# IVRL/NoiseDiff

Measured on AMD Instinct MI355X. Metric: sampled RAW patches/sec (256x256x4, 1000-step DDPM), higher is better.
Workload: dtype f32; 1 GPU; NoiseDiffNet dim=64, 256x256x4 patches, 1000-step DDPM (sigmoid2, pred_v), 16 patches per GPU; a step = one reverse-diffusion step (U-Net forward + fused posterior/noise update) over the per-GPU batch; patches/s = n_gpus*16/(1000*s_per_step); global_batch=16, launch=hipGraph replay, noise=device Philox4x32-10

## Files before the change

### include/noisediff_hip.h

```cpp
#ifndef NOISEDIFF_HIP_H
#define NOISEDIFF_HIP_H

#include <stdint.h>

#ifdef __cplusplus
extern "C" {
#endif

#define ND_E_BADARG   (-1)
#define ND_E_SHAPE    (-2)
#define ND_E_ALIGN    (-3)
#define ND_E_STATE    (-4)

int         nd_version(void);
const char* nd_last_error(void);
int         nd_device_arch(char* buf, int n);


enum nd_prologue {
    ND_PRO_NONE        = 0,
    ND_PRO_AFFINE_SILU = 1,
    ND_PRO_AFFINE_MAP_SILU = 2,
    ND_PRO_LAYERNORM   = 3,
    ND_PRO_SILU        = 4,
    ND_PRO_LEAKY       = 5,
    ND_PRO_LEAKY_SECOND = 6,
    ND_PRO_AFFINE_GENMAP_SILU = 7
};

typedef struct nd_src {
    const float* p0;
    const float* p1;
    int32_t c0, c1;
    int32_t ld0, ld1;
    int32_t mode;
    int32_t upsample;
    int32_t unshuffle;
    int32_t map_blocked;
    const float* mad;
    const float* map;
    const float* vec;
    const float* gamma;
    const float* beta;
    const float* rowstats;
} nd_src;

enum nd_act { ND_ACT_NONE = 0, ND_ACT_GELU = 1, ND_ACT_SILU = 2 };


typedef struct nd_conv3x3 {
    nd_src   src;
    const float* weight;
    const float* bias;
    float*   out;
    float*   stats;
    float*   slot_count;
    int32_t  B, H, W;
    int32_t  cin, cout, ldo;
} nd_conv3x3;

int nd_conv3x3_nhwc_f32(const nd_conv3x3* d, void* stream);
int nd_conv3x3_stat_slots(int H, int W, int cout, int B);
int nd_conv3x3_tiling_id(int B, int H, int W, int cout);
int64_t nd_pack_conv3x3_weight_floats(int cin, int cout);
int nd_pack_conv3x3_weight(const float* oihw, float* packed, int cin, int cout, void* stream);
int nd_pack_conv3x3_weight_dgrad(const float* oihw_fwd, float* packed, int cin, int cout, void* stream);

int nd_conv3x3_wino_nhwc_f32(const nd_conv3x3* d, void* stream);
int nd_conv3x3_wino2_nhwc_f32(const nd_conv3x3* d, void* stream);
int nd_conv3x3_wino_stat_slots(int H, int W);
int64_t nd_pack_conv3x3_wino_weight_floats(int cin, int cout);
int nd_pack_conv3x3_wino_weight(const float* oihw, float* packed, int cin, int cout, void* stream);
int nd_pack_conv3x3_wino_weight_dgrad(const float* oihw_fwd, float* packed, int cin, int cout, void* stream);

int nd_conv3x3_wino4_nhwc_f32(const nd_conv3x3* d, void* stream);
int nd_conv3x3_wino4_16_nhwc_f32(const nd_conv3x3* d, void* stream);
int nd_conv3x3_wino4_stat_slots(int H, int W);
int64_t nd_pack_conv3x3_wino4_weight_floats(int cin, int cout);
int nd_pack_conv3x3_wino4_weight(const float* oihw, float* packed, int cin, int cout, void* stream);
int nd_pack_conv3x3_wino4_weight_dgrad(const float* oihw_fwd, float* packed, int cin, int cout, void* stream);
typedef struct nd_pack_item {
    const float* w;
    float*       packed;
    int32_t      cin, cout, transposed, reserved;
} nd_pack_item;
int nd_pack_conv3x3_wino4_weights_batch(const nd_pack_item* items_dev, int n_items, void* stream);
int nd_conv3x3_wino4_splitk_plan(int B, int H, int W, int cin, int cout);
int64_t nd_conv3x3_wino4_splitk_workspace_floats(int B, int H, int W, int cout, int splits);
int nd_conv3x3_wino4_splitk_nhwc_f32(const nd_conv3x3* d, float* workspace, int splits, void* stream);
int nd_conv3x3_wino4_16_splitk_plan(int H, int W, int cin, int cout);
int nd_conv3x3_wino4_16_splitk_nhwc_f32(const nd_conv3x3* d, float* workspace, int splits, void* stream);


int64_t nd_conv3x3_wgrad_workspace_floats(int B, int H, int W, int cin, int cout);
int nd_conv3x3_wgrad_cat_nhwc_f32(const float* x0, int ldx0, int c0, const float* x1, int ldx1, int c1, const float* dy, int ldy, float* dw_oihw,
                                  float* dbias, float* workspace, int B, int H, int W, int cout, void* stream);
int nd_conv3x3_wgrad_form(int form);
int nd_conv3x3_wgrad_nhwc_f32(const float* x, int ldx, const float* dy, int ldy, float* dw_oihw, float* dbias, float* workspace,
                              int B, int H, int W, int cin, int cout, void* stream);
int nd_conv3x3_wgrad_leaky_nhwc_f32(const float* x, int ldx, const float* dy, int ldy, float* dw_oihw, float* dbias, float* workspace,
                                    int B, int H, int W, int cin, int cout, void* stream);
int64_t nd_conv3x3_wgrad_cat_workspace_floats(int B, int H, int W, int c0, int c1, int cout);
int nd_conv3x3_wgrad_cat_leaky_second_nhwc_f32(const float* x0, int ldx0, int c0, const float* x1, int ldx1, int c1, const float* dy, int ldy,
                                               float* dw_oihw, float* dbias, float* workspace, int B, int H, int W, int cout, void* stream);
int nd_leaky_grad_join_f32(const float* z, float* dz, const float* d_direct, int ld_direct, const float* d_pool, int B, int H, int W, int C,
                           void* stream);

int64_t nd_groupnorm_train_workspace_floats(int B, int HW, int C);
int nd_groupnorm_train_forward_f32(const float* x, int ldx, const float* gamma, const float* beta, float* y, int ldy, float* mean_rstd,
                                   float* workspace, int B, int HW, int C, int groups, float eps, void* stream);
int nd_groupnorm_train_backward_f32(const float* dy, int lddy, const float* x, int ldx, const float* gamma, const float* mean_rstd,
                                    float* dx, int lddx, float* dgamma, float* dbeta, float* workspace, int B, int HW, int C, int groups,
                                    void* stream);

int64_t nd_groupnorm_silu_train_workspace_floats(int B, int HW, int C);
int nd_groupnorm_silu_train_forward_f32(const float* x, int ldx, const float* gamma, const float* beta, const float* scale_shift, const float* res, int ldr,
                                        float* y, int ldy, float* mean_rstd, float* mad, float* workspace, int B, int HW, int C, int groups, float eps,
                                        void* stream);
int nd_groupnorm_silu_train_backward_f32(const float* dy, int lddy, const float* x, int ldx, const float* gamma, const float* beta,
                                         const float* scale_shift, const float* mean_rstd, const float* mad, float* dx, int lddx,
                                         float* dgamma, float* dbeta, float* dscale_shift, float* workspace, int B, int HW, int C, int groups,
                                         void* stream);

int nd_modulate_silu_forward_f32(const float* n, int ldn, const float* map, int ldm, float* y, int ldy, int64_t N, int C, void* stream);
int nd_modulate_silu_backward_f32(const float* dy, int lddy, const float* n, int ldn, const float* map, int ldm, float* dn, int lddn, float* dmap, int lddm,
                                  int64_t N, int C, void* stream);

int64_t nd_token_sum_workspace_floats(int B, int HW, int C);
int nd_token_sum_f32(const float* x, int ldx, float* out, float* workspace, int B, int HW, int C, void* stream);

int64_t nd_layernorm_train_workspace_floats(int64_t N, int C);
int nd_layernorm_train_forward_f32(const float* x, int ldx, const float* gamma, const float* beta, float* y, int ldy, float* stats,
                                   int64_t N, int C, float eps, void* stream);
int nd_layernorm_train_backward_f32(const float* dy, int lddy, const float* x, int ldx, const float* gamma, const float* stats,
                                    float* dx, int lddx, float* dgamma, float* dbeta, float* workspace, int64_t N, int C, void* stream);

int64_t nd_linear_wgrad_workspace_floats(int64_t N, int cin, int cout);
int nd_linear_wgrad_f32(const float* x, int ldx, const float* dy, int ldy, float* dw, float* dbias, float* workspace,
                        int64_t N, int cin, int cout, void* stream);
int nd_linear_wgrad_leaky_f32(const float* x, int ldx, const float* dy, int ldy, float* dw, float* dbias, float* workspace,
                              int64_t N, int cin, int cout, void* stream);
int64_t nd_convt2x2_wgrad_workspace_floats(int B, int h, int w, int cin, int cout);
int nd_convt2x2_wgrad_leaky_f32(const float* x, int ldx, const float* d_up, int ld_up, float* dw, float* workspace, int B, int h, int w,
                                int cin, int cout, int up_h, int up_w, void* stream);


typedef struct nd_pointwise {
    nd_src   src;
    const float* weight;
    const float* bias;
    float*   out;
    const float* res0; const float* res1;
    const float* vec;
    const float* gn_t;
    const float* gn_mad;
    int32_t  B, HW, W;
    int32_t  cin, cout, ldo, ldr0, ldr1, ldt;
    int32_t  act;
    int32_t  shuffle_c;
    int32_t  shuffle_h, shuffle_w;
} nd_pointwise;

int nd_pointwise_gemm_nhwc_f32(const nd_pointwise* d, void* stream);
int nd_pointwise_gemm_unshuffle_crop_nhwc_f32(const nd_pointwise* d, int src_h, int src_w, void* stream);

int64_t nd_image_quality_workspace_bytes(int B, int C, int H, int W);
int nd_image_quality_f32(const float* est, const float* target, const float* scale, double data_range, double* psnr, double* ssim,
                         double* mse, void* workspace, int B, int C, int H, int W, void* stream);
int64_t nd_illum_scale_workspace_bytes(int B, int C, int H, int W);
int nd_illum_scale_f32(const float* pred, const float* source, int source_batch, float* k32, double* k64, void* workspace,
                       int B, int C, int H, int W, void* stream);
int nd_illum_apply_f32(const float* pred, const float* k32, float* out, int B, int C, int H, int W, void* stream);

int     nd_histogram_chunk_elements(void);
int64_t nd_histogram_workspace_bytes(int S, int64_t n, int n_bins);
int nd_histogram_f32(const float* x, int S, int64_t n, const double* edges, int n_edges, int64_t* counts, void* workspace, void* stream);
int nd_kl_div_f64(const int64_t* p_counts, const int64_t* q_counts, int64_t n_p, int64_t n_q, int n_bins, int S, int q_sets, double* out,
                  void* stream);
int nd_kl_div_hist_f64(const double* p, const double* q, int n_bins, int S, int q_sets, double* out, void* stream);
int64_t nd_patch_std_mean_workspace_bytes(int B, int C, int H, int W);
int nd_patch_std_mean_f32(const float* x, float* std, float* mean, double* fit, void* workspace, int B, int C, int H, int W, void* stream);

int64_t nd_level_table_bytes(int n_levels);
int nd_level_moments_reset(uint64_t* table, int n_levels, uint64_t* counters, void* stream);
int nd_level_moments_f32(const float* clean, const float* noisy, int64_t n, float scale, int n_levels, uint64_t* table, uint64_t* counters,
                         void* stream);
int nd_level_stats_f64(const uint64_t* table, int n_levels, int64_t* count, double* mean, double* std, void* stream);
int nd_level_curve_f64(const int64_t* count, const double* std, int n_levels, float scale, int below_median, double* x, double* y, int32_t* m,
                       void* stream);
int64_t nd_theil_sen_workspace_bytes(int max_m, int64_t n_pairs);
int nd_theil_sen_f64(const double* x, const double* y, const int32_t* m, int max_m, const int32_t* pairs, int64_t n_pairs, int max_iter,
                     double tol, double* out, void* workspace, void* stream);

typedef struct nd_denoise_sample {
    int32_t x0, y0;
    int32_t cx, cy;
    int32_t flip;
    int32_t branch;
    float iso, ratio, blc;
    int32_t reserved[3];
} nd_denoise_sample;
#define ND_DENOISE_SNA_WORDS 8
int nd_denoise_batch_f32(const float* noise, const float* clean, const float* ds_k_high, const float* ds_b_high, const float* ds_k_low,
                         const float* ds_b_low, int map_h, int map_w, const nd_denoise_sample* table, const float* sna, const int64_t* rng,
                         uint64_t seed, int64_t first_sample, int32_t draw, const float* counts_in, float* counts_out, float* noisy,
                         float* clean_out, int B, int patch, int crop_h, int crop_w, void* stream);
int nd_philox_poisson_f32(const float* rate, float* out, uint64_t seed, int64_t first_sample, int32_t draw, int B, int64_t n_per_sample,
                          void* stream);
int nd_pack_darkshading_f32(const float* bayer, float* planes, int H2, int W2, void* stream);

typedef struct nd_raw_sample {
    int32_t frame;
    int32_t frame_clean;
    int32_t x0, y0;
    int32_t flip;
    int32_t branch;
    float iso, ratio, blc;
    int32_t reserved;
    double k, sd, ratio64;
} nd_raw_sample;
enum nd_raw_mode {
    ND_RAW_PACK = 0,
    ND_RAW_PACK_SHADED = 1,
    ND_RAW_TRAIN_REAL = 2
};
#define ND_RAW_RESCALE 1
#define ND_RAW_CLIP 2
int nd_raw_pack_u16_f32(const uint16_t* frames, int N, int H2, int W2, const float* ds_k_high, const float* ds_b_high, const float* ds_k_low,
                        const float* ds_b_low, int map_h, int map_w, const nd_raw_sample* table, int mode, int flags, float black, float white,
                        float* out, float* clean_out, int B, int h, int w, void* stream);
int nd_raw_poisson_gaussian_f32(const uint16_t* frames, int N, int H2, int W2, const nd_raw_sample* table, const int64_t* rng, uint64_t seed,
                                int64_t first_sample, int32_t draw, const float* counts_in, const float* normals_in, float* counts_out,
                                float* normals_out, float black, float white, float* noisy, float* clean_out, int B, int h, int w,
                                void* stream);
int nd_raw_to_bayer_u16(const float* img, uint16_t* out, const int32_t* bl, int white, int B, int h, int w, void* stream);
int nd_raw_diffusion_batch_f32(const uint16_t* frames, int N, int H2, int W2, const nd_raw_sample* table, float black, float white, float* noise,
                               float* noisy, float* clean, float* coord, int B, int h, int w, void* stream);
int64_t nd_pack_pointwise_weight_floats(int cin, int cout);
int nd_pack_pointwise_weight(const float* w, float* packed, int cin, int cout, int unshuffle_c, void* stream);
int nd_pack_pointwise_weight_t(const float* w_t, float* packed, int cin, int cout, void* stream);
int nd_pack_pointwise_weights_batch(const nd_pack_item* items_dev, int n_items, void* stream);

int nd_pointwise_gemm_split_nhwc_f32(const nd_pointwise* d, void* stream);
int nd_pointwise_gemm_split_takes(const nd_pointwise* d);
int64_t nd_pack_pointwise_weight_split_floats(int cin, int cout);
int nd_pack_pointwise_weight_split(const float* w, float* packed, int cin, int cout, void* stream);

enum nd_chain_res { ND_CHAIN_RES_NONE = 0, ND_CHAIN_RES_INPUT = 1 , ND_CHAIN_RES_INPUT_RAW = 2  };
typedef struct nd_chain_stage {
    const float* weight;
    const float* bias;
    int32_t  cin, cout;
    int32_t  act;
    int32_t  res;
} nd_chain_stage;
typedef struct nd_chain {
    nd_src   src;
    nd_chain_stage st[3];
    float*   out;
    int32_t  n_stages, B, HW, ldo;
} nd_chain;
int nd_pointwise_chain_nhwc_f32(const nd_chain* d, void* stream);
int nd_pointwise_chain_supported(int cin, int n1, int n2, int n3);
int64_t nd_pack_chain_weight_floats(int cin, int cout, int first_stage);
int nd_pack_chain_weight(const float* w, float* packed, int cin, int cout, int first_stage, void* stream);
int nd_pointwise_chain_split_nhwc_f32(const nd_chain* d, void* stream);
int64_t nd_pack_chain_weight_split_floats(int cin, int cout, int first_stage);
int nd_pack_chain_weight_split(const float* w, float* packed, int cin, int cout, int first_stage, void* stream);


int nd_groupnorm_finalize_f32(const float* stats, const float* slot_count, int slots,
                              const float* gamma, const float* beta,
                              const float* scale_shift, int ld_ss,
                              float* mad, int B, int C, int groups, float eps, void* stream);
int nd_groupnorm_finalize_train_f32(const float* stats, const float* slot_count, int slots, const float* gamma, const float* beta,
                                    const float* scale_shift, int ld_ss, float* mad, float* mean_rstd, int B, int C, int groups, float eps,
                                    void* stream);

int nd_layernorm_stats_f32(const float* x, int ldx, const float* vec, float* stats,
                           int B, int HW, int C, float eps, void* stream);

int nd_affine_silu_add_f32(const float* t, int ldt, const float* mad,
                           const float* res0, int ldr0, const float* res1, int ldr1,
                           float* out, int ldo, int B, int HW, int C, void* stream);


int nd_linear_rows_f32(const float* in, int ld_in, const float* W, const float* bias,
                       float* out, int ld_out, int B, int K, int N,
                       int act_in, int act_out, void* stream);
int nd_sinusoidal_time_emb_f32(const int64_t* time, const float* freqs, float* emb, int B, int half, void* stream);
int64_t nd_cond_step_lds_bytes(int B, int dim);
int nd_cond_step_f32(const int64_t* time, const float* freqs, const float* W1, const float* b1, const float* W2, const float* b2,
                     const float* Wp, const float* bp, float* out, int ld_out, int B, int dim, int J, void* stream);
int nd_cond_table_build_f32(const float* freqs, const float* W1, const float* b1, const float* W2, const float* b2, float* table, int rows, int dim,
                            void* stream);
int nd_cond_step_table_f32(const int64_t* time, const float* freqs, const float* W1, const float* b1, const float* W2, const float* b2,
                           const float* Wp, const float* bp, float* out, int ld_out, int B, int dim, int J, const float* table, int table_rows,
                           void* stream);
int nd_cond_step_ptable_f32(const int64_t* time, const float* freqs, const float* W1, const float* b1, const float* W2, const float* b2,
                            const float* Wp, const float* bp, float* out, int ld_out, int B, int dim, int J, const float* table, int table_rows,
                            const float* ptable, void* stream);
int nd_embedding_rows_f32(const int64_t* idx, const float* table, float* out, int B, int rows, int dim, void* stream);


int nd_conv7x7_c4_f32(const float* x, const float* wpacked, const float* bias, float* out, int ldo,
                      int B, int H, int W, int cout, void* stream);
int64_t nd_conv7x7_c4_wgrad_workspace_floats(int B, int H, int W, int cout);
int nd_conv7x7_c4_wgrad_f32(const float* x, const float* dy, int ldy, float* dw_oihw, float* dbias, float* workspace, int B, int H, int W, int cout,
                            void* stream);
int nd_pack_conv7x7_weight(const float* oihw, float* packed, int cout, void* stream);
int nd_conv7x7_c4_split_f32(const float* x, const float* wsplit, const float* bias, float* out, int ldo,
                            int B, int H, int W, int cout, void* stream);
int64_t nd_pack_conv7x7_weight_split_floats(int cout);
int nd_pack_conv7x7_weight_split(const float* oihw, float* packed, int cout, void* stream);
int nd_pos_enc_f32(const float* position_nchw, const float* w , const float* bias,
                   float* out, int B, int H, int W, int hid, void* stream);
int nd_maxpool2x2_nhwc_f32(const float* in, float* out, int B, int H, int W, int C, void* stream);
int nd_nchw_to_nhwc_f32(const float* in, float* out, int B, int C, int H, int W, void* stream);
int nd_nhwc_to_nchw_f32(const float* in, float* out, int B, int C, int H, int W, void* stream);
int nd_nchw_to_nhwc_pad_f32(const float* in, float* out, int B, int C, int H, int W, int Cpad, void* stream);


typedef struct nd_sampler_state {
    int32_t* step;
    const int32_t* t_cur;
    const int32_t* t_next;
    const float* coef;
    int64_t* time_out;
    const int64_t* rng;
    int32_t n_steps, B;
} nd_sampler_state;

int nd_sampler_begin_step(const nd_sampler_state* s, void* stream);
int nd_sampler_advance(const nd_sampler_state* s, void* stream);

int nd_sampler_step_ddpm_f32(float* x, const float* model_out, const float* noise, int64_t noise_step_stride,
                             const nd_sampler_state* s, int objective,
                             uint64_t seed, int64_t first_sample,
                             int B, int HW, int C, void* stream);
int nd_sampler_step_ddim_f32(float* x, const float* model_out, const float* noise, int64_t noise_step_stride,
                             const nd_sampler_state* s, int objective,
                             uint64_t seed, int64_t first_sample,
                             int B, int HW, int C, void* stream);
int nd_philox_normal_f32(float* out, uint64_t seed, int64_t first_sample, int32_t step,
                         int B, int HW, int C, void* stream);


int nd_attention_mfma_f32(const float* qkv, int ld_qkv, float* out, int ld_out,
                          int B, int N, int heads, int dh, void* stream);
int64_t nd_linear_attention_workspace_floats(int B, int N, int heads);
int nd_linear_attention_f32(const float* qkv, int ld_qkv, float* out, int ld_out, float* workspace,
                            int B, int N, int heads, int dh, void* stream);
int nd_rmsnorm_nhwc_f32(const float* x, int ldx, const float* g, float* out, int ldo,
                        int B, int HW, int C, void* stream);
int nd_rmsnorm_add_nhwc_f32(const float* x, int ldx, const float* g, const float* res, int ldr, float* out, int ldo, int B, int HW, int C, void* stream);


int nd_attention_train_forward_f32(const float* qkv, int ld_qkv, float* out, int ld_out, float* lse,
                                   int B, int N, int heads, int dh, void* stream);
int64_t nd_attention_backward_workspace_floats(int B, int N, int heads);
int nd_attention_backward_f32(const float* qkv, int ld_qkv, const float* out, int ld_out, const float* dout, int ld_dout, const float* lse,
                              float* dqkv, int ld_dqkv, float* workspace, int B, int N, int heads, int dh, void* stream);
int64_t nd_linear_attention_backward_workspace_floats(int B, int N, int heads);
int nd_linear_attention_backward_f32(const float* qkv, int ld_qkv, const float* dout, int ld_dout, const float* fwd_workspace, float* dqkv,
                                     int ld_dqkv, float* workspace, int B, int N, int heads, int dh, void* stream);
int64_t nd_rmsnorm_backward_workspace_floats(int64_t npix, int C);
int nd_rmsnorm_backward_f32(const float* dy, int lddy, const float* x, int ldx, const float* g, float* dx, int lddx, float* dg, float* workspace,
                            int B, int HW, int C, void* stream);

typedef struct nd_adam_item {
    float*       p;
    const float* g;
    float*       m;
    float*       v;
    int64_t      n;
    float        step_size, bias2_sqrt;
    int32_t      vec4, reserved;
    float*       step;
} nd_adam_item;
int nd_adam_chunk_elements(void);
int nd_adam_step_f32(const nd_adam_item* items_dev, int n_items, const int32_t* chunks_dev, int n_chunks, float beta1, float beta2, float eps,
                     float weight_decay, void* stream);
int nd_adam_step_capturable_f32(const nd_adam_item* items_dev, int n_items, const int32_t* chunks_dev, int n_chunks, float lr, float beta1, float beta2,
                                float eps, float weight_decay, void* stream);
int nd_adam_step_capturable_lr_f32(const nd_adam_item* items_dev, int n_items, const int32_t* chunks_dev, int n_chunks, const float* lr_dev, float beta1,
                                   float beta2, float eps, float weight_decay, void* stream);

typedef struct nd_ema_item {
    float*       ema;
    const float* src;
    int64_t      n;
    int32_t      vec4, no_ema;
} nd_ema_item;
int nd_ema_chunk_elements(void);
int nd_ema_update_f32(const nd_ema_item* items_dev, int n_items, const int32_t* chunks_dev, int n_chunks, int64_t* step_dev, uint8_t* initted_dev,
                      void* plan_dev, double beta, int64_t update_after_step, int64_t update_every, double inv_gamma, double power, double min_value,
                      void* stream);

typedef struct nd_diffusion_noising {
    const float* x0;
    const float* noise;
    const float* offset;
    const int64_t* t_in;
    const float* sqrt_alphas_cumprod;
    const float* sqrt_one_minus_alphas_cumprod;
    const int64_t* rng;
    int64_t* t_out;
    float* x_t;
    float* target;
    float* noise_out;
    float* offset_out;
    uint64_t seed;
    int64_t first_sample;
    int64_t draw;
    float offset_strength;
    int32_t B, C, H, W, T;
    int32_t objective, auto_normalize, x0_channels_last;
} nd_diffusion_noising;
int nd_diffusion_noising_f32(const nd_diffusion_noising* p, void* stream);
int nd_diffusion_train_advance(int64_t* rng, void* stream);
int nd_diffusion_loss_slice_elements(void);
int64_t nd_diffusion_loss_workspace_bytes(int B, int C, int HW);
int nd_diffusion_loss_f32(const float* model_out, const float* target, const int64_t* t, const float* loss_weight, int B, int C, int HW, int T,
                          int x0_term, void* workspace, float* loss, float* sample_loss, void* stream);
int nd_diffusion_loss_backward_f32(const float* model_out, const float* target, const int64_t* t, const float* loss_weight, const float* g,
                                   const void* workspace, float* grad_out, int B, int C, int HW, int T, int x0_term, void* stream);

enum nd_layout { ND_LAYOUT_NCHW = 0, ND_LAYOUT_NHWC = 1 };
int nd_denoise_loss_slice_pixels(void);
int64_t nd_denoise_loss_workspace_bytes(int B, int C, int HW);
int nd_denoise_loss_f32(const float* out, int out_layout, const float* target, int B, int C, int HW, double lambda_l1, double lambda_mse,
                        void* workspace, float* terms, float* sample_terms, void* stream);
int nd_denoise_loss_backward_f32(const float* out, int out_layout, const float* target, const float* g, float* grad, int B, int C, int HW,
                                 double lambda_l1, double lambda_mse, void* stream);

int nd_stream_create(void** stream);
int nd_stream_destroy(void* stream);
int nd_stream_sync(void* stream);
int nd_graph_begin(void* stream);
int nd_graph_end(void* stream, void** graph_exec);
int nd_graph_launch(void* graph_exec, void* stream);
int nd_graph_destroy(void* graph_exec);
int nd_stream_device(void* stream);
int nd_event_create(void** ev);
int nd_event_record(void* ev, void* stream);
int nd_event_elapsed_ms(void* start, void* stop, float* ms);
int nd_event_destroy(void* ev);
int nd_event_create_untimed(void** ev);
int nd_stream_wait_event(void* stream, void* ev);

#ifdef __cplusplus
}
#endif
#endif
```

### noisediff_amd/_lib.py

```python
from __future__ import annotations

import ctypes as C
import os
from typing import Optional

HERE = os.path.dirname(os.path.abspath(__file__))
LIB_PATH = os.path.join(HERE, "libnoisediff_hip.so")

PRO_NONE, PRO_AFFINE_SILU, PRO_AFFINE_MAP_SILU, PRO_LAYERNORM, PRO_SILU, PRO_LEAKY, PRO_LEAKY_SECOND, PRO_AFFINE_GENMAP_SILU = 0, 1, 2, 3, 4, 5, 6, 7
ACT_NONE, ACT_GELU, ACT_SILU = 0, 1, 2
OBJECTIVES = {"pred_noise": 0, "pred_x0": 1, "pred_v": 2}
LAYOUT_NCHW, LAYOUT_NHWC = 0, 1

fptr = C.c_void_p


class HipError(RuntimeError):
    pass


class Src(C.Structure):
    _fields_ = [("p0", fptr), ("p1", fptr), ("c0", C.c_int32), ("c1", C.c_int32), ("ld0", C.c_int32), ("ld1", C.c_int32),
                ("mode", C.c_int32), ("upsample", C.c_int32), ("unshuffle", C.c_int32), ("map_blocked", C.c_int32),
                ("mad", fptr), ("map", fptr), ("vec", fptr), ("gamma", fptr), ("beta", fptr), ("rowstats", fptr)]


class AdamItem(C.Structure):
    _fields_ = [("p", fptr), ("g", fptr), ("m", fptr), ("v", fptr), ("n", C.c_int64), ("step_size", C.c_float), ("bias2_sqrt", C.c_float),
                ("vec4", C.c_int32), ("reserved", C.c_int32), ("step", fptr)]


class EmaItem(C.Structure):
    _fields_ = [("ema", fptr), ("src", fptr), ("n", C.c_int64), ("vec4", C.c_int32), ("no_ema", C.c_int32)]


class PackItem(C.Structure):
    _fields_ = [("w", fptr), ("packed", fptr), ("cin", C.c_int32), ("cout", C.c_int32), ("transposed", C.c_int32), ("reserved", C.c_int32)]


class Conv3x3(C.Structure):
    _fields_ = [("src", Src), ("weight", fptr), ("bias", fptr), ("out", fptr), ("stats", fptr), ("slot_count", fptr),
                ("B", C.c_int32), ("H", C.c_int32), ("W", C.c_int32), ("cin", C.c_int32), ("cout", C.c_int32), ("ldo", C.c_int32)]


class Pointwise(C.Structure):
    _fields_ = [("src", Src), ("weight", fptr), ("bias", fptr), ("out", fptr), ("res0", fptr), ("res1", fptr), ("vec", fptr),
                ("gn_t", fptr), ("gn_mad", fptr), ("B", C.c_int32), ("HW", C.c_int32), ("W", C.c_int32), ("cin", C.c_int32),
                ("cout", C.c_int32), ("ldo", C.c_int32), ("ldr0", C.c_int32), ("ldr1", C.c_int32), ("ldt", C.c_int32), ("act", C.c_int32),
                ("shuffle_c", C.c_int32), ("shuffle_h", C.c_int32), ("shuffle_w", C.c_int32)]


class ChainStage(C.Structure):
    _fields_ = [("weight", fptr), ("bias", fptr), ("cin", C.c_int32), ("cout", C.c_int32), ("act", C.c_int32), ("res", C.c_int32)]


class Chain(C.Structure):
    _fields_ = [("src", Src), ("st", ChainStage * 3), ("out", fptr), ("n_stages", C.c_int32), ("B", C.c_int32), ("HW", C.c_int32),
                ("ldo", C.c_int32)]


class RawSample(C.Structure):
    _fields_ = [("frame", C.c_int32), ("frame_clean", C.c_int32), ("x0", C.c_int32), ("y0", C.c_int32), ("flip", C.c_int32),
                ("branch", C.c_int32), ("iso", C.c_float), ("ratio", C.c_float), ("blc", C.c_float), ("reserved", C.c_int32),
                ("k", C.c_double), ("sd", C.c_double), ("ratio64", C.c_double)]


RAW_PACK, RAW_PACK_SHADED, RAW_TRAIN_REAL = 0, 1, 2
RAW_RESCALE, RAW_CLIP = 1, 2
CHAIN_RES_NONE, CHAIN_RES_INPUT, CHAIN_RES_INPUT_RAW = 0, 1, 2


class SamplerState(C.Structure):
    _fields_ = [("step", fptr), ("t_cur", fptr), ("t_next", fptr), ("coef", fptr), ("time_out", fptr), ("rng", fptr),
                ("n_steps", C.c_int32), ("B", C.c_int32)]


class DiffusionNoising(C.Structure):
    _fields_ = [("x0", fptr), ("noise", fptr), ("offset", fptr), ("t_in", fptr), ("sqrt_alphas_cumprod", fptr), ("sqrt_one_minus_alphas_cumprod", fptr),
                ("rng", fptr), ("t_out", fptr), ("x_t", fptr), ("target", fptr), ("noise_out", fptr), ("offset_out", fptr),
                ("seed", C.c_uint64), ("first_sample", C.c_int64), ("draw", C.c_int64), ("offset_strength", C.c_float),
                ("B", C.c_int32), ("C", C.c_int32), ("H", C.c_int32), ("W", C.c_int32), ("T", C.c_int32),
                ("objective", C.c_int32), ("auto_normalize", C.c_int32), ("x0_channels_last", C.c_int32)]


i32, i64, u64, vp, f32, f64 = C.c_int, C.c_int64, C.c_uint64, C.c_void_p, C.c_float, C.c_double

SIGNATURES = {
    "nd_version": (i32, []),
    "nd_last_error": (C.c_char_p, []),
    "nd_device_arch": (i32, [C.c_char_p, i32]),
    "nd_conv3x3_nhwc_f32": (i32, [C.POINTER(Conv3x3), vp]),
    "nd_conv3x3_stat_slots": (i32, [i32, i32, i32, i32]),
    "nd_conv3x3_tiling_id": (i32, [i32, i32, i32, i32]),
    "nd_pack_conv3x3_weight_floats": (i64, [i32, i32]),
    "nd_pack_conv3x3_weight": (i32, [vp, vp, i32, i32, vp]),
    "nd_pack_conv3x3_weight_dgrad": (i32, [vp, vp, i32, i32, vp]),
    "nd_conv3x3_wino_nhwc_f32": (i32, [C.POINTER(Conv3x3), vp]),
    "nd_conv3x3_wino2_nhwc_f32": (i32, [C.POINTER(Conv3x3), vp]),
    "nd_conv3x3_wino_stat_slots": (i32, [i32, i32]),
    "nd_conv3x3_wino4_stat_slots": (i32, [i32, i32]),
    "nd_pack_conv3x3_wino_weight_floats": (i64, [i32, i32]),
    "nd_pack_conv3x3_wino_weight": (i32, [vp, vp, i32, i32, vp]),
    "nd_pack_conv3x3_wino_weight_dgrad": (i32, [vp, vp, i32, i32, vp]),
    "nd_conv3x3_wino4_nhwc_f32": (i32, [C.POINTER(Conv3x3), vp]),
    "nd_conv3x3_wino4_16_nhwc_f32": (i32, [C.POINTER(Conv3x3), vp]),
    "nd_pack_conv3x3_wino4_weight_floats": (i64, [i32, i32]),
    "nd_pack_conv3x3_wino4_weight": (i32, [vp, vp, i32, i32, vp]),
    "nd_pack_conv3x3_wino4_weight_dgrad": (i32, [vp, vp, i32, i32, vp]),
    "nd_conv3x3_wino4_splitk_plan": (i32, [i32, i32, i32, i32, i32]),
    "nd_conv3x3_wino4_splitk_workspace_floats": (i64, [i32, i32, i32, i32, i32]),
    "nd_conv3x3_wino4_splitk_nhwc_f32": (i32, [vp, vp, i32, vp]),
    "nd_conv3x3_wino4_16_splitk_plan": (i32, [i32, i32, i32, i32]),
    "nd_conv3x3_wino4_16_splitk_nhwc_f32": (i32, [vp, vp, i32, vp]),
    "nd_conv3x3_wgrad_workspace_floats": (i64, [i32, i32, i32, i32, i32]),
    "nd_conv3x3_wgrad_nhwc_f32": (i32, [vp, i32, vp, i32, vp, vp, vp, i32, i32, i32, i32, i32, vp]),
    "nd_groupnorm_train_workspace_floats": (i64, [i32, i32, i32]),
    "nd_linear_wgrad_workspace_floats": (i64, [i64, i32, i32]),
    "nd_groupnorm_silu_train_workspace_floats": (i64, [i32, i32, i32]),
    "nd_groupnorm_silu_train_forward_f32": (i32, [vp, i32, vp, vp, vp, vp, i32, vp, i32, vp, vp, vp, i32, i32, i32, i32, C.c_float, vp]),
    "nd_token_sum_workspace_floats": (i64, [i32, i32, i32]),
    "nd_token_sum_f32": (i32, [vp, i32, vp, vp, i32, i32, i32, vp]),
    "nd_modulate_silu_forward_f32": (i32, [vp, i32, vp, i32, vp, i32, i64, i32, vp]),
    "nd_modulate_silu_backward_f32": (i32, [vp, i32, vp, i32, vp, i32, vp, i32, vp, i32, i64, i32, vp]),
    "nd_groupnorm_silu_train_backward_f32": (i32, [vp, i32, vp, i32, vp, vp, vp, vp, vp, vp, i32, vp, vp, vp, vp, i32, i32, i32, i32, vp]),
    "nd_layernorm_train_workspace_floats": (i64, [i64, i32]),
    "nd_layernorm_train_forward_f32": (i32, [vp, i32, vp, vp, vp, i32, vp, i64, i32, C.c_float, vp]),
    "nd_layernorm_train_backward_f32": (i32, [vp, i32, vp, i32, vp, vp, vp, i32, vp, vp, vp, i64, i32, vp]),
    "nd_linear_wgrad_f32": (i32, [vp, i32, vp, i32, vp, vp, vp, i64, i32, i32, vp]),
    "nd_groupnorm_train_forward_f32": (i32, [vp, i32, vp, vp, vp, i32, vp, vp, i32, i32, i32, i32, C.c_float, vp]),
    "nd_groupnorm_train_backward_f32": (i32, [vp, i32, vp, i32, vp, vp, vp, i32, vp, vp, vp, i32, i32, i32, i32, vp]),
    "nd_pointwise_gemm_nhwc_f32": (i32, [C.POINTER(Pointwise), vp]),
    "nd_pointwise_chain_nhwc_f32": (i32, [C.POINTER(Chain), vp]),
    "nd_pointwise_chain_supported": (i32, [i32, i32, i32, i32]),
    "nd_pack_chain_weight_floats": (i64, [i32, i32, i32]),
    "nd_pack_chain_weight": (i32, [vp, vp, i32, i32, i32, vp]),
    "nd_pointwise_chain_split_nhwc_f32": (i32, [C.POINTER(Chain), vp]),
    "nd_pack_chain_weight_split_floats": (i64, [i32, i32, i32]),
    "nd_pack_chain_weight_split": (i32, [vp, vp, i32, i32, i32, vp]),
    "nd_pointwise_gemm_split_nhwc_f32": (i32, [C.POINTER(Pointwise), vp]),
    "nd_pointwise_gemm_split_takes": (i32, [C.POINTER(Pointwise)]),
    "nd_pack_pointwise_weight_split_floats": (i64, [i32, i32]),
    "nd_pack_pointwise_weight_split": (i32, [vp, vp, i32, i32, vp]),
    "nd_pack_pointwise_weight_floats": (i64, [i32, i32]),
    "nd_pack_pointwise_weight": (i32, [vp, vp, i32, i32, i32, vp]),
    "nd_pack_pointwise_weight_t": (i32, [vp, vp, i32, i32, vp]),
    "nd_pack_pointwise_weights_batch": (i32, [vp, i32, vp]),
    "nd_pack_conv3x3_wino4_weights_batch": (i32, [vp, i32, vp]),
    "nd_conv3x3_wgrad_cat_nhwc_f32": (i32, [vp, i32, i32, vp, i32, i32, vp, i32, vp, vp, vp, i32, i32, i32, i32, vp]),
    "nd_conv3x3_wgrad_form": (i32, [i32]),
    "nd_conv7x7_c4_wgrad_workspace_floats": (i64, [i32, i32, i32, i32]),
    "nd_conv7x7_c4_wgrad_f32": (i32, [vp, vp, i32, vp, vp, vp, i32, i32, i32, i32, vp]),
    "nd_adam_chunk_elements": (i32, []),
    "nd_adam_step_f32": (i32, [vp, i32, vp, i32, f32, f32, f32, f32, vp]),
    "nd_adam_step_capturable_f32": (i32, [vp, i32, vp, i32, f32, f32, f32, f32, f32, vp]),
    "nd_adam_step_capturable_lr_f32": (i32, [vp, i32, vp, i32, vp, f32, f32, f32, f32, vp]),
    "nd_ema_chunk_elements": (i32, []),
    "nd_ema_update_f32": (i32, [vp, i32, vp, i32, vp, vp, vp, f64, i64, i64, f64, f64, f64, vp]),
    "nd_diffusion_noising_f32": (i32, [C.POINTER(DiffusionNoising), vp]),
    "nd_diffusion_train_advance": (i32, [vp, vp]),
    "nd_diffusion_loss_slice_elements": (i32, []),
    "nd_diffusion_loss_workspace_bytes": (i64, [i32, i32, i32]),
    "nd_diffusion_loss_f32": (i32, [vp, vp, vp, vp, i32, i32, i32, i32, i32, vp, vp, vp, vp]),
    "nd_diffusion_loss_backward_f32": (i32, [vp, vp, vp, vp, vp, vp, vp, i32, i32, i32, i32, i32, vp]),
    "nd_denoise_loss_slice_pixels": (i32, []),
    "nd_denoise_loss_workspace_bytes": (i64, [i32, i32, i32]),
    "nd_denoise_loss_f32": (i32, [vp, i32, vp, i32, i32, i32, f64, f64, vp, vp, vp, vp]),
    "nd_denoise_loss_backward_f32": (i32, [vp, i32, vp, vp, vp, i32, i32, i32, f64, f64, vp]),
    "nd_groupnorm_finalize_f32": (i32, [vp, vp, i32, vp, vp, vp, i32, vp, i32, i32, i32, f32, vp]),
    "nd_groupnorm_finalize_train_f32": (i32, [vp, vp, i32, vp, vp, vp, i32, vp, vp, i32, i32, i32, f32, vp]),
    "nd_layernorm_stats_f32": (i32, [vp, i32, vp, vp, i32, i32, i32, f32, vp]),
    "nd_affine_silu_add_f32": (i32, [vp, i32, vp, vp, i32, vp, i32, vp, i32, i32, i32, i32, vp]),
    "nd_linear_rows_f32": (i32, [vp, i32, vp, vp, vp, i32, i32, i32, i32, i32, i32, vp]),
    "nd_sinusoidal_time_emb_f32": (i32, [vp, vp, vp, i32, i32, vp]),
    "nd_cond_step_lds_bytes": (i64, [i32, i32]),
    "nd_cond_step_f32": (i32, [vp, vp, vp, vp, vp, vp, vp, vp, vp, i32, i32, i32, i32, vp]),
    "nd_cond_table_build_f32": (i32, [vp, vp, vp, vp, vp, vp, i32, i32, vp]),
    "nd_cond_step_table_f32": (i32, [vp, vp, vp, vp, vp, vp, vp, vp, vp, i32, i32, i32, i32, vp, i32, vp]),
    "nd_cond_step_ptable_f32": (i32, [vp, vp, vp, vp, vp, vp, vp, vp, vp, i32, i32, i32, i32, vp, i32, vp, vp]),
    "nd_embedding_rows_f32": (i32, [vp, vp, vp, i32, i32, i32, vp]),
    "nd_conv7x7_c4_f32": (i32, [vp, vp, vp, vp, i32, i32, i32, i32, i32, vp]),
    "nd_pack_conv7x7_weight": (i32, [vp, vp, i32, vp]),
    "nd_conv7x7_c4_split_f32": (i32, [vp, vp, vp, vp, i32, i32, i32, i32, i32, vp]),
    "nd_pack_conv7x7_weight_split_floats": (i64, [i32]),
    "nd_pack_conv7x7_weight_split": (i32, [vp, vp, i32, vp]),
    "nd_pos_enc_f32": (i32, [vp, vp, vp, vp, i32, i32, i32, i32, vp]),
    "nd_maxpool2x2_nhwc_f32": (i32, [vp, vp, i32, i32, i32, i32, vp]),
    "nd_nchw_to_nhwc_pad_f32": (i32, [vp, vp, i32, i32, i32, i32, i32, vp]),
    "nd_nchw_to_nhwc_f32": (i32, [vp, vp, i32, i32, i32, i32, vp]),
    "nd_nhwc_to_nchw_f32": (i32, [vp, vp, i32, i32, i32, i32, vp]),
    "nd_sampler_begin_step": (i32, [C.POINTER(SamplerState), vp]),
    "nd_sampler_advance": (i32, [C.POINTER(SamplerState), vp]),
    "nd_sampler_step_ddpm_f32": (i32, [vp, vp, vp, i64, C.POINTER(SamplerState), i32, u64, i64, i32, i32, i32, vp]),
    "nd_sampler_step_ddim_f32": (i32, [vp, vp, vp, i64, C.POINTER(SamplerState), i32, u64, i64, i32, i32, i32, vp]),
    "nd_philox_normal_f32": (i32, [vp, u64, i64, i32, i32, i32, i32, vp]),
    "nd_attention_mfma_f32": (i32, [vp, i32, vp, i32, i32, i32, i32, i32, vp]),
    "nd_attention_train_forward_f32": (i32, [vp, i32, vp, i32, vp, i32, i32, i32, i32, vp]),
    "nd_attention_backward_workspace_floats": (i64, [i32, i32, i32]),
    "nd_attention_backward_f32": (i32, [vp, i32, vp, i32, vp, i32, vp, vp, i32, vp, i32, i32, i32, i32, vp]),
    "nd_linear_attention_backward_workspace_floats": (i64, [i32, i32, i32]),
    "nd_linear_attention_backward_f32": (i32, [vp, i32, vp, i32, vp, vp, i32, vp, i32, i32, i32, i32, vp]),
    "nd_rmsnorm_backward_workspace_floats": (i64, [i64, i32]),
    "nd_rmsnorm_backward_f32": (i32, [vp, i32, vp, i32, vp, vp, i32, vp, vp, i32, i32, i32, vp]),
    "nd_linear_attention_workspace_floats": (i64, [i32, i32, i32]),
    "nd_linear_attention_f32": (i32, [vp, i32, vp, i32, vp, i32, i32, i32, i32, vp]),
    "nd_rmsnorm_nhwc_f32": (i32, [vp, i32, vp, vp, i32, i32, i32, i32, vp]),
    "nd_rmsnorm_add_nhwc_f32": (i32, [vp, i32, vp, vp, i32, vp, i32, i32, i32, i32, vp]),
    "nd_stream_create": (i32, [C.POINTER(vp)]),
    "nd_stream_destroy": (i32, [vp]),
    "nd_stream_sync": (i32, [vp]),
    "nd_graph_begin": (i32, [vp]),
    "nd_graph_end": (i32, [vp, C.POINTER(vp)]),
    "nd_graph_launch": (i32, [vp, vp]),
    "nd_graph_destroy": (i32, [vp]),
    "nd_event_create": (i32, [C.POINTER(vp)]),
    "nd_event_record": (i32, [vp, vp]),
    "nd_event_elapsed_ms": (i32, [vp, vp, C.POINTER(f32)]),
    "nd_event_destroy": (i32, [vp]),
    "nd_event_create_untimed": (i32, [C.POINTER(vp)]),
    "nd_stream_wait_event": (i32, [vp, vp]),
    "nd_stream_device": (i32, [vp]),
    "nd_conv3x3_wgrad_leaky_nhwc_f32": (i32, [vp, i32, vp, i32, vp, vp, vp, i32, i32, i32, i32, i32, vp]),
    "nd_conv3x3_wgrad_cat_workspace_floats": (i64, [i32, i32, i32, i32, i32, i32]),
    "nd_conv3x3_wgrad_cat_leaky_second_nhwc_f32": (i32, [vp, i32, i32, vp, i32, i32, vp, i32, vp, vp, vp, i32, i32, i32, i32, vp]),
    "nd_leaky_grad_join_f32": (i32, [vp, vp, vp, i32, vp, i32, i32, i32, i32, vp]),
    "nd_linear_wgrad_leaky_f32": (i32, [vp, i32, vp, i32, vp, vp, vp, i64, i32, i32, vp]),
    "nd_convt2x2_wgrad_workspace_floats": (i64, [i32, i32, i32, i32, i32]),
    "nd_convt2x2_wgrad_leaky_f32": (i32, [vp, i32, vp, i32, vp, vp, i32, i32, i32, i32, i32, i32, i32, vp]),
    "nd_pointwise_gemm_unshuffle_crop_nhwc_f32": (i32, [C.POINTER(Pointwise), i32, i32, vp]),
    "nd_image_quality_workspace_bytes": (i64, [i32, i32, i32, i32]),
    "nd_image_quality_f32": (i32, [vp, vp, vp, f64, vp, vp, vp, vp, i32, i32, i32, i32, vp]),
    "nd_illum_scale_workspace_bytes": (i64, [i32, i32, i32, i32]),
    "nd_illum_scale_f32": (i32, [vp, vp, i32, vp, vp, vp, i32, i32, i32, i32, vp]),
    "nd_illum_apply_f32": (i32, [vp, vp, vp, i32, i32, i32, i32, vp]),
    "nd_histogram_chunk_elements": (i32, []),
    "nd_histogram_workspace_bytes": (i64, [i32, i64, i32]),
    "nd_histogram_f32": (i32, [vp, i32, i64, vp, i32, vp, vp, vp]),
    "nd_kl_div_f64": (i32, [vp, vp, i64, i64, i32, i32, i32, vp, vp]),
    "nd_kl_div_hist_f64": (i32, [vp, vp, i32, i32, i32, vp, vp]),
    "nd_patch_std_mean_workspace_bytes": (i64, [i32, i32, i32, i32]),
    "nd_patch_std_mean_f32": (i32, [vp, vp, vp, vp, vp, i32, i32, i32, i32, vp]),
    "nd_level_table_bytes": (i64, [i32]),
    "nd_level_moments_reset": (i32, [vp, i32, vp, vp]),
    "nd_level_moments_f32": (i32, [vp, vp, i64, f32, i32, vp, vp, vp]),
    "nd_level_stats_f64": (i32, [vp, i32, vp, vp, vp, vp]),
    "nd_level_curve_f64": (i32, [vp, vp, i32, f32, i32, vp, vp, vp, vp]),
    "nd_theil_sen_workspace_bytes": (i64, [i32, i64]),
    "nd_theil_sen_f64": (i32, [vp, vp, vp, i32, vp, i64, i32, f64, vp, vp, vp]),
    "nd_denoise_batch_f32": (i32, [vp, vp, vp, vp, vp, vp, i32, i32, vp, vp, vp, u64, i64, i32, vp, vp, vp, vp, i32, i32, i32, i32, vp]),
    "nd_philox_poisson_f32": (i32, [vp, vp, u64, i64, i32, i32, i64, vp]),
    "nd_pack_darkshading_f32": (i32, [vp, vp, i32, i32, vp]),
    "nd_raw_pack_u16_f32": (i32, [vp, i32, i32, i32, vp, vp, vp, vp, i32, i32, vp, i32, i32, f32, f32, vp, vp, i32, i32, i32, vp]),
    "nd_raw_poisson_gaussian_f32": (i32, [vp, i32, i32, i32, vp, vp, u64, i64, i32, vp, vp, vp, vp, f32, f32, vp, vp, i32, i32, i32, vp]),
    "nd_raw_to_bayer_u16": (i32, [vp, vp, C.POINTER(C.c_int32), i32, i32, i32, i32, vp]),
    "nd_raw_diffusion_batch_f32": (i32, [vp, i32, i32, i32, vp, f32, f32, vp, vp, vp, vp, i32, i32, i32, vp]),
}

_UNCHECKED = {"nd_version", "nd_last_error", "nd_stream_device", "nd_conv3x3_wgrad_form", "nd_adam_chunk_elements", "nd_ema_chunk_elements", "nd_conv7x7_c4_wgrad_workspace_floats", "nd_conv3x3_stat_slots", "nd_conv3x3_tiling_id", "nd_pack_conv3x3_weight_floats",
              "nd_pack_pointwise_weight_floats", "nd_linear_attention_workspace_floats", "nd_conv3x3_wino_stat_slots", "nd_conv3x3_wino4_stat_slots",
              "nd_pack_conv3x3_wino_weight_floats", "nd_pack_conv3x3_wino4_weight_floats", "nd_conv3x3_wino4_splitk_plan", "nd_conv3x3_wino4_16_splitk_plan", "nd_conv3x3_wino4_splitk_workspace_floats", "nd_token_sum_workspace_floats", "nd_cond_step_lds_bytes", "nd_conv3x3_wgrad_workspace_floats",
              "nd_groupnorm_train_workspace_floats", "nd_linear_wgrad_workspace_floats",
              "nd_layernorm_train_workspace_floats", "nd_groupnorm_silu_train_workspace_floats", "nd_conv3x3_wgrad_cat_workspace_floats",
              "nd_convt2x2_wgrad_workspace_floats", "nd_image_quality_workspace_bytes", "nd_illum_scale_workspace_bytes",
              "nd_histogram_chunk_elements", "nd_histogram_workspace_bytes", "nd_patch_std_mean_workspace_bytes", "nd_level_table_bytes",
              "nd_theil_sen_workspace_bytes", "nd_attention_backward_workspace_floats", "nd_linear_attention_backward_workspace_floats",
              "nd_rmsnorm_backward_workspace_floats", "nd_diffusion_loss_slice_elements", "nd_diffusion_loss_workspace_bytes",
              "nd_denoise_loss_slice_pixels", "nd_denoise_loss_workspace_bytes"}

_lib: Optional[C.CDLL] = None


def load(path: str = LIB_PATH) -> C.CDLL:
    global _lib
    if _lib is not None:
        return _lib
    import torch
    if not os.path.exists(path):
        raise HipError(f"{path} is missing: the HIP library is the product and there is no fallback. "
                       "Build it with `python -m noisediff_amd.build`.")
    lib = C.CDLL(path)
    for name, (res, args) in SIGNATURES.items():
        fn = getattr(lib, name)
        fn.restype, fn.argtypes = res, args
    _lib = lib
    return lib


def check(code: int, what: str = "") -> None:
    if code != 0:
        msg = load().nd_last_error().decode(errors="replace")
        raise HipError(f"{what or 'libnoisediff_hip'} failed with code {code}: {msg}")


def call(name: str, *args):
    r = getattr(load(), name)(*args)
    if name not in _UNCHECKED:
        check(r, name)
    return r


def ptr(t) -> Optional[int]:
    return None if t is None else t.data_ptr()
```

### noisediff_amd/csrc/pointwise.hip

```cpp
#include <stdlib.h>
#include <type_traits>
#include "nd_common.h"
#include "split_bf16.h"

namespace {

constexpr int KC = 64;
constexpr int LDA = KC + 4;

struct PwArgs {
    nd_pointwise d;
    int m_tiles, n_tiles, coutP, cinP, total_wg;
    int uns_h, uns_w;
};

template <int MB, int NB, int JB = 0>
__device__ __forceinline__ void pw_epilogue(const PwArgs& a, f32x16 (&acc)[MB][NB], float* As, int b, int p0, int n0, unsigned long long* ph = nullptr) {
    constexpr int BM = 2 * MB * 32, BN = 2 * NB * 32;
    constexpr int LDO = BN + 4;
    const int tid = threadIdx.x, lane = tid & 63, wave = tid >> 6;
    const int wm = wave >> 1, wn = wave & 1;
    const int col = lane & 31;
    const int HW = a.d.HW, W = a.d.W, Cout = a.d.cout;
    if (ph) ph[0] = __builtin_amdgcn_s_memtime();
// ... 530 lines not shown
                const float* m = s.mad + (size_t)b * 3 * Cin + c + 4 * j;
                pA[j] = nd_ld4(m); pB[j] = nd_ld4(m + Cin); pC[j] = nd_ld4(m + 2 * Cin);
            }
        }
    };
    auto stage_write = [&](char* dst) {
#pragma unroll
        for (int it = 0; it < 2; ++it) {
            const int r = prow + it * 64;
            u32x4 t1, t2, t3;
#pragma unroll
            for (int j = 0; j < 2; ++j) {
                f32x4 v = raw[it][j];
                if (MODE == ND_PRO_LAYERNORM) v = ((v + pC[j]) - rmean[it]) * rrstd[it] * pA[j] + pB[j];
                else if (MODE == ND_PRO_SILU) v = nd_silu4(v);
                else if (MODE == ND_PRO_AFFINE_SILU) v = nd_silu4((v - pA[j]) * pB[j] + pC[j]);
                else if (MODE == ND_PRO_LEAKY) v = nd_leaky4(v);
                const f32x4 zero = {0, 0, 0, 0};
                v = (p0 + r < HW) ? v : zero;
                unsigned u1, u2, u3;
                nd_split2_bf16(v.x, v.y, u1, u2, u3);  t1[2 * j] = u1;  t2[2 * j] = u2;  t3[2 * j] = u3;
                nd_split2_bf16(v.z, v.w, u1, u2, u3);  t1[2 * j + 1] = u1;  t2[2 * j + 1] = u2;  t3[2 * j + 1] = u3;
            }
            char* o = dst + r * SROW + seg * 16;
            *reinterpret_cast<u32x4*>(o) = t1;
            *reinterpret_cast<u32x4*>(o + SPLANE) = t2;
            *reinterpret_cast<u32x4*>(o + 2 * SPLANE) = t3;
        }
    };
    auto kstep = [&](auto slot_c, const char* src, int k2) {
        constexpr int S = decltype(slot_c)::value;
        u32x4 av[MB][3];
#pragma unroll
        for (int mb = 0; mb < MB; ++mb)
#pragma unroll
            for (int t = 0; t < 3; ++t) av[mb][t] = *reinterpret_cast<const u32x4*>(src + t * SPLANE + a_off[mb] + k2 * 32);
#pragma unroll
        for (int mb = 0; mb < MB; ++mb)
#pragma unroll
            for (int nb = 0; nb < NB; ++nb) {
                f32x16 c = acc[mb][nb];
                c = nd_mfma_bf16(av[mb][0], bq[S][0][nb], c);
                c = nd_mfma_bf16(av[mb][1], bq[S][0][nb], c);
                c = nd_mfma_bf16(av[mb][0], bq[S][1][nb], c);
                c = nd_mfma_bf16(av[mb][1], bq[S][1][nb], c);
                c = nd_mfma_bf16(av[mb][2], bq[S][0][nb], c);
                c = nd_mfma_bf16(av[mb][0], bq[S][2][nb], c);
                acc[mb][nb] = c;
            }
    };
    using S0 = std::integral_constant<int, 0>;
    using S1 = std::integral_constant<int, 1>;

    const int n_chunks = a.cinP / SKC, last_ks = 2 * n_chunks - 1;
#ifdef PWS_STAMP
    const unsigned long long st0 = __builtin_amdgcn_s_memtime();
#endif
    stage_load(0);
    load_b(0, 0);
    load_b(1, 1);
    stage_write(As);
    __syncthreads();
#ifdef PWS_STAMP
    const unsigned long long st1 = __builtin_amdgcn_s_memtime();
#endif
    for (int c = 0; c < n_chunks; ++c) {
        const char* cur = As + (c & 1) * SABUF;
        char* nxt = As + ((c + 1) & 1) * SABUF;
        const int cbn = (c + 1 < n_chunks ? c + 1 : c) * SKC;
        stage_load(cbn);
        __builtin_amdgcn_sched_barrier(0);
        kstep(S0{}, cur, 0);
        __builtin_amdgcn_sched_barrier(0);
        load_b(0, min(2 * c + 2, last_ks));
        __builtin_amdgcn_sched_barrier(0);
        kstep(S1{}, cur, 1);
        __builtin_amdgcn_sched_barrier(0);
        load_b(1, min(2 * c + 3, last_ks));
        stage_write(nxt);
        __syncthreads();
    }
#ifdef PWS_STAMP
    const unsigned long long st2 = __builtin_amdgcn_s_memtime();
    unsigned long long ph[4];
    pw_epilogue<MB, NB, 8>(a, acc, Ab, b, p0, n0, ph);
    if (tid == 0) {
        unsigned long long* o = reinterpret_cast<unsigned long long*>(a.d.out + ((size_t)b * HW + p0) * a.d.ldo + n0);
        const unsigned long long st3 = __builtin_amdgcn_s_memtime();
        o[0] = st1 - st0;  o[1] = st2 - st1;  o[2] = st3 - st2;
        o[3] = (ph[1] - ph[0]) | ((ph[2] - ph[1]) << 16) | ((ph[3] - ph[2]) << 32) | ((st3 - ph[3]) << 48);
    }
#else
    pw_epilogue<MB, NB, 8>(a, acc, Ab, b, p0, n0);
#endif
}

template <int MB, int NB, int MODE>
__global__ __launch_bounds__(256) void pointwise_kernel(const PwArgs a) {
    constexpr int WM = 2, WN = 2;
    constexpr int BM = WM * MB * 32, BN = WN * NB * 32;
    constexpr int STAGE_IT = BM / 16;
    constexpr int LDO = BN + 4;
    constexpr int SMEM = BM * (LDA > LDO ? LDA : LDO);
    __shared__ __attribute__((aligned(16))) float As[SMEM];

    const int tid = threadIdx.x, lane = tid & 63, wave = tid >> 6;
    const int wm = wave >> 1, wn = wave & 1;
    const int half = lane >> 5, col = lane & 31;

    int lid = nd_xcd_remap(blockIdx.x, a.total_wg);
    const int nt = lid % a.n_tiles;  lid /= a.n_tiles;
    const int mt = lid % a.m_tiles;
    const int b = lid / a.m_tiles;

    const nd_src& s = a.d.src;
    const int HW = a.d.HW, W = a.d.W, Cin = a.d.cin;
    const int p0 = mt * BM, n0 = nt * BN;

    int a_off[MB];
#pragma unroll
    for (int mb = 0; mb < MB; ++mb) a_off[mb] = ((wm * MB + mb) * 32 + col) * LDA + 4 * half;
    const __amdgpu_buffer_rsrc_t wrsrc = __builtin_amdgcn_make_buffer_rsrc(const_cast<float*>(a.d.weight), 0, a.cinP * a.coutP * 4, 0x00020000);
    const unsigned wvoff = (unsigned)((half * a.coutP + n0 + wn * NB * 32 + col) * 16);

    f32x16 acc[MB][NB];
#pragma unroll
    for (int mb = 0; mb < MB; ++mb)
#pragma unroll
        for (int nb = 0; nb < NB; ++nb)
#pragma unroll
            for (int r = 0; r < 16; ++r) acc[mb][nb][r] = 0.0f;

    const int quad = tid & 15, prow = tid >> 4;
    const int Cs = s.unshuffle ? (s.c0 >> 2) : 1;
    const int Hs2 = a.uns_h > 0 ? a.uns_h : 2 * (HW / max(W, 1));
    const int Ws2 = a.uns_w > 0 ? a.uns_w : 2 * W;

    for (int cb = 0; cb < a.cinP; cb += KC) {
        const int ng = min(8, (a.cinP - cb) >> 3);
        f32x4 bq[8][NB];
#pragma unroll
        for (int g = 0; g < 8; ++g)
#pragma unroll
            for (int nb = 0; nb < NB; ++nb)
                bq[g][nb] = __builtin_bit_cast(f32x4, __builtin_amdgcn_raw_buffer_load_b128(
                    wrsrc, wvoff, __builtin_amdgcn_readfirstlane((((cb >> 2) + 2 * min(g, ng - 1)) * a.coutP + nb * 32) * 16), 0));
        {
            const int c = cb + quad * 4;
            const bool cvalid = c < Cin;
            const int cs = cvalid ? c : 0;
            const float* base = s.p0;
            int ld = s.ld0, cc = cs, py = 0, px = 0;
            if (s.unshuffle) {
                const int sub = cs / Cs;
                cc = cs - sub * Cs; py = sub >> 1; px = sub & 1;
            } else if (cs >= s.c0) {
                base = s.p1; ld = s.ld1; cc = cs - s.c0;
            }
            f32x4 g4 = {1, 1, 1, 1}, b4 = {0, 0, 0, 0}, vec4 = {0, 0, 0, 0};
            f32x4 tM = {0, 0, 0, 0}, tA = {1, 1, 1, 1}, tD = {0, 0, 0, 0};
            if (MODE == ND_PRO_LAYERNORM) {
                g4 = nd_ld4(s.gamma + cs); b4 = nd_ld4(s.beta + cs);
                if (s.vec) vec4 = nd_ld4(s.vec + (size_t)b * Cin + cs);
            }
            if (MODE == ND_PRO_AFFINE_SILU) {
                const float* m = s.mad + (size_t)b * 3 * Cin + cs;
                tM = nd_ld4(m); tA = nd_ld4(m + Cin); tD = nd_ld4(m + 2 * Cin);
            }
            f32x4 raw[STAGE_IT];
            float rmean[STAGE_IT], rrstd[STAGE_IT];
            bool uin[STAGE_IT];
#pragma unroll
            for (int it = 0; it < STAGE_IT; ++it) {
                const int p = min(p0 + prow + it * 16, HW - 1);
                size_t pix = (size_t)b * HW + p;
                uin[it] = true;
                if (s.unshuffle) {
                    const int y = p / W, x = p - y * W;
                    const int sy = 2 * y + py, sx = 2 * x + px;
                    uin[it] = sy < Hs2 && sx < Ws2;
                    pix = ((size_t)b * Hs2 + (uin[it] ? sy : 0)) * Ws2 + (uin[it] ? sx : 0);
                }
                raw[it] = nd_ld4(base + pix * ld + cc);
                if (MODE == ND_PRO_LAYERNORM && s.rowstats) {
                    rmean[it] = s.rowstats[2 * pix];
                    rrstd[it] = s.rowstats[2 * pix + 1];
                }
            }
            if (MODE == ND_PRO_LAYERNORM && !s.rowstats) {
                const f32x4 zero = {0, 0, 0, 0};
#pragma unroll
                for (int it = 0; it < STAGE_IT; ++it) {
                    const f32x4 v = cvalid ? raw[it] + vec4 : zero;
                    const float mean = nd_row16_sum(v.x + v.y + v.z + v.w) / (float)Cin;
                    const f32x4 dv = cvalid ? v - mean : zero;
                    const float m2 = nd_row16_sum(dv.x * dv.x + dv.y * dv.y + dv.z * dv.z + dv.w * dv.w);
                    rmean[it] = mean;
                    rrstd[it] = rsqrtf(m2 / (float)Cin + 1e-5f);
                }
            }
            __syncthreads();
#pragma unroll
            for (int it = 0; it < STAGE_IT; ++it) {
                const int r = prow + it * 16;
                f32x4 v = raw[it];
                if (MODE == ND_PRO_LAYERNORM) v = ((v + vec4) - rmean[it]) * rrstd[it] * g4 + b4;
                else if (MODE == ND_PRO_SILU) v = nd_silu4(v);
                else if (MODE == ND_PRO_AFFINE_SILU) v = nd_silu4((v - tM) * tA + tD);
                else if (MODE == ND_PRO_LEAKY) v = nd_leaky4(v);
                const f32x4 zero = {0, 0, 0, 0};
                v = (cvalid && p0 + r < HW && uin[it]) ? v : zero;
                nd_st4(&As[r * LDA + quad * 4], v);
            }
        }
        __syncthreads();

        if (ng == 8) {
#pragma unroll
            for (int g = 0; g < 8; ++g) {
                f32x4 av[MB];
#pragma unroll
                for (int mb = 0; mb < MB; ++mb) av[mb] = nd_ld4(&As[a_off[mb] + g * 8]);
#pragma unroll
                for (int k = 0; k < 4; ++k)
#pragma unroll
                    for (int mb = 0; mb < MB; ++mb)
#pragma unroll
                        for (int nb = 0; nb < NB; ++nb)
                            acc[mb][nb] = nd_mfma(av[mb][k], bq[g][nb][k], acc[mb][nb]);
            }
        } else {
#pragma unroll
            for (int g = 0; g < 8; ++g) {
                if (g < ng) {
                    f32x4 av[MB];
#pragma unroll
                    for (int mb = 0; mb < MB; ++mb) av[mb] = nd_ld4(&As[a_off[mb] + g * 8]);
#pragma unroll
                    for (int k = 0; k < 4; ++k)
#pragma unroll
                        for (int mb = 0; mb < MB; ++mb)
#pragma unroll
                            for (int nb = 0; nb < NB; ++nb)
                                acc[mb][nb] = nd_mfma(av[mb][k], bq[g][nb][k], acc[mb][nb]);
                }
            }
        }
    }

    pw_epilogue<MB, NB>(a, acc, As, b, p0, n0);
}

template <int CO>
__global__ __launch_bounds__(256) void pointwise_narrow_kernel(const PwArgs a) {
    __shared__ __attribute__((aligned(16))) float wl[256 * 8 * 4];
    const int tid = threadIdx.x, part = tid & 3;
    const nd_src& s = a.d.src;
    const int nq = a.d.cin >> 2, cout = a.d.cout;
    for (int i = tid; i < nq * CO; i += 256) {
        const int kq = i / CO, n = i - kq * CO;
        const f32x4 zero = {0, 0, 0, 0};
        nd_st4(wl + i * 4, n < cout ? nd_ld4(a.d.weight + ((size_t)kq * a.coutP + n) * 4) : zero);
    }
    __syncthreads();
    const long P = (long)a.d.B * a.d.HW;
    for (long base = (long)blockIdx.x * 64; base < P; base += (long)gridDim.x * 64) {
        const long pix = base + (tid >> 2), pc = pix < P ? pix : P - 1;
        float acc[CO];
#pragma unroll
        for (int n = 0; n < CO; ++n) acc[n] = 0.0f;
        const float* r0 = s.p0 + pc * s.ld0;
        const float* r1 = s.p1 ? s.p1 + pc * s.ld1 - s.c0 : r0;
#pragma unroll 4
        for (int kq = part; kq < nq; kq += 4) {
            const int c = kq * 4;
            const f32x4 x = nd_ld4((c < s.c0 ? r0 : r1) + c);
#pragma unroll
            for (int n = 0; n < CO; ++n) {
                const f32x4 w = nd_ld4(wl + (kq * CO + n) * 4);
                acc[n] = fmaf(x.w, w.w, fmaf(x.z, w.z, fmaf(x.y, w.y, fmaf(x.x, w.x, acc[n]))));
            }
        }
#pragma unroll
        for (int n = 0; n < CO; ++n) {
            acc[n] += __int_as_float(__builtin_amdgcn_update_dpp(0, __float_as_int(acc[n]), 0xB1, 0xF, 0xF, true));
            acc[n] += __int_as_float(__builtin_amdgcn_update_dpp(0, __float_as_int(acc[n]), 0x4E, 0xF, 0xF, true));
        }
        if (part == 0 && pix < P) {
#pragma unroll
            for (int q = 0; q < CO / 4; ++q) {
                if (q * 4 >= cout) break;
                f32x4 v = {acc[4 * q], acc[4 * q + 1], acc[4 * q + 2], acc[4 * q + 3]};
                if (a.d.bias) v += nd_ld4(a.d.bias + 4 * q);
                if (a.d.act == ND_ACT_GELU) v = nd_gelu4(v);
                else if (a.d.act == ND_ACT_SILU) v = nd_silu4(v);
                if (a.d.res0) v += nd_ld4(a.d.res0 + pix * a.d.ldr0 + 4 * q);
                if (a.d.res1) v += nd_ld4(a.d.res1 + pix * a.d.ldr1 + 4 * q);
                nd_st4(a.d.out + pix * a.d.ldo + 4 * q, v);
            }
        }
    }
}

__global__ void pack_pointwise_kernel(const float* __restrict__ w, float* __restrict__ out,
                                      int cin, int cout, int cinP, int coutP, int unshuffle_c, int transposed) {
    const size_t total = (size_t)cinP * coutP;
    for (size_t i = blockIdx.x * (size_t)blockDim.x + threadIdx.x; i < total; i += (size_t)gridDim.x * blockDim.x) {
        const int e = i & 3;
        size_t r = i >> 2;
        const int n = r % coutP;
        const int q = r / coutP;
        const int kp = q * 4 + e;
        float v = 0.0f;
        if (n < cout && kp < cin) {
            int k = kp;
            if (unshuffle_c > 0) {
                const int sub = kp / unshuffle_c, c = kp - sub * unshuffle_c;
                k = c * 4 + sub;
            }
            v = transposed ? w[(size_t)k * cout + n] : w[(size_t)n * cin + k];
        }
        out[i] = v;
    }
}

__global__ void pack_pointwise_batch_kernel(const nd_pack_item* __restrict__ items) {
    const nd_pack_item it = items[blockIdx.y];
    const int cinP = (it.cin + 7) / 8 * 8, coutP = (it.cout + 63) / 64 * 64;
    const size_t total = (size_t)cinP * coutP;
    for (size_t i = blockIdx.x * (size_t)blockDim.x + threadIdx.x; i < total; i += (size_t)gridDim.x * blockDim.x) {
        const int e = i & 3;
        const size_t r = i >> 2;
        const int n = r % coutP, kp = (int)(r / coutP) * 4 + e;
        float v = 0.0f;
        if (n < it.cout && kp < it.cin) v = it.transposed ? it.w[(size_t)kp * it.cout + n] : it.w[(size_t)n * it.cin + kp];
        it.packed[i] = v;
    }
}

template <int MB, int NB>
void launch_pipe(const PwArgs& a, hipStream_t st) {
    const dim3 grid(a.total_wg), block(256);
    switch (a.d.src.mode) {
        case ND_PRO_LAYERNORM: hipLaunchKernelGGL((pointwise_pipe_kernel<MB, NB, ND_PRO_LAYERNORM>), grid, block, 0, st, a); break;
        case ND_PRO_SILU: hipLaunchKernelGGL((pointwise_pipe_kernel<MB, NB, ND_PRO_SILU>), grid, block, 0, st, a); break;
        case ND_PRO_AFFINE_SILU: hipLaunchKernelGGL((pointwise_pipe_kernel<MB, NB, ND_PRO_AFFINE_SILU>), grid, block, 0, st, a); break;
        case ND_PRO_LEAKY: hipLaunchKernelGGL((pointwise_pipe_kernel<MB, NB, ND_PRO_LEAKY>), grid, block, 0, st, a); break;
        default: hipLaunchKernelGGL((pointwise_pipe_kernel<MB, NB, ND_PRO_NONE>), grid, block, 0, st, a);
    }
}

template <int NB>
int launch_big(const PwArgs& a, hipStream_t st) {
    constexpr size_t lds = sizeof(float) * (2 * 128 * BLDA > 128 * (64 * NB + 4) ? 2 * 128 * BLDA : 128 * (64 * NB + 4));
    const dim3 grid(a.total_wg), block(256);
#define PWB_LAUNCH(MODE)                                                                                                      \
    {                                                                                                                         \
        static nd_device_once configured;                                                                                     \
        if (int e = nd_reserve_lds(configured, reinterpret_cast<const void*>(pointwise_big_kernel<NB, MODE>), lds, "nd_pointwise")) return e; \
        hipLaunchKernelGGL((pointwise_big_kernel<NB, MODE>), grid, block, lds, st, a);                                    \
    }
    switch (a.d.src.mode) {
        case ND_PRO_LAYERNORM: PWB_LAUNCH(ND_PRO_LAYERNORM) break;
        case ND_PRO_SILU: PWB_LAUNCH(ND_PRO_SILU) break;
        case ND_PRO_AFFINE_SILU: PWB_LAUNCH(ND_PRO_AFFINE_SILU) break;
        case ND_PRO_LEAKY: PWB_LAUNCH(ND_PRO_LEAKY) break;
        default: PWB_LAUNCH(ND_PRO_NONE)
    }
#undef PWB_LAUNCH
    return 0;
}

template <int MB, int NB>
void launch(const PwArgs& a, hipStream_t st) {
    const dim3 grid(a.total_wg), block(256);
    switch (a.d.src.mode) {
        case ND_PRO_LAYERNORM: hipLaunchKernelGGL((pointwise_kernel<MB, NB, ND_PRO_LAYERNORM>), grid, block, 0, st, a); break;
        case ND_PRO_SILU: hipLaunchKernelGGL((pointwise_kernel<MB, NB, ND_PRO_SILU>), grid, block, 0, st, a); break;
        case ND_PRO_AFFINE_SILU: hipLaunchKernelGGL((pointwise_kernel<MB, NB, ND_PRO_AFFINE_SILU>), grid, block, 0, st, a); break;
        case ND_PRO_LEAKY: hipLaunchKernelGGL((pointwise_kernel<MB, NB, ND_PRO_LEAKY>), grid, block, 0, st, a); break;
        default: hipLaunchKernelGGL((pointwise_kernel<MB, NB, ND_PRO_NONE>), grid, block, 0, st, a);
    }
}

__global__ void pack_pointwise_split_kernel(const float* __restrict__ w, unsigned short* __restrict__ out, int cin, int cout, int cinP, int coutP) {
    const size_t total = (size_t)cinP * coutP;
    const int n32 = coutP / 32;
    for (size_t idx = blockIdx.x * (size_t)blockDim.x + threadIdx.x; idx < total; idx += (size_t)gridDim.x * blockDim.x) {
        const int i = (int)(idx & 7), l = (int)((idx >> 3) & 63);
        const size_t rest = idx >> 9;
        const int tile = (int)(rest % n32), ks = (int)(rest / n32);
        const int n = 32 * tile + (l & 31), k = 16 * ks + 8 * (l >> 5) + i;
        const float v = (n < cout && k < cin) ? w[(size_t)n * cin + k] : 0.0f;
        const bf16_terms t = nd_split3_bf16(v);
        unsigned short* o = out + (((size_t)ks * 3 * n32 + tile) * 64 + l) * 8 + i;
        const size_t term = (size_t)n32 * 512;
        o[0] = t.t1;  o[term] = t.t2;  o[2 * term] = t.t3;
    }
}

int launch_split(const PwArgs& a, hipStream_t st) {
    const dim3 grid(a.total_wg), block(256);
#define PWS_LAUNCH(MODE)                                                                                                      \
    {                                                                                                                         \
        static nd_device_once configured;                                                                                     \
        if (int e = nd_reserve_lds(configured, reinterpret_cast<const void*>(pointwise_split_kernel<MODE>), SPLIT_LDS, "nd_pointwise_split")) return e; \
        hipLaunchKernelGGL((pointwise_split_kernel<MODE>), grid, block, SPLIT_LDS, st, a);                                    \
    }
    switch (a.d.src.mode) {
        case ND_PRO_LAYERNORM: PWS_LAUNCH(ND_PRO_LAYERNORM) break;
        case ND_PRO_SILU: PWS_LAUNCH(ND_PRO_SILU) break;
        case ND_PRO_AFFINE_SILU: PWS_LAUNCH(ND_PRO_AFFINE_SILU) break;
        case ND_PRO_LEAKY: PWS_LAUNCH(ND_PRO_LEAKY) break;
        default: PWS_LAUNCH(ND_PRO_NONE)
    }
#undef PWS_LAUNCH
    return 0;
}

}

extern "C" int64_t nd_pack_pointwise_weight_floats(int cin, int cout) {
    return (int64_t)nd_round_up(cin, 8) * nd_round_up(cout, 64);
}

extern "C" int nd_pack_pointwise_weight(const float* w, float* packed, int cin, int cout, int unshuffle_c, void* stream) {
    ND_REQUIRE(w && packed, ND_E_BADARG, "nd_pack_pointwise_weight: null pointer");
    ND_REQUIRE(cin > 0 && cout > 0, ND_E_BADARG, "nd_pack_pointwise_weight: non-positive size");
    ND_REQUIRE(unshuffle_c == 0 || (unshuffle_c * 4 == cin && unshuffle_c % 4 == 0), ND_E_SHAPE,
               "nd_pack_pointwise_weight: unshuffle_c=%d must be cin/4 and a multiple of 4", unshuffle_c);
    const int cinP = nd_round_up(cin, 8), coutP = nd_round_up(cout, 64);
    const size_t total = (size_t)cinP * coutP;
    const int blocks = (int)((total + 255) / 256 < 2048 ? (total + 255) / 256 : 2048);
    hipLaunchKernelGGL(pack_pointwise_kernel, dim3(blocks), dim3(256), 0, (hipStream_t)stream, w, packed, cin, cout, cinP, coutP, unshuffle_c, 0);
    return nd_launch_status("nd_pack_pointwise_weight");
}

extern "C" int nd_pack_pointwise_weight_t(const float* w_t, float* packed, int cin, int cout, void* stream) {
    ND_REQUIRE(w_t && packed, ND_E_BADARG, "nd_pack_pointwise_weight_t: null pointer");
    ND_REQUIRE(cin > 0 && cout > 0, ND_E_BADARG, "nd_pack_pointwise_weight_t: non-positive size");
    const int cinP = nd_round_up(cin, 8), coutP = nd_round_up(cout, 64);
    const size_t total = (size_t)cinP * coutP;
    const int blocks = (int)((total + 255) / 256 < 2048 ? (total + 255) / 256 : 2048);
    hipLaunchKernelGGL(pack_pointwise_kernel, dim3(blocks), dim3(256), 0, (hipStream_t)stream, w_t, packed, cin, cout, cinP, coutP, 0, 1);
    return nd_launch_status("nd_pack_pointwise_weight_t");
}

extern "C" int nd_pack_pointwise_weights_batch(const nd_pack_item* items_dev, int n_items, void* stream) {
    ND_REQUIRE(items_dev && n_items > 0 && n_items <= 65535, ND_E_BADARG, "nd_pack_pointwise_weights_batch: needs 1 .. 65535 items in device memory");
    hipLaunchKernelGGL(pack_pointwise_batch_kernel, dim3(32, (unsigned)n_items), dim3(256), 0, (hipStream_t)stream, items_dev);
    return nd_launch_status("nd_pack_pointwise_weights_batch");
}

namespace {
bool pw_pipe_takes(const nd_pointwise* d) {
    static const bool use_pipe = !(getenv("ND_PW_PIPE") && atoi(getenv("ND_PW_PIPE")) == 0);
    const nd_src& s = d->src;
    return use_pipe && d->cin % PKC == 0 && d->cin >= 2 * PKC && !s.unshuffle && (s.mode != ND_PRO_LAYERNORM || s.rowstats) && (s.c1 == 0 || nd_aligned16(s.p1));
}
long pw_big_tiles(const nd_pointwise* d) {
    static const int use_big = getenv("ND_PW_BIG") ? atoi(getenv("ND_PW_BIG")) : 1;
    const nd_src& s = d->src;
    if (!(pw_pipe_takes(d) && use_big && d->cin % BKC == 0 && d->cin >= 2 * BKC && d->cout % 128 == 0 && d->shuffle_c == 0 &&
          (s.c1 == 0 || s.c0 % BKC == 0) && (long)d->B * d->HW * s.ld0 * 4 < (1L << 32) && (long)d->B * d->HW * s.ld1 * 4 < (1L << 32))) return 0;
    const long tiles = (long)d->B * nd_cdiv(d->HW, 128) * (d->cout / 128);
    return tiles >= nd_device_cus() ? tiles : 0;
}

bool pw_split_takes(const nd_pointwise* d) {
    const nd_src& s = d->src;
    return d->cin % SKC == 0 && d->cin >= 2 * SKC && d->cout % 128 == 0 && !s.unshuffle && d->shuffle_c == 0 && (s.mode != ND_PRO_LAYERNORM || s.rowstats) &&
           (s.c1 == 0 || (s.c0 % SKC == 0 && nd_aligned16(s.p1)));
}

int pw_run(const nd_pointwise* d, void* stream, bool split = false, int uns_h = 0, int uns_w = 0) {
    ND_REQUIRE(d, ND_E_BADARG, "nd_pointwise: null descriptor");
    const nd_src& s = d->src;
    ND_REQUIRE(s.p0 && d->weight && d->out, ND_E_BADARG, "nd_pointwise: null tensor pointer");
    ND_REQUIRE(d->B > 0 && d->HW > 0 && d->cin > 0 && d->cout > 0, ND_E_BADARG, "nd_pointwise: non-positive size");
    ND_REQUIRE(d->cin % 4 == 0, ND_E_SHAPE, "nd_pointwise: cin=%d must be a multiple of 4", d->cin);
    ND_REQUIRE(s.c0 + s.c1 == d->cin && s.c0 % 4 == 0 && s.c1 % 4 == 0 && s.c0 > 0, ND_E_SHAPE,
               "nd_pointwise: source channels %d+%d do not match cin=%d", s.c0, s.c1, d->cin);
    ND_REQUIRE((s.c1 == 0) == (s.p1 == nullptr), ND_E_BADARG, "nd_pointwise: p1/c1 mismatch");
    ND_REQUIRE(s.ld0 % 4 == 0 && (s.c1 == 0 || s.ld1 % 4 == 0), ND_E_ALIGN, "nd_pointwise: pixel strides must be multiples of 4");
    ND_REQUIRE(nd_aligned16(s.p0) && nd_aligned16(s.p1) && nd_aligned16(d->weight) && nd_aligned16(s.vec) &&
               nd_aligned16(s.gamma) && nd_aligned16(s.beta) && nd_aligned16(s.mad), ND_E_ALIGN, "nd_pointwise: pointers must be 16-byte aligned");
    ND_REQUIRE(!s.upsample, ND_E_BADARG, "nd_pointwise: upsample is a conv3x3-only addressing mode");
    if (s.unshuffle) {
        ND_REQUIRE(s.c1 == 0 && d->W > 0 && d->HW % d->W == 0 && (s.c0 / 4) % 4 == 0 && s.mode == ND_PRO_NONE, ND_E_SHAPE,
                   "nd_pointwise: unshuffle needs one source, W | HW, c0/4 %% 4 == 0, no prologue");
        ND_REQUIRE(s.ld0 >= s.c0 / 4, ND_E_SHAPE, "nd_pointwise: ld0 < source channels");
    } else {
        ND_REQUIRE(s.ld0 >= s.c0 && (s.c1 == 0 || s.ld1 >= s.c1), ND_E_SHAPE, "nd_pointwise: ld < channels");
    }
    ND_REQUIRE(s.mode == ND_PRO_NONE || s.mode == ND_PRO_LAYERNORM || s.mode == ND_PRO_SILU || s.mode == ND_PRO_AFFINE_SILU ||
               s.mode == ND_PRO_LEAKY, ND_E_BADARG, "nd_pointwise: unsupported prologue %d", s.mode);
    if (d->shuffle_c > 0)
        ND_REQUIRE(d->cout == 4 * d->shuffle_c && d->shuffle_c % 4 == 0 && d->W > 0 && d->HW % d->W == 0 && d->shuffle_h > 0 && d->shuffle_w > 0 &&
                   d->ldo >= d->shuffle_c && !d->res0 && !d->res1 && !d->gn_t && !d->vec, ND_E_SHAPE,
                   "nd_pointwise: shuffle_c=%d needs cout == 4*shuffle_c, W | HW, an output size and no residual operands", d->shuffle_c);
    if (s.mode == ND_PRO_LAYERNORM) {
        ND_REQUIRE(s.gamma && s.beta && s.c1 == 0 && d->cin <= 1024, ND_E_SHAPE, "nd_pointwise: LayerNorm needs gamma/beta, one source, C <= 1024");
        ND_REQUIRE(d->cin <= 64 || s.rowstats, ND_E_BADARG, "nd_pointwise: LayerNorm over C=%d > 64 needs src.rowstats (nd_layernorm_stats_f32)", d->cin);
    }
    if (s.mode == ND_PRO_AFFINE_SILU) ND_REQUIRE(s.mad && s.c1 == 0, ND_E_BADARG, "nd_pointwise: affine prologue needs mad, one source");
    ND_REQUIRE(d->ldo >= d->cout || d->shuffle_c > 0, ND_E_SHAPE, "nd_pointwise: ldo < cout");
    ND_REQUIRE(d->ldo % 4 == 0 && (!d->res0 || d->ldr0 % 4 == 0) && (!d->res1 || d->ldr1 % 4 == 0) && (!d->gn_t || d->ldt % 4 == 0),
               ND_E_ALIGN, "nd_pointwise: output / residual pixel strides must be multiples of 4");
    ND_REQUIRE(nd_aligned16(d->out) && nd_aligned16(d->res0) && nd_aligned16(d->res1) && nd_aligned16(d->gn_t) && nd_aligned16(d->bias) &&
               nd_aligned16(d->vec) && nd_aligned16(d->gn_mad), ND_E_ALIGN, "nd_pointwise: epilogue pointers must be 16-byte aligned");
    ND_REQUIRE(!d->res0 || d->ldr0 >= d->cout, ND_E_SHAPE, "nd_pointwise: ldr0 < cout");
    ND_REQUIRE(!d->res1 || d->ldr1 >= d->cout, ND_E_SHAPE, "nd_pointwise: ldr1 < cout");
    ND_REQUIRE(!d->gn_t || (d->gn_mad && d->ldt >= d->cout), ND_E_BADARG, "nd_pointwise: gn_t needs gn_mad and ldt >= cout");
    ND_REQUIRE(d->act >= ND_ACT_NONE && d->act <= ND_ACT_SILU, ND_E_BADARG, "nd_pointwise: bad act");

    if (uns_h > 0 || uns_w > 0)
        ND_REQUIRE(s.unshuffle && uns_h > 0 && uns_w > 0 && uns_h <= 2 * (d->HW / d->W) && uns_w <= 2 * d->W, ND_E_SHAPE,
                   "nd_pointwise_gemm_unshuffle_crop: source (%d, %d) must lie within twice the (%d, %d) output", uns_h, uns_w, d->HW / d->W, d->W);
    PwArgs a;
    a.d = *d;
    a.uns_h = uns_h;  a.uns_w = uns_w;
    if (split) {
        ND_REQUIRE(pw_split_takes(d), ND_E_SHAPE, "nd_pointwise_gemm_split: %d -> %d is not a layer of the split kernel (cin %% 32, cin >= 64, cout %% 128, plain "
                   "addressing, LayerNorm with rowstats, concat on a 32-channel boundary: nd_pointwise_gemm_split_takes)", d->cin, d->cout);
        a.cinP = d->cin;  a.coutP = d->cout;
        a.m_tiles = nd_cdiv(d->HW, 128);
        a.n_tiles = d->cout / 128;
        const long wgs = (long)d->B * a.m_tiles * a.n_tiles;
        ND_REQUIRE(wgs < (1L << 31), ND_E_SHAPE, "nd_pointwise_gemm_split: grid too large");
        a.total_wg = (int)wgs;
        if (int e = launch_split(a, (hipStream_t)stream)) return e;
        return nd_launch_status("nd_pointwise_gemm_split_nhwc_f32");
    }
    a.cinP = nd_round_up(d->cin, 8);
    a.coutP = nd_round_up(d->cout, 64);
    static const int force_mb = getenv("ND_PW_MB") ? atoi(getenv("ND_PW_MB")) : 0;
    static const int force_nb = getenv("ND_PW_NB") ? atoi(getenv("ND_PW_NB")) : 0;
    int mb = force_mb ? force_mb : 1, nb = force_nb ? force_nb : ((d->cout % 128 == 0) ? 2 : 1);
    auto count = [&](int mb_, int nb_) { return (long)d->B * nd_cdiv(d->HW, 64 * mb_) * nd_cdiv(d->cout, 64 * nb_); };
    if (nb == 2 && count(mb, 2) < 512) nb = 1;
    if (count(mb, nb) < 512) mb = 1;
    a.m_tiles = nd_cdiv(d->HW, 64 * mb);
    a.n_tiles = nd_cdiv(d->cout, 64 * nb);
    const long wg = count(mb, nb);
    ND_REQUIRE(wg < (1L << 31), ND_E_SHAPE, "nd_pointwise: grid too large");
    a.total_wg = (int)wg;
    hipStream_t st = (hipStream_t)stream;
    static const bool use_narrow = !(getenv("ND_PW_NARROW") && atoi(getenv("ND_PW_NARROW")) == 0);
    if (use_narrow && d->cout <= 8 && d->cout % 4 == 0 && d->cin <= 1024 && s.mode == ND_PRO_NONE && !s.unshuffle && d->shuffle_c == 0 && !d->gn_t && !d->vec &&
        (s.c1 == 0 || nd_aligned16(s.p1))) {
        const long blocks = ((long)d->B * d->HW + 63) / 64;
        const int grid = (int)(blocks < 8L * nd_device_cus() ? blocks : 8L * nd_device_cus());
        if (d->cout <= 4) hipLaunchKernelGGL((pointwise_narrow_kernel<4>), dim3(grid), dim3(256), 0, st, a);
        else hipLaunchKernelGGL((pointwise_narrow_kernel<8>), dim3(grid), dim3(256), 0, st, a);
        return nd_launch_status("nd_pointwise_gemm_nhwc_f32");
    }
    const bool pipe = pw_pipe_takes(d);
    const long tiles = pw_big_tiles(d);
    if (tiles > 0) {
        a.m_tiles = nd_cdiv(d->HW, 128);
        a.n_tiles = d->cout / 128;
        a.total_wg = (int)tiles;
        if (int e = launch_big<2>(a, st)) return e;
        return nd_launch_status("nd_pointwise_gemm_nhwc_f32");
    }
    if (pipe) {
        if (mb == 2 && nb == 2) launch_pipe<2, 2>(a, st);
        else if (mb == 2) launch_pipe<2, 1>(a, st);
        else if (nb == 2) launch_pipe<1, 2>(a, st);
        else launch_pipe<1, 1>(a, st);
        return nd_launch_status("nd_pointwise_gemm_nhwc_f32");
    }
    if (mb == 2 && nb == 2) launch<2, 2>(a, st);
    else if (mb == 2) launch<2, 1>(a, st);
    else if (nb == 2) launch<1, 2>(a, st);
    else launch<1, 1>(a, st);
    return nd_launch_status("nd_pointwise_gemm_nhwc_f32");
}
}

extern "C" int nd_pointwise_gemm_nhwc_f32(const nd_pointwise* d, void* stream) { return pw_run(d, stream); }

extern "C" int nd_pointwise_gemm_unshuffle_crop_nhwc_f32(const nd_pointwise* d, int src_h, int src_w, void* stream) {
    ND_REQUIRE(d && d->W > 0 && d->src.unshuffle && src_h > 0 && src_w > 0, ND_E_BADARG, "nd_pointwise_gemm_unshuffle_crop: needs src.unshuffle and a source size");
    return pw_run(d, stream, false, src_h, src_w);
}

extern "C" int nd_pointwise_gemm_split_nhwc_f32(const nd_pointwise* d, void* stream) { return pw_run(d, stream, true); }

extern "C" int nd_pointwise_gemm_split_takes(const nd_pointwise* d) { return d && pw_split_takes(d) ? 1 : 0; }

extern "C" int64_t nd_pack_pointwise_weight_split_floats(int cin, int cout) {
    return (int64_t)nd_round_up(cin, 32) * nd_round_up(cout, 128) * 3 / 2;
}

extern "C" int nd_pack_pointwise_weight_split(const float* w, float* packed, int cin, int cout, void* stream) {
    ND_REQUIRE(w && packed && nd_aligned16(packed), ND_E_BADARG, "nd_pack_pointwise_weight_split: null or unaligned pointer");
    ND_REQUIRE(cin > 0 && cout > 0, ND_E_BADARG, "nd_pack_pointwise_weight_split: non-positive size");
    const int cinP = nd_round_up(cin, 32), coutP = nd_round_up(cout, 128);
    const size_t total = (size_t)cinP * coutP;
    const int blocks = (int)((total + 255) / 256 < 2048 ? (total + 255) / 256 : 2048);
    hipLaunchKernelGGL(pack_pointwise_split_kernel, dim3(blocks), dim3(256), 0, (hipStream_t)stream, w, reinterpret_cast<unsigned short*>(packed), cin, cout, cinP, coutP);
    return nd_launch_status("nd_pack_pointwise_weight_split");
}
```

### noisediff_amd/csrc/pwchain.hip

```cpp
#include <type_traits>
#include "nd_common.h"
#include "split_bf16.h"

namespace {

struct ChainArgs {
    nd_chain d;
    int n_tiles;
    int tiles_per_sample;
};

template <int K, int N>
__device__ __forceinline__ void chain_gemm(const float (&in)[K / 2], const float* __restrict__ w, const float* __restrict__ bias,
                                           f32x16 (&acc)[N / 32], const int lane) {
    const int half = lane >> 5;
#pragma unroll
    for (int nt = 0; nt < N / 32; ++nt)
#pragma unroll
        for (int g = 0; g < 4; ++g) {
            const f32x4 b4 = nd_ld4(bias + 32 * nt + 8 * g + 4 * half);
#pragma unroll
            for (int i = 0; i < 4; ++i) acc[nt][4 * g + i] = b4[i];
        }
#pragma unroll
    for (int jq = 0; jq < K / 8; ++jq)
#pragma unroll
        for (int nt = 0; nt < N / 32; ++nt) {
            const f32x4 a4 = nd_ld4(w + ((nt * (K / 8) + jq) * 64 + lane) * 4);
#pragma unroll
            for (int i = 0; i < 4; ++i) acc[nt] = nd_mfma(a4[i], in[4 * jq + i], acc[nt]);
        }
}

template <int K, int N>
__device__ __forceinline__ void chain_gemm_split(const float (&in)[K / 2], const char* __restrict__ w, const float* __restrict__ bias,
                                                 f32x16 (&acc)[N / 32], const int lane) {
    static_assert(K % 16 == 0, "whole 16-channel K steps");
    constexpr int S = K / 16, NT = N / 32;
    const int half = lane >> 5;
    const u32x4* const wl = reinterpret_cast<const u32x4*>(w) + lane;
    u32x4 wq[2][3], xs[2][3];
    auto load_w = [&](int slot, int s_, int nt_) {
        const u32x4* p = wl + ((nt_ * S + s_) * 3) * 64;
        wq[slot][0] = p[0];  wq[slot][1] = p[64];  wq[slot][2] = p[128];
    };
    auto split = [&](int slot, int s_) {
#pragma unroll
        for (int j = 0; j < 4; ++j) {
            unsigned t1, t2, t3;
            nd_split2_bf16(in[8 * s_ + 2 * j], in[8 * s_ + 2 * j + 1], t1, t2, t3);
            xs[slot][0][j] = t1;  xs[slot][1][j] = t2;  xs[slot][2][j] = t3;
        }
    };
    load_w(0, 0, 0);
#pragma unroll
    for (int nt = 0; nt < NT; ++nt)
#pragma unroll
        for (int g = 0; g < 4; ++g) {
            const f32x4 b4 = nd_ld4(bias + 32 * nt + 8 * g + 4 * half);
#pragma unroll
            for (int i = 0; i < 4; ++i) acc[nt][4 * g + i] = b4[i];
        }
    split(0, 0);
#pragma unroll
    for (int s = 0; s < S; ++s)
#pragma unroll
        for (int nt = 0; nt < NT; ++nt) {
            const int g = s * NT + nt;
            if (g + 1 < S * NT) load_w((g + 1) & 1, nt + 1 < NT ? s : s + 1, nt + 1 < NT ? nt + 1 : 0);
            __builtin_amdgcn_sched_barrier(0);
            if (nt == 0 && s + 1 < S) split((s + 1) & 1, s + 1);
            const u32x4 w1 = wq[g & 1][0], w2 = wq[g & 1][1], w3 = wq[g & 1][2];
            const u32x4 x1 = xs[s & 1][0], x2 = xs[s & 1][1], x3 = xs[s & 1][2];
            acc[nt] = nd_mfma_bf16(w1, x1, acc[nt]);
            acc[nt] = nd_mfma_bf16(w1, x2, acc[nt]);
            acc[nt] = nd_mfma_bf16(w2, x1, acc[nt]);
            acc[nt] = nd_mfma_bf16(w2, x2, acc[nt]);
            acc[nt] = nd_mfma_bf16(w1, x3, acc[nt]);
            acc[nt] = nd_mfma_bf16(w3, x1, acc[nt]);
            __builtin_amdgcn_sched_barrier(0);
        }
}

template <int N>
__device__ __forceinline__ void chain_act(f32x16 (&acc)[N / 32], const int act) {
    if (act == ND_ACT_NONE) return;
#pragma unroll
    for (int nt = 0; nt < N / 32; ++nt)
#pragma unroll
        for (int r = 0; r < 16; r += 2) {
            if (act == ND_ACT_GELU) {
                const f32x2 g = nd_gelu2(f32x2{acc[nt][r], acc[nt][r + 1]});
                acc[nt][r] = g.x;  acc[nt][r + 1] = g.y;
            } else { acc[nt][r] = nd_silu(acc[nt][r]);  acc[nt][r + 1] = nd_silu(acc[nt][r + 1]); }
        }
}

template <int K0, int N>
__device__ __forceinline__ void chain_res(f32x16 (&acc)[N / 32], const f32x4 (&x)[K0 / 8], const float* vstash, const int res, const int half) {
    if (res == ND_CHAIN_RES_NONE) return;
#pragma unroll
    for (int nt = 0; nt < N / 32; ++nt)
#pragma unroll
        for (int g = 0; g < 4; ++g) {
            const int q = 4 * nt + g;
            if (q < K0 / 8) {
                f32x4 v = x[q];
                if (res == ND_CHAIN_RES_INPUT_RAW && vstash) v -= nd_ld4(vstash + 8 * q + 4 * half);
#pragma unroll
                for (int i = 0; i < 4; ++i) acc[nt][4 * g + i] += v[i];
            }
        }
}

template <int N>
__device__ __forceinline__ void chain_store_buf(const f32x16 (&acc)[N / 32], __amdgpu_buffer_rsrc_t rso, const unsigned row_bytes, const int cout, const int half) {
#pragma unroll
    for (int nt = 0; nt < N / 32; ++nt)
#pragma unroll
        for (int g = 0; g < 4; ++g) {
            const int n0 = 32 * nt + 8 * g + 4 * half;
            const f32x4 v = {acc[nt][4 * g], acc[nt][4 * g + 1], acc[nt][4 * g + 2], acc[nt][4 * g + 3]};
            __builtin_amdgcn_raw_buffer_store_b128(__builtin_bit_cast(u32x4, v), rso, n0 < cout ? row_bytes + n0 * 4u : 0xFFFFFFF0u, 0, 0);
        }
}

template <int N>
__device__ __forceinline__ void chain_store(const f32x16 (&acc)[N / 32], float* row, const int cout, const int half) {
#pragma unroll
    for (int nt = 0; nt < N / 32; ++nt)
#pragma unroll
        for (int g = 0; g < 4; ++g) {
            const int n0 = 32 * nt + 8 * g + 4 * half;
            if (n0 < cout) {
                const f32x4 v = {acc[nt][4 * g], acc[nt][4 * g + 1], acc[nt][4 * g + 2], acc[nt][4 * g + 3]};
                nd_st4(row + n0, v);
            }
        }
}

constexpr int chain_threads(int n1, bool split = false, int k0 = 0) { return split ? (n1 >= 128 || k0 >= 48 ? 512 : 768) : (n1 >= 128 ? 768 : 1024); }

#ifdef CHAIN_STAMP
__device__ unsigned long long chain_dbg[4096 * 16 * 10];
#define CH_T0() (stamp_t = __builtin_amdgcn_s_memtime())
#define CH_ACC(i) { const unsigned long long now_ = __builtin_amdgcn_s_memtime(); stamp[i] += now_ - stamp_t; stamp_t = now_; }
#else
#define CH_T0()
#define CH_ACC(i)
#endif

template <bool SPLIT> constexpr int chain_w_floats(int n, int k) { return SPLIT ? n * k * 3 / 2 : n * k; }

template <int K0, int N1, int N2, int N3, int MODE, bool SPLIT = false>
__global__ __launch_bounds__(chain_threads(N1, SPLIT, K0), 1) void chain_kernel(const ChainArgs a) {
    constexpr int THREADS = chain_threads(N1, SPLIT, K0), WAVES = THREADS / 64;
    static_assert(!SPLIT || K0 % 16 == 0, "SPLIT: the first stage reads whole 16-channel K steps");
    extern __shared__ __attribute__((aligned(16))) float lds[];
    float* w1 = lds;
    float* w2 = w1 + chain_w_floats<SPLIT>(N1, K0);
    float* w3 = w2 + chain_w_floats<SPLIT>(N2, N1);
    float* b1 = w3 + chain_w_floats<SPLIT>(N3, N2);
    float* b2 = b1 + N1;
    float* b3 = b2 + N2;
    float* gam = b3 + (N3 > 0 ? N3 : 0);
    float* bet = gam + K0;
    float* vst = bet + K0;

    const int tid = threadIdx.x, lane = tid & 63, wave = tid >> 6, half = lane >> 5;
    const nd_src& s = a.d.src;
    const int cin = s.c0 + s.c1;

    {
        auto copy4 = [&](float* dst, const float* src, int n) {
            for (int i = tid * 4; i < n; i += THREADS * 4) nd_st4(dst + i, nd_ld4(src + i));
        };
        auto copy_pad = [&](float* dst, const float* src, int n, int npad, float fill) {
            for (int i = tid; i < npad; i += THREADS) dst[i] = (src && i < n) ? src[i] : fill;
        };
        copy4(w1, a.d.st[0].weight, chain_w_floats<SPLIT>(N1, K0));
        copy4(w2, a.d.st[1].weight, chain_w_floats<SPLIT>(N2, N1));
        copy_pad(b1, a.d.st[0].bias, a.d.st[0].cout, N1, 0.0f);
        copy_pad(b2, a.d.st[1].bias, a.d.st[1].cout, N2, 0.0f);
        if (N3 > 0) {
            copy4(w3, a.d.st[2].weight, chain_w_floats<SPLIT>(N3, N2));
            copy_pad(b3, a.d.st[2].bias, a.d.st[2].cout, N3, 0.0f);
        }
        if (MODE == ND_PRO_LAYERNORM) {
            copy_pad(gam, s.gamma, cin, K0, 0.0f);
            copy_pad(bet, s.beta, cin, K0, 0.0f);
        }
    }
    __syncthreads();

    const int n_waves = gridDim.x * WAVES, wid = blockIdx.x * WAVES + wave;
    const int t_begin = (int)((long)wid * a.n_tiles / n_waves), t_end = (int)((long)(wid + 1) * a.n_tiles / n_waves);
    float* myv = vst + wave * K0;
    int b_cur = -1;
    const int cout_last = a.d.st[N3 > 0 ? 2 : 1].cout;

    constexpr bool TWO = SPLIT && K0 == 16;
    constexpr unsigned OOB = 0xFFFFFFF0u;
    const __amdgpu_buffer_rsrc_t rs0 = __builtin_amdgcn_make_buffer_rsrc(const_cast<float*>(s.p0), 0, (int)((unsigned)a.d.B * a.d.HW * s.ld0 * 4u), 0x00020000);
    const __amdgpu_buffer_rsrc_t rs1 = __builtin_amdgcn_make_buffer_rsrc(const_cast<float*>(s.p1 ? s.p1 : s.p0), 0,
                                                                          s.p1 ? (int)((unsigned)a.d.B * a.d.HW * s.ld1 * 4u) : 0, 0x00020000);
    const __amdgpu_buffer_rsrc_t rso = __builtin_amdgcn_make_buffer_rsrc(a.d.out, 0, (int)((unsigned)a.d.B * a.d.HW * a.d.ldo * 4u), 0x00020000);
    f32x4 Xn[SPLIT ? K0 / 8 : 1], Xm[TWO ? K0 / 8 : 1];
    auto prefetch_rows = [&](int t_) {
        const unsigned pix_ = (unsigned)t_ * 32u + (unsigned)(lane & 31);
#pragma unroll
        for (int q = 0; q < K0 / 8; ++q) {
            const int c = 8 * q + 4 * half;
            Xn[SPLIT ? q : 0] = __builtin_bit_cast(f32x4, __builtin_amdgcn_raw_buffer_load_b128(rs0, c < s.c0 ? (pix_ * (unsigned)s.ld0 + c) * 4u : OOB, 0, 0));
            if constexpr (TWO)
                Xm[q] = __builtin_bit_cast(f32x4, __builtin_amdgcn_raw_buffer_load_b128(rs1, (c >= s.c0 && c < cin) ? (pix_ * (unsigned)s.ld1 + (c - s.c0)) * 4u : OOB, 0, 0));
        }
    };
    if constexpr (SPLIT) {
        if (t_begin < t_end) prefetch_rows(t_begin);
    }

#ifdef CHAIN_STAMP
    unsigned long long stamp[8] = {0, 0, 0, 0, 0, 0, 0, 0}, stamp_t = 0;
    const unsigned long long stamp_c0 = __builtin_amdgcn_s_memtime(), stamp_r0 = __builtin_amdgcn_s_memrealtime();
#endif
    for (int t = t_begin; t < t_end; ++t) {
        CH_T0();
        const int b = t / a.tiles_per_sample;
        const size_t pix = (size_t)t * 32 + (lane & 31);
        if (s.vec && b != b_cur) {
            for (int c = lane; c < K0; c += 64) myv[c] = c < cin ? s.vec[(size_t)b * cin + c] : 0.0f;
            b_cur = b;
        }
        f32x4 X[K0 / 8];
        if constexpr (SPLIT) {
#pragma unroll
            for (int q = 0; q < K0 / 8; ++q) {
                X[q] = Xn[q];
                if constexpr (TWO) X[q] += Xm[q];
            }
            prefetch_rows(t + 1 < t_end ? t + 1 : t);
            if (s.vec) {
#pragma unroll
                for (int q = 0; q < K0 / 8; ++q) X[q] += nd_ld4(myv + 8 * q + 4 * half);
            }
        } else {
#pragma unroll
            for (int q = 0; q < K0 / 8; ++q) {
                const int c = 8 * q + 4 * half;
                const f32x4 zero = {0, 0, 0, 0};
                X[q] = zero;
                if (c < s.c0) X[q] = nd_ld4(s.p0 + pix * s.ld0 + c);
                else if (c < cin) X[q] = nd_ld4(s.p1 + pix * s.ld1 + (c - s.c0));
                if (s.vec) X[q] += nd_ld4(myv + c);
            }
        }
        float in0[K0 / 2];
        if (MODE == ND_PRO_LAYERNORM) {
            float sum = 0.0f;
#pragma unroll
            for (int q = 0; q < K0 / 8; ++q) sum += (X[q][0] + X[q][1]) + (X[q][2] + X[q][3]);
            sum += __shfl_xor(sum, 32);
            const float mean = sum / (float)cin;
            float m2 = 0.0f;
#pragma unroll
            for (int q = 0; q < K0 / 8; ++q) {
                if (8 * q + 4 * half < cin) {
#pragma unroll
                    for (int i = 0; i < 4; ++i) { const float dv = X[q][i] - mean; m2 = fmaf(dv, dv, m2); }
                }
            }
            m2 += __shfl_xor(m2, 32);
            const float rstd = rsqrtf(m2 / (float)cin + 1e-5f);
#pragma unroll
            for (int q = 0; q < K0 / 8; ++q) {
                const f32x4 g4 = nd_ld4(gam + 8 * q + 4 * half), be4 = nd_ld4(bet + 8 * q + 4 * half);
#pragma unroll
                for (int i = 0; i < 4; ++i) in0[4 * q + i] = (X[q][i] - mean) * rstd * g4[i] + be4[i];
            }
        } else {
#pragma unroll
            for (int q = 0; q < K0 / 8; ++q)
#pragma unroll
                for (int i = 0; i < 4; ++i) in0[4 * q + i] = X[q][i];
        }

        CH_ACC(0);
        f32x16 H1[N1 / 32];
        if constexpr (SPLIT) chain_gemm_split<K0, N1>(in0, reinterpret_cast<const char*>(w1), b1, H1, lane);
        else chain_gemm<K0, N1>(in0, w1, b1, H1, lane);
        CH_ACC(1);
        chain_res<K0, N1>(H1, X, s.vec ? myv : nullptr, a.d.st[0].res, half);
        chain_act<N1>(H1, a.d.st[0].act);
        CH_ACC(2);
        float in1[N1 / 2];
#pragma unroll
        for (int nt = 0; nt < N1 / 32; ++nt)
#pragma unroll
            for (int r = 0; r < 16; ++r) in1[16 * nt + r] = H1[nt][r];
        f32x16 H2[N2 / 32];
        if constexpr (SPLIT) chain_gemm_split<N1, N2>(in1, reinterpret_cast<const char*>(w2), b2, H2, lane);
        else chain_gemm<N1, N2>(in1, w2, b2, H2, lane);
        CH_ACC(3);
        chain_res<K0, N2>(H2, X, s.vec ? myv : nullptr, a.d.st[1].res, half);
        chain_act<N2>(H2, a.d.st[1].act);
        CH_ACC(4);
        float* row = a.d.out + pix * a.d.ldo;
        if (N3 > 0) {
            float in2[N2 / 2];
#pragma unroll
            for (int nt = 0; nt < N2 / 32; ++nt)
#pragma unroll
                for (int r = 0; r < 16; ++r) in2[16 * nt + r] = H2[nt][r];
            f32x16 H3[(N3 > 0 ? N3 : 32) / 32];
            if constexpr (SPLIT) chain_gemm_split<N2, (N3 > 0 ? N3 : 32)>(in2, reinterpret_cast<const char*>(w3), b3, H3, lane);
            else chain_gemm<N2, (N3 > 0 ? N3 : 32)>(in2, w3, b3, H3, lane);
            CH_ACC(5);
            chain_res<K0, (N3 > 0 ? N3 : 32)>(H3, X, s.vec ? myv : nullptr, a.d.st[2].res, half);
            chain_act<(N3 > 0 ? N3 : 32)>(H3, a.d.st[2].act);
            if constexpr (SPLIT) chain_store_buf<(N3 > 0 ? N3 : 32)>(H3, rso, (unsigned)pix * (unsigned)a.d.ldo * 4u, cout_last, half);
            else chain_store<(N3 > 0 ? N3 : 32)>(H3, row, cout_last, half);
        } else {
            if constexpr (SPLIT) chain_store_buf<N2>(H2, rso, (unsigned)pix * (unsigned)a.d.ldo * 4u, cout_last, half);
            else chain_store<N2>(H2, row, cout_last, half);
        }
        CH_ACC(6);
    }
#ifdef CHAIN_STAMP
    if (lane == 0 && wid < 4096 * 16) {
        unsigned long long* o = chain_dbg + (size_t)wid * 10;
        for (int i = 0; i < 7; ++i) o[i] = stamp[i];
        o[7] = __builtin_amdgcn_s_memtime() - stamp_c0;
        o[8] = __builtin_amdgcn_s_memrealtime() - stamp_r0;
        o[9] = (unsigned long long)(t_end - t_begin);
    }
#endif
}

__global__ void pack_chain_kernel(const float* __restrict__ w, float* __restrict__ out, int cin, int cout, int KP, int NP) {
    const int total = KP * NP;
    for (int idx = blockIdx.x * blockDim.x + threadIdx.x; idx < total; idx += gridDim.x * blockDim.x) {
        const int i = idx & 3, l = (idx >> 2) & 63, rest = idx >> 8;
        const int jq = rest % (KP / 8), nt = rest / (KP / 8);
        const int n = 32 * nt + (l & 31), k = 8 * jq + i + 4 * (l >> 5);
        out[idx] = (n < cout && k < cin) ? w[(size_t)n * cin + k] : 0.0f;
    }
}

__global__ void pack_chain_split_kernel(const float* __restrict__ w, unsigned short* __restrict__ out, int cin, int cout, int KP, int NP) {
    const int total = KP * NP;
    for (int idx = blockIdx.x * blockDim.x + threadIdx.x; idx < total; idx += gridDim.x * blockDim.x) {
        const int i = idx & 7, l = (idx >> 3) & 63, rest = idx >> 9;
        const int s = rest % (KP / 16), nt = rest / (KP / 16);
        const int n = 32 * nt + (l & 31), k = 16 * s + 8 * (i >> 2) + 4 * (l >> 5) + (i & 3);
        const float v = (n < cout && k < cin) ? w[(size_t)n * cin + k] : 0.0f;
        const bf16_terms t = nd_split3_bf16(v);
        unsigned short* o = out + ((size_t)(nt * (KP / 16) + s) * 3 * 64 + l) * 8 + i;
        o[0] = t.t1;  o[512] = t.t2;  o[1024] = t.t3;
    }
}

template <int K0, int N1, int N2, int N3, int MODE, bool SPLIT = false>
int launch(const ChainArgs& a, hipStream_t st) {
    static nd_device_once configured;
    constexpr int THREADS = chain_threads(N1, SPLIT, K0), WAVES = THREADS / 64;
    const size_t lds = (size_t)(chain_w_floats<SPLIT>(N1, K0) + chain_w_floats<SPLIT>(N2, N1) + chain_w_floats<SPLIT>(N3, N2) + N1 + N2 + N3 + 2 * K0 + WAVES * K0) * sizeof(float);
    static_assert((size_t)(chain_w_floats<SPLIT>(N1, K0) + chain_w_floats<SPLIT>(N2, N1) + chain_w_floats<SPLIT>(N3, N2) + N1 + N2 + N3 + 2 * K0 + 16 * K0) * 4 <= 160 * 1024, "LDS");
    if (int e = nd_reserve_lds(configured, reinterpret_cast<const void*>(chain_kernel<K0, N1, N2, N3, MODE, SPLIT>), lds, "nd_pointwise_chain")) return e;
    const int wgs = nd_cdiv(a.n_tiles, WAVES);
    const int grid = wgs < nd_device_cus() ? wgs : nd_device_cus();
    hipLaunchKernelGGL((chain_kernel<K0, N1, N2, N3, MODE, SPLIT>), dim3(grid), dim3(THREADS), lds, st, a);
    return 0;
}

template <int K0, int N1, int N2, int N3, bool SPLIT = false>
int launch_mode(const ChainArgs& a, hipStream_t st) {
    if (a.d.src.mode == ND_PRO_LAYERNORM) return launch<K0, N1, N2, N3, ND_PRO_LAYERNORM, SPLIT>(a, st);
    return launch<K0, N1, N2, N3, ND_PRO_NONE, SPLIT>(a, st);
}

}

extern "C" int64_t nd_pack_chain_weight_floats(int cin, int cout, int first_stage) {
    return (int64_t)nd_round_up(cin, first_stage ? 8 : 32) * nd_round_up(cout, 32);
}

extern "C" int nd_pack_chain_weight(const float* w, float* packed, int cin, int cout, int first_stage, void* stream) {
    ND_REQUIRE(w && packed, ND_E_BADARG, "nd_pack_chain_weight: null pointer");
    ND_REQUIRE(cin > 0 && cout > 0, ND_E_SHAPE, "nd_pack_chain_weight: non-positive size");
    const int KP = nd_round_up(cin, first_stage ? 8 : 32), NP = nd_round_up(cout, 32);
    const int total = KP * NP;
    hipLaunchKernelGGL(pack_chain_kernel, dim3(nd_cdiv(total, 256) < 1024 ? nd_cdiv(total, 256) : 1024), dim3(256), 0, (hipStream_t)stream,
                       w, packed, cin, cout, KP, NP);
    return nd_launch_status("nd_pack_chain_weight");
}

extern "C" int nd_pointwise_chain_supported(int cin, int n1, int n2, int n3) {
    const int K0 = nd_round_up(cin, 8), N1 = nd_round_up(n1, 32), N2 = nd_round_up(n2, 32), N3 = n3 > 0 ? nd_round_up(n3, 32) : 0;
    static const int table[][4] = {{8, 32, 32, 0},  {16, 32, 32, 0}, {16, 32, 32, 32}, {32, 32, 32, 0}, {32, 64, 32, 32},
                                   {8, 64, 64, 0},  {48, 64, 64, 0}, {48, 96, 64, 64}, {64, 64, 64, 0}, {64, 128, 64, 64},
                                   {64, 64, 32, 0}, {32, 32, 32, 32}, {48, 64, 32, 0}};
    for (const auto& e : table)
        if (e[0] == K0 && e[1] == N1 && e[2] == N2 && e[3] == N3) return 1;
    return 0;
}

extern "C" int64_t nd_pack_chain_weight_split_floats(int cin, int cout, int first_stage) {
    return (int64_t)nd_round_up(cin, first_stage ? 16 : 32) * nd_round_up(cout, 32) * 3 / 2;
}

extern "C" int nd_pack_chain_weight_split(const float* w, float* packed, int cin, int cout, int first_stage, void* stream) {
    ND_REQUIRE(w && packed && nd_aligned16(packed), ND_E_BADARG, "nd_pack_chain_weight_split: null or unaligned pointer");
    ND_REQUIRE(cin > 0 && cout > 0, ND_E_SHAPE, "nd_pack_chain_weight_split: non-positive size");
    const int KP = nd_round_up(cin, first_stage ? 16 : 32), NP = nd_round_up(cout, 32);
    const int total = KP * NP;
    hipLaunchKernelGGL(pack_chain_split_kernel, dim3(nd_cdiv(total, 256) < 1024 ? nd_cdiv(total, 256) : 1024), dim3(256), 0, (hipStream_t)stream,
                       w, reinterpret_cast<unsigned short*>(packed), cin, cout, KP, NP);
    return nd_launch_status("nd_pack_chain_weight_split");
}

static int chain_run(const nd_chain* d, void* stream, bool split) {
    ND_REQUIRE(d, ND_E_BADARG, "nd_pointwise_chain: null descriptor");
    const nd_src& s = d->src;
    ND_REQUIRE(d->n_stages == 2 || d->n_stages == 3, ND_E_BADARG, "nd_pointwise_chain: n_stages=%d (2 or 3)", d->n_stages);
    ND_REQUIRE(s.p0 && d->out, ND_E_BADARG, "nd_pointwise_chain: null tensor pointer");
    ND_REQUIRE(d->B > 0 && d->HW > 0 && d->HW % 32 == 0, ND_E_SHAPE, "nd_pointwise_chain: HW=%d must be a positive multiple of 32", d->HW);
    ND_REQUIRE(s.c0 > 0 && s.c0 % 4 == 0 && s.c1 % 4 == 0 && (s.c1 == 0) == (s.p1 == nullptr), ND_E_SHAPE,
               "nd_pointwise_chain: source channels %d+%d (multiples of 4; p1 iff c1)", s.c0, s.c1);
    const int cin = s.c0 + s.c1;
    ND_REQUIRE(s.ld0 >= s.c0 && s.ld0 % 4 == 0 && (s.c1 == 0 || (s.ld1 >= s.c1 && s.ld1 % 4 == 0)), ND_E_ALIGN,
               "nd_pointwise_chain: pixel strides must be >= channels and multiples of 4");
    ND_REQUIRE(s.mode == ND_PRO_NONE || s.mode == ND_PRO_LAYERNORM, ND_E_BADARG, "nd_pointwise_chain: unsupported prologue %d", s.mode);
    ND_REQUIRE(s.mode != ND_PRO_LAYERNORM || (s.gamma && s.beta), ND_E_BADARG, "nd_pointwise_chain: LayerNorm needs gamma and beta");
    ND_REQUIRE(!s.upsample && !s.unshuffle && !s.rowstats, ND_E_BADARG, "nd_pointwise_chain: plain pixel addressing only");
    int width = cin;
    for (int i = 0; i < d->n_stages; ++i) {
        const nd_chain_stage& g = d->st[i];
        ND_REQUIRE(g.weight && g.cin == width && g.cout > 0, ND_E_SHAPE, "nd_pointwise_chain: stage %d is %d->%d, expected input width %d", i,
                   g.cin, g.cout, width);
        ND_REQUIRE(g.res == ND_CHAIN_RES_NONE || g.cout == cin, ND_E_SHAPE, "nd_pointwise_chain: stage %d residual needs cout == input width", i);
        ND_REQUIRE(nd_aligned16(g.weight), ND_E_ALIGN, "nd_pointwise_chain: weights must be 16-byte aligned");
        width = g.cout;
    }
    ND_REQUIRE(width % 4 == 0 && d->ldo >= width && d->ldo % 4 == 0, ND_E_SHAPE, "nd_pointwise_chain: output width %d, ldo %d", width, d->ldo);
    ND_REQUIRE(nd_aligned16(s.p0) && nd_aligned16(s.p1) && nd_aligned16(d->out), ND_E_ALIGN, "nd_pointwise_chain: tensors must be 16-byte aligned");
    const int n3 = d->n_stages == 3 ? d->st[2].cout : 0;
    ND_REQUIRE(nd_pointwise_chain_supported(cin, d->st[0].cout, d->st[1].cout, n3), ND_E_SHAPE,
               "nd_pointwise_chain: widths %d->%d->%d->%d are not instantiated (use nd_pointwise_gemm_nhwc_f32 per layer)", cin,
               d->st[0].cout, d->st[1].cout, n3);
    ChainArgs a;
    a.d = *d;
    a.tiles_per_sample = d->HW / 32;
    const long tiles = (long)d->B * a.tiles_per_sample;
    ND_REQUIRE(tiles < (1L << 31), ND_E_SHAPE, "nd_pointwise_chain: too many pixels");
    a.n_tiles = (int)tiles;
    hipStream_t st = (hipStream_t)stream;
    const int K0 = nd_round_up(cin, split ? 16 : 8), N1 = nd_round_up(d->st[0].cout, 32), N2 = nd_round_up(d->st[1].cout, 32), N3 = n3 ? nd_round_up(n3, 32) : 0;
    int rc = ND_E_SHAPE;
    if (split) {
        ND_REQUIRE(s.c1 == 0 || K0 == 16, ND_E_SHAPE, "nd_pointwise_chain_split: two sources only with cin <= 16 (got %d + %d)", s.c0, s.c1);
        ND_REQUIRE((long)d->B * d->HW * s.ld0 * 4 < (1L << 32) - 65536 && (long)d->B * d->HW * (s.c1 ? s.ld1 : 0) * 4 < (1L << 32) - 65536 &&
                   (long)d->B * d->HW * d->ldo * 4 < (1L << 32) - 65536, ND_E_SHAPE, "nd_pointwise_chain_split: a tensor of 4 GiB or more");
#define ND_CHAIN_SPLIT_CASE(k0, n1, n2, n3) \
        if (K0 == k0 && N1 == n1 && N2 == n2 && N3 == n3) rc = launch_mode<k0, n1, n2, n3, true>(a, st);
        ND_CHAIN_SPLIT_CASE(16, 32, 32, 0)
        ND_CHAIN_SPLIT_CASE(16, 32, 32, 32)
        ND_CHAIN_SPLIT_CASE(32, 32, 32, 0)
        ND_CHAIN_SPLIT_CASE(32, 32, 32, 32)
        ND_CHAIN_SPLIT_CASE(32, 64, 32, 32)
        ND_CHAIN_SPLIT_CASE(16, 64, 64, 0)
        ND_CHAIN_SPLIT_CASE(48, 64, 64, 0)
        ND_CHAIN_SPLIT_CASE(48, 96, 64, 64)
        ND_CHAIN_SPLIT_CASE(64, 64, 64, 0)
        ND_CHAIN_SPLIT_CASE(64, 64, 32, 0)
        ND_CHAIN_SPLIT_CASE(48, 64, 32, 0)
        ND_CHAIN_SPLIT_CASE(64, 128, 64, 64)
#undef ND_CHAIN_SPLIT_CASE
        if (rc) return rc;
        return nd_launch_status("nd_pointwise_chain_split_nhwc_f32");
    }
#define ND_CHAIN_CASE(k0, n1, n2, n3) \
    if (K0 == k0 && N1 == n1 && N2 == n2 && N3 == n3) rc = launch_mode<k0, n1, n2, n3>(a, st);
    ND_CHAIN_CASE(8, 32, 32, 0)
    ND_CHAIN_CASE(16, 32, 32, 0)
    ND_CHAIN_CASE(16, 32, 32, 32)
    ND_CHAIN_CASE(32, 32, 32, 0)
    ND_CHAIN_CASE(32, 32, 32, 32)
    ND_CHAIN_CASE(32, 64, 32, 32)
    ND_CHAIN_CASE(8, 64, 64, 0)
    ND_CHAIN_CASE(48, 64, 64, 0)
    ND_CHAIN_CASE(48, 96, 64, 64)
    ND_CHAIN_CASE(64, 64, 64, 0)
    ND_CHAIN_CASE(64, 64, 32, 0)
    ND_CHAIN_CASE(48, 64, 32, 0)
    ND_CHAIN_CASE(64, 128, 64, 64)
#undef ND_CHAIN_CASE
    if (rc) return rc;
    return nd_launch_status("nd_pointwise_chain_nhwc_f32");
}

#ifdef CHAIN_STAMP
extern "C" int nd_chain_debug_read(unsigned long long* host, int n_words) {
    return (int)hipMemcpyFromSymbol(host, HIP_SYMBOL(chain_dbg), (size_t)n_words * 8);
}
#endif

extern "C" int nd_pointwise_chain_nhwc_f32(const nd_chain* d, void* stream) { return chain_run(d, stream, false); }

extern "C" int nd_pointwise_chain_split_nhwc_f32(const nd_chain* d, void* stream) { return chain_run(d, stream, true); }
```

### noisediff_amd/engine.py

```python
from __future__ import annotations

import ctypes as C
import logging
import math
import os
import threading
from dataclasses import dataclass
from typing import Callable, Dict, List, Optional, Sequence, Tuple

import torch

from . import _lib as L
from .spec import (normalize_stage_attn, stage_attention_param_spec, ATTN_DIM_HEAD, ATTN_HEADS, ISO_DIM, ISO_TABLE_ROWS, POS_DIM, POS_GROUPS, RESNET_GROUPS, SHOT_GROUPS,
                   arch_param_spec, arch_traits, attention_param_spec, stage_dims)

GN_EPS = 1e-5
_log = logging.getLogger("noisediff_amd")
WINOGRAD = os.environ.get("ND_WINOGRAD", "1") != "0"
PREACT = True
PREACT_MIN = 256
CHAIN = True
_CHAIN_FIRST = (".ff.net.0.0.weight", ".fc1.weight")
_CHAIN_LATER = (".ff.net.2.weight", ".proj_out.weight", ".fc2.weight")
WINO2 = os.environ.get("ND_WINO2", "1") != "0"
MAP_BLOCKED = True
GENMAP = os.environ.get("ND_GENMAP", "1") != "0"
COND_STEP = True
WINO4 = os.environ.get("ND_WINO4", "1") != "0"
SPLIT_K = os.environ.get("ND_SPLIT_K", "0") != "0"
EIGHT_TILES_RULE = True
WINO4_16 = os.environ.get("ND_WINO4_16", "narrow")
WINO4_16_SPLIT = True
_ALIGN = 64
_SPLIT = os.environ.get("ND_SPLIT_GEMM", "1")
SPLIT_GEMM = _SPLIT != "0"
SPLIT_CHAIN, SPLIT_PW = _SPLIT in ("1", "chain"), _SPLIT in ("1", "pw")
TIME_TABLE = True
PROJ_TABLE = True
TIME_TABLE_ROWS = 1000


def _few_items(H: int, W: int, cout: int) -> bool:
    return ((H + 15) // 16) * ((W + 31) // 32) * ((cout + 63) // 64) <= 8


def _wino4_layer(cin: int, cout: int) -> bool:
    return cin > 16 and cin % 4 == 0 and cout % 4 == 0


_MAP_PRODUCERS = ("pos_block1.mlp.1.weight", "pos_block2.mlp.1.weight")


def _blocked_map_rows(C_: int) -> torch.Tensor:
    i = torch.arange(2 * C_)
    c, j = i // 32, i % 32
    return torch.where(j < 16, 16 * c + j, C_ + 16 * c + j - 16)


_CHAIN_SPLIT_LIMIT = (1 << 32) - (1 << 17)


def _split_layer(cin: int, cout: int) -> bool:
    return SPLIT_PW and cin % 32 == 0 and cin >= 64 and cout % 128 == 0


def _classify(name: str, shape: Sequence[int]) -> str:
    if ".attn.to_q." in name or ".attn.to_k." in name or ".norm1." in name:
        return "skip"
    if len(shape) == 4:
        k = shape[-1]
        if name == "pos_enc.weights.weight" or name.endswith(".g"):
            return "raw"
        if k == 7:
            return "conv7"
        if k == 3:
            return "conv3"
        if name.startswith("downs.") and name.endswith((".3.1.weight", ".2.1.weight")):
            return "pw_unshuffle"
        return "pw"
    if len(shape) == 2 and (".ff.net." in name):
        return "pw"
    return "raw"


@dataclass
class Slot:
    offset: int
    numel: int
    kind: str
    shape: Tuple[int, ...]


class Engine:

    def __init__(self, dim: int, device: torch.device, mid_attn: bool = False, inp_dim: int = 4, arch: str = "NoiseDiffNet", stage_attn=None):
        if device.type != "cuda":
            raise L.HipError("noisediff_amd runs on MI355X only: got device %r (there is no CPU path)" % (device,))
        self.lib = L.load()
        self.dim, self.device, self.mid_attn, self.inp_dim = dim, device, mid_attn, inp_dim
        self.arch, self.traits = arch, arch_traits(arch)
        self.spec = list(arch_param_spec(arch, dim, inp_dim))
        if mid_attn:
            self.spec += attention_param_spec("mid_attn", 8 * dim)
        self.stage_attn = normalize_stage_attn(stage_attn)
        if self.stage_attn:
            self.spec += stage_attention_param_spec(dim, self.stage_attn)
        self.resnet_names = [p.name[:-len(".mlp.1.weight")] for p in self.spec
                             if p.name.endswith(".mlp.1.weight") and len(p.shape) == 2]
        self.tproj_off: Dict[str, int] = {}
        self._layout()
        with torch.inference_mode(False):
            self.arena = torch.empty(self.arena_floats, dtype=torch.float32, device=device)
        with torch.cuda.device(device):
            s = C.c_void_p()
            L.call("nd_stream_create", C.byref(s))
        self.stream = s
        self.plans: Dict[Tuple[int, int, int], "Plan"] = {}
        self.loaded = False
        self.used: set = set()
        self.valid: Optional[set] = None

    def __del__(self):
        s, self.stream = getattr(self, "stream", None), None
        for q in (s,):
            if q:
                try:
                    L.call("nd_stream_sync", q)
                    L.call("nd_stream_destroy", q)
                except Exception:
                    pass

    def _layout(self) -> None:
        self.slots: Dict[str, Slot] = {}
        off = 0

        def add(name, numel, kind, shape):
            nonlocal off
            self.slots[name] = Slot(off, int(numel), kind, tuple(shape))
            off += (int(numel) + _ALIGN - 1) // _ALIGN * _ALIGN

        for p in self.spec:
            kind = _classify(p.name, p.shape)
            if kind == "skip":
                continue
            if kind == "conv3":
                n = self.lib.nd_pack_conv3x3_weight_floats(p.shape[1], p.shape[0])
                add(p.name + ".wino", self.lib.nd_pack_conv3x3_wino_weight_floats(p.shape[1], p.shape[0]), "derived", p.shape)
                if WINO4 and _wino4_layer(p.shape[1], p.shape[0]):
                    add(p.name + ".wino4", self.lib.nd_pack_conv3x3_wino4_weight_floats(p.shape[1], p.shape[0]), "derived", p.shape)
            elif kind in ("pw", "pw_unshuffle"):
                n = self.lib.nd_pack_pointwise_weight_floats(p.shape[1], p.shape[0])
                if p.name in _MAP_PRODUCERS and p.shape[0] % 32 == 0:
                    add(p.name + ".blk16", n, "derived", p.shape)
                    add(p.name[:-len("weight")] + "bias.blk16", p.shape[0], "derived", (p.shape[0],))
                    if GENMAP and p.shape[1] == POS_DIM == 8 and p.shape[0] % 32 == 0:
                        add(p.name + ".gen", p.shape[0] * p.shape[1], "derived", p.shape)
                if kind == "pw" and p.name.endswith(_CHAIN_FIRST + _CHAIN_LATER):
                    first = int(p.name.endswith(_CHAIN_FIRST))
                    add(p.name + ".chain", self.lib.nd_pack_chain_weight_floats(p.shape[1], p.shape[0], first), "derived", p.shape)
                    if SPLIT_CHAIN:
                        add(p.name + ".chain_s", self.lib.nd_pack_chain_weight_split_floats(p.shape[1], p.shape[0], first), "derived", p.shape)
                if kind == "pw" and _split_layer(p.shape[1], p.shape[0]):
                    add(p.name + ".split", self.lib.nd_pack_pointwise_weight_split_floats(p.shape[1], p.shape[0]), "derived", p.shape)
            elif kind == "conv7":
                n = 196 * p.shape[0]
                if SPLIT_PW and p.name == "init_conv.weight":
                    add(p.name + ".split", self.lib.nd_pack_conv7x7_weight_split_floats(p.shape[0]), "derived", p.shape)
            else:
                n = math.prod(p.shape)
            add(p.name, n, kind, p.shape)
        j = 0
        for r in self.resnet_names:
            self.tproj_off[r] = j
            j += self.slots[r + ".mlp.1.weight"].shape[0]
        self.tproj_rows = j
        add("tproj.weight", j * 4 * self.dim, "derived", (j, 4 * self.dim))
        add("tproj.bias", j, "derived", (j,))
        add("time_freqs", self.dim // 2, "derived", (self.dim // 2,))
        self.time_table = TIME_TABLE and 4 * self.dim <= 2048 and self.lib.nd_cond_step_lds_bytes(16, self.dim) <= 160 * 1024
        if self.time_table:
            add("time_table", TIME_TABLE_ROWS * 4 * self.dim, "derived", (TIME_TABLE_ROWS, 4 * self.dim))
            if PROJ_TABLE and self.tproj_rows % 4 == 0 and TIME_TABLE_ROWS * self.tproj_rows * 4 <= (192 << 20):
                add("tproj_table", TIME_TABLE_ROWS * self.tproj_rows, "derived", (TIME_TABLE_ROWS, self.tproj_rows))
        self.arena_floats = off

    def view(self, name: str) -> torch.Tensor:
        s = self.slots[name]
        return self.arena[s.offset:s.offset + s.numel]

    def p(self, name: str) -> int:
        s = self.slots[name]
        if self.valid is not None and name not in self.valid:
            raise L.HipError(f"arena slice {name!r} was not part of this rank's weight broadcast (it carried the slices of the plans "
                             "recorded before it): record the plan before Engine.broadcast(only_used=True), or broadcast the whole arena")
        self.used.add(name)
        return self.arena.data_ptr() + 4 * s.offset

    def load_state_dict(self, sd: Dict[str, torch.Tensor]) -> None:
        st = self.stream
        self.valid = None
        keep = []
        used = set(self.used)
        with torch.cuda.device(self.device):
            for p in self.spec:
                if p.name not in self.slots:
                    continue
                t = sd[p.name].detach().to(device=self.device, dtype=torch.float32).contiguous()
                if tuple(t.shape) != tuple(p.shape):
                    raise ValueError(f"{p.name}: shape {tuple(t.shape)} != {tuple(p.shape)}")
                keep.append(t)
                kind = self.slots[p.name].kind
                if kind == "raw":
                    self.view(p.name).copy_(t.reshape(-1))
            torch.cuda.synchronize(self.device)
            for p, t in zip([q for q in self.spec if q.name in self.slots], keep):
                kind, dst = self.slots[p.name].kind, self.p(p.name)
                if kind == "conv3":
                    L.call("nd_pack_conv3x3_weight", t.data_ptr(), dst, p.shape[1], p.shape[0], st)
                    L.call("nd_pack_conv3x3_wino_weight", t.data_ptr(), self.p(p.name + ".wino"), p.shape[1], p.shape[0], st)
                    if p.name + ".wino4" in self.slots:
                        L.call("nd_pack_conv3x3_wino4_weight", t.data_ptr(), self.p(p.name + ".wino4"), p.shape[1], p.shape[0], st)
                elif kind == "pw":
                    L.call("nd_pack_pointwise_weight", t.data_ptr(), dst, p.shape[1], p.shape[0], 0, st)
                    if p.name + ".blk16" in self.slots:
                        perm = _blocked_map_rows(p.shape[0] // 2).to(self.device)
                        tp = t[perm].contiguous()
                        keep.append(tp)
                        L.call("nd_pack_pointwise_weight", tp.data_ptr(), self.p(p.name + ".blk16"), p.shape[1], p.shape[0], 0, st)
                        bname = p.name[:-len("weight")] + "bias"
                        self.view(bname + ".blk16").copy_(sd[bname].detach().to(device=self.device, dtype=torch.float32)[perm])
                    if p.name + ".gen" in self.slots:
                        self.view(p.name + ".gen").copy_(t.reshape(-1))
                    if p.name + ".chain" in self.slots:
                        L.call("nd_pack_chain_weight", t.data_ptr(), self.p(p.name + ".chain"), p.shape[1], p.shape[0],
                               int(p.name.endswith(_CHAIN_FIRST)), st)
                    if p.name + ".chain_s" in self.slots:
                        L.call("nd_pack_chain_weight_split", t.data_ptr(), self.p(p.name + ".chain_s"), p.shape[1], p.shape[0],
                               int(p.name.endswith(_CHAIN_FIRST)), st)
                    if p.name + ".split" in self.slots:
                        L.call("nd_pack_pointwise_weight_split", t.data_ptr(), self.p(p.name + ".split"), p.shape[1], p.shape[0], st)
                elif kind == "pw_unshuffle":
                    L.call("nd_pack_pointwise_weight", t.data_ptr(), dst, p.shape[1], p.shape[0], p.shape[1] // 4, st)
                elif kind == "conv7":
                    L.call("nd_pack_conv7x7_weight", t.data_ptr(), dst, p.shape[0], st)
                    if p.name + ".split" in self.slots:
                        L.call("nd_pack_conv7x7_weight_split", t.data_ptr(), self.p(p.name + ".split"), p.shape[0], st)
            L.call("nd_stream_sync", st)
            tw = torch.cat([self.view(r + ".mlp.1.weight") for r in self.resnet_names])
            tb = torch.cat([self.view(r + ".mlp.1.bias") for r in self.resnet_names])
            self.view("tproj.weight").copy_(tw)
            self.view("tproj.bias").copy_(tb)
            half = self.dim // 2
            e = math.log(10000) / (half - 1)
            self.view("time_freqs").copy_(torch.exp(torch.arange(half) * -e).to(torch.float32))
            torch.cuda.synchronize(self.device)
            self._build_time_tables()
        self.loaded, self.valid, self.used = True, None, used

    _DERIVED_TABLES = ("time_table", "tproj_table")

    def _build_time_tables(self) -> None:
        if not self.time_table:
            return
        st, used = self.stream, set(self.used)
        with torch.cuda.device(self.device):
            L.call("nd_cond_table_build_f32", self.p("time_freqs"), self.p("time_mlp.1.weight"), self.p("time_mlp.1.bias"), self.p("time_mlp.3.weight"),
                   self.p("time_mlp.3.bias"), self.p("time_table"), TIME_TABLE_ROWS, self.dim, st)
            L.call("nd_stream_sync", st)
            if "tproj_table" in self.slots:
                ts = torch.arange(TIME_TABLE_ROWS, dtype=torch.int64, device=self.device)
                torch.cuda.synchronize(self.device)
                J = self.tproj_rows
                for t0 in range(0, TIME_TABLE_ROWS, 16):
                    nb = min(16, TIME_TABLE_ROWS - t0)
                    L.call("nd_cond_step_table_f32", ts.data_ptr() + 8 * t0, self.p("time_freqs"), self.p("time_mlp.1.weight"), self.p("time_mlp.1.bias"),
                           self.p("time_mlp.3.weight"), self.p("time_mlp.3.bias"), self.p("tproj.weight"), self.p("tproj.bias"),
                           self.p("tproj_table") + 4 * t0 * J, J, nb, self.dim, J, self.p("time_table"), TIME_TABLE_ROWS, st)
                L.call("nd_stream_sync", st)
        self.used = used

    def broadcast_state_dict(self, sd: Optional[Dict[str, torch.Tensor]], src: int = 0, group=None) -> int:
        import torch.distributed as dist
        names = [p for p in self.spec if p.name in self.slots]
        total = sum(math.prod(p.shape) for p in names)
        with torch.cuda.device(self.device), torch.inference_mode(False):
            if dist.get_rank(group) == src:
                flat = torch.cat([sd[p.name].detach().reshape(-1).to(torch.float32) for p in names]).to(self.device)
                if flat.numel() != total:
                    raise ValueError("broadcast_state_dict: the state dict does not match the network's parameter spec")
            else:
                flat = torch.empty(total, dtype=torch.float32, device=self.device)
            torch.cuda.synchronize(self.device)
            dist.broadcast(flat, src=src, group=group)
            torch.cuda.synchronize(self.device)
            views, at = {}, 0
            for p in names:
                n = math.prod(p.shape)
                views[p.name] = flat[at:at + n].view(*p.shape)
                at += n
        self.load_state_dict(views)
        return total * 4

    def broadcast(self, src: int = 0, group=None, only_used: bool = False) -> int:
        import torch.distributed as dist
        with torch.cuda.device(self.device):
            torch.cuda.synchronize(self.device)
            if not only_used:
                dist.broadcast(self.arena, src=src, group=group)
                nbytes = self.arena.numel() * 4
            else:
                tables = [n for n in self._DERIVED_TABLES if n in self.used]
                if tables:
                    for dep in ("time_freqs", "time_mlp.1.weight", "time_mlp.1.bias", "time_mlp.3.weight", "time_mlp.3.bias", "tproj.weight", "tproj.bias"):
                        self.used.add(dep)
                names = sorted((n for n in self.used if n not in self._DERIVED_TABLES), key=lambda n: self.slots[n].offset)
                every = [None] * dist.get_world_size(group)
                dist.all_gather_object(every, names, group=group)
                if any(e != names for e in every):
                    raise L.HipError("Engine.broadcast(only_used=True): the ranks recorded different plans")
                ranges: List[List[int]] = []
                for n in names:
                    sl = self.slots[n]
                    lo, hi = sl.offset, sl.offset + (sl.numel + _ALIGN - 1) // _ALIGN * _ALIGN
                    if ranges and ranges[-1][1] == lo:
                        ranges[-1][1] = hi
                    else:
                        ranges.append([lo, hi])
                is_src = dist.get_rank(group) == src
                with torch.inference_mode(False):
                    stage = (torch.cat([self.arena[lo:hi] for lo, hi in ranges]) if is_src
                             else torch.empty(sum(hi - lo for lo, hi in ranges), dtype=torch.float32, device=self.device))
                dist.broadcast(stage, src=src, group=group)
                if not is_src:
                    at = 0
                    for lo, hi in ranges:
                        self.arena[lo:hi].copy_(stage[at:at + hi - lo])
                        at += hi - lo
                    self.valid = set(names) | set(tables)
                    if tables:
                        torch.cuda.synchronize(self.device)
                        self._build_time_tables()
                nbytes = stage.numel() * 4
            torch.cuda.synchronize(self.device)
        self.loaded = True
        return nbytes

    def copy_from(self, other: "Engine") -> None:
        if other.arena_floats != self.arena_floats or not other.loaded:
            raise L.HipError("Engine.copy_from: the source engine has no weights or another layout")
        other.sync()
        torch.cuda.synchronize(other.device)
        with torch.cuda.device(self.device):
            self.arena.copy_(other.arena)
            torch.cuda.synchronize(self.device)
        self.loaded, self.valid = True, other.valid

    def plan(self, B: int, H: int, W: int, debug: bool = False, tag: int = 0, allow_empty: bool = False) -> "Plan":
        if not self.loaded and not allow_empty:
            raise L.HipError("Engine has no weights: call load_state_dict() or broadcast() first")
        key = (B, H, W, debug, tag)
        if key not in self.plans:
            self.plans[key] = Plan(self, B, H, W, debug)
        return self.plans[key]

    def sync(self) -> None:
        L.call("nd_stream_sync", self.stream)


Op = Tuple[Callable, tuple]


class Plan:

    def __init__(self, eng: Engine, B: int, H: int, W: int, debug: bool = False):
        self.debug, self.taps = debug, {}
        self.lock = threading.Lock()
        if H % 8 or W % 8:
            raise AssertionError(f"your input dimensions {(H, W)} need to be divisible by 8, given the unet")
        self.e, self.B, self.H, self.W = eng, B, H, W
        self.dev = eng.device
        self._keep: List[object] = []
        self._free: Dict[int, List[torch.Tensor]] = {}
        self.workspace_floats = 0
        d = eng.dim
        with torch.cuda.device(self.dev), torch.inference_mode(False):
            f = lambda *s: torch.empty(*s, dtype=torch.float32, device=self.dev)
            self.x = f(B, H, W, eng.inp_dim)
            self.clean = f(B, H, W, eng.inp_dim)
            self.position = f(B, 2, H, W)
            self.iso_idx = torch.zeros(B, dtype=torch.int64, device=self.dev)
            self.time = torch.zeros(B, dtype=torch.int64, device=self.dev)
            self.model_out = f(B, H, W, eng.inp_dim)
            self.nchw_tmp = f(B, eng.inp_dim, H, W)
            self.pos_emb = f(B, H, W, POS_DIM)
            self.posgen = (GENMAP and eng.traits.position and all(b + ".mlp.1.weight.gen" in eng.slots for b in ("pos_block1", "pos_block2")) and d % 16 == 0 and
                           self._wino4_kind("pos_block1.block2.proj", L.PRO_AFFINE_GENMAP_SILU, False, d, 0, d, 0, d, d, H, W,
                                            self._conv_rows(H, W, 0, d, 0, d, d, L.PRO_AFFINE_GENMAP_SILU)) == "wino4")
            self.posmap1 = self.posmap2 = None
            if self.posgen:
                self.pos_e = f(B, H, W, POS_DIM)
                self.pos_e_mad = torch.tensor([0.0, 1.0, 0.0], device=self.dev).repeat_interleave(POS_DIM).repeat(B).view(B, 3, POS_DIM).contiguous()
            else:
                self.posmap1 = f(B, H, W, 2 * d)
                self.posmap2 = f(B, H, W, 2 * d)
            self.posmap_blocked = (not self.posgen and MAP_BLOCKED and "pos_block1.mlp.1.weight.blk16" in eng.slots and
                                   self._wino4_takes("pos_block1.block2.proj", L.PRO_AFFINE_MAP_SILU, False, d, 0, d, 0, d, d, H, W))
            self.iso_emb = f(B, ISO_DIM)
            self.attn_names = [p.name[:-len(".attn.to_v.weight")] for p in eng.spec if p.name.endswith(".attn.to_v.weight")]
            self.cb = {n: f(B, eng.slots[n + ".proj_out.bias"].shape[0]) for n in self.attn_names}
            self.emb = f(B, d)
            self.t1 = f(B, 4 * d)
            self.st = f(B, 4 * d)
            self.tproj = f(B, eng.tproj_rows)
        self.cond_ops: List[Op] = []
        self.step_ops: List[Op] = []
        self._ops = self.cond_ops
        self._record_condition()
        self._ops = self.step_ops
        self._record_time()
        self._record_net()
        self.condition_set = False

    def _alloc(self, *shape) -> torch.Tensor:
        n = math.prod(shape)
        lst = self._free.get(n)
        if lst:
            return lst.pop().view(*shape)
        self.workspace_floats += n
        with torch.cuda.device(self.dev), torch.inference_mode(False):
            t = torch.empty(n, dtype=torch.float32, device=self.dev)
        self._keep.append(t)
        return t.view(*shape)

    def _tap(self, name: str, t: torch.Tensor) -> torch.Tensor:
        if self.debug:
            self.taps[name] = t
        return t

    def _release(self, *ts: torch.Tensor) -> None:
        if self.debug:
            return
        for t in ts:
            self._free.setdefault(t.numel(), []).append(t.reshape(-1))

    def _add(self, name: str, *args, meta: Optional[dict] = None) -> None:
        fn = getattr(self.e.lib, name)
        self._keep.append(args)
        self._ops.append((fn, args, name, meta))

    def _src(self, t: torch.Tensor, t2: Optional[torch.Tensor] = None, mode=L.PRO_NONE, **kw) -> L.Src:
        s = L.Src()
        s.p0, s.c0, s.ld0 = t.data_ptr(), t.shape[-1], t.shape[-1]
        if t2 is not None:
            s.p1, s.c1, s.ld1 = t2.data_ptr(), t2.shape[-1], t2.shape[-1]
        s.mode = mode
        for k, v in kw.items():
            setattr(s, k, v.data_ptr() if isinstance(v, torch.Tensor) else v)
        return s

    def _conv_rows(self, H: int, W: int, up: int, ld0: int, ld1: int, cin: int, cout: int, mode: int, splits: int = 1) -> int:
        sh, sw, lim = H >> up, W >> up, (1 << 30) - (1 << 16)

        def fits(b: int) -> bool:
            px = b * sh * sw + sw + 2
            return (px * 4 * max(ld0, ld1) < lim and px < (1 << 24) and b * H * W < (1 << 24) and b * H * W * cout * 4 < (1 << 32) - (1 << 16)
                    and (mode != L.PRO_AFFINE_MAP_SILU or (b * H + 2) * W * 8 * cin < lim) and splits * b * H * W * cout * 4 < (1 << 31))
        if fits(self.B):
            return self.B
        lo, hi = 1, self.B
        while lo < hi:
            mid = (lo + hi + 1) // 2
            lo, hi = (mid, hi) if fits(mid) else (lo, mid - 1)
        if not fits(lo):
            raise L.HipError(f"conv3x3 at {H} x {W} x {max(ld0, ld1)}: one sample exceeds the kernels' 1 GiB source limit")
        pieces = -(-self.B // lo)
        return -(-self.B // pieces)

    def conv3(self, name: str, src: L.Src, cin: int, cout: int, H: int, W: int, stats: bool):
        e = self.e
        out = self._alloc(self.B, H, W, cout)
        wino = WINOGRAD and H >= 16 and W >= 16
        up = 1 if src.upsample else 0
        rows = self._conv_rows(H, W, up, src.ld0, src.ld1, cin, cout, src.mode) if wino else self.B
        wino2 = (wino and WINO2 and not (src.mode == L.PRO_AFFINE_MAP_SILU and src.upsample)
                 and (src.c1 == 0 or src.c0 % 32 == 0) and rows * H * W < (1 << 24)
                 and rows * H * W * 4 * max(src.ld0, src.ld1, 2 * cin if src.mode == L.PRO_AFFINE_MAP_SILU else 0) < (1 << 31))
        w4kind = self._wino4_kind(name, src.mode, bool(src.upsample), src.c0, src.c1, src.ld0, src.ld1, cin, cout, H, W, rows) if wino else ""
        wino4 = bool(w4kind)
        if src.mode == L.PRO_AFFINE_GENMAP_SILU and w4kind != "wino4":
            raise L.HipError(f"{name}: maps formed in the kernel need conv3x3_wino4's 16 x 32-region form (Plan.posgen decides by the same rule)")
        if wino and not wino4 and (name + ".weight.wino4") in e.slots and src.mode in (L.PRO_NONE, L.PRO_AFFINE_SILU, L.PRO_AFFINE_MAP_SILU) and not _few_items(H, W, cout):
            _log.warning("%s (%d -> %d at %d x %d, batch %d): not on the F(4x4) kernel", name, cin, cout, H, W, self.B)
        st = sc = None
        slots = 0
        if stats:
            slots = (e.lib.nd_conv3x3_wino4_stat_slots(H, W) if wino4 else e.lib.nd_conv3x3_wino_stat_slots(H, W) if wino
                     else e.lib.nd_conv3x3_stat_slots(H, W, cout, self.B))
            st = self._alloc(self.B, slots, cout, 2)
            sc = self._alloc(slots)
        if src.map_blocked and not wino4:
            raise L.HipError(f"{name}: the scale / shift map was produced in the blocked layout but the layer does not run on conv3x3_wino4")
        lowlat_split = SPLIT_K and w4kind == "wino4" and src.mode in (L.PRO_NONE, L.PRO_AFFINE_SILU) and int(e.lib.nd_conv3x3_wino4_splitk_plan(self.B, H, W, cin, cout)) > 1
        weight = e.p(name + (".weight.wino4" if wino4 else ".weight.wino" if wino else ".weight"))
        entry = (f"nd_conv3x3_{w4kind}_nhwc_f32" if wino4 else "nd_conv3x3_wino2_nhwc_f32" if wino2 else
                 "nd_conv3x3_wino_nhwc_f32" if wino else "nd_conv3x3_nhwc_f32")
        tiling = (9016 if w4kind == "wino4_16" else 9004) if wino4 else 9002 if wino2 else 9001 if wino else e.lib.nd_conv3x3_tiling_id(self.B, H, W, cout)
        splits = int(e.lib.nd_conv3x3_wino4_splitk_plan(self.B, H, W, cin, cout)) if lowlat_split else 1
        if w4kind == "wino4_16" and WINO4_16_SPLIT:
            splits = int(e.lib.nd_conv3x3_wino4_16_splitk_plan(H, W, cin, cout))
        if splits > 1:
            rows = self._conv_rows(H, W, up, src.ld0, src.ld1, cin, cout, src.mode, splits)
        ws = self._alloc(splits * rows * H * W * cout) if splits > 1 else None
        sh, sw, ctot = H >> up, W >> up, src.c0 + src.c1
        for b0 in range(0, self.B, rows):
            nb = min(rows, self.B - b0)
            d = L.Conv3x3()
            s = L.Src.from_buffer_copy(src)
            if b0:
                s.p0 = src.p0 + 4 * b0 * sh * sw * src.ld0
                if src.p1:
                    s.p1 = src.p1 + 4 * b0 * sh * sw * src.ld1
                if src.mad:
                    s.mad = src.mad + 4 * b0 * 3 * ctot
                if src.map:
                    s.map = src.map + 4 * b0 * H * W * (POS_DIM if src.mode == L.PRO_AFFINE_GENMAP_SILU else 2 * ctot)
            d.src, d.weight, d.bias, d.out = s, weight, e.p(name + ".bias"), out.data_ptr() + 4 * b0 * H * W * cout
            d.B, d.H, d.W, d.cin, d.cout, d.ldo = nb, H, W, cin, cout, cout
            if stats:
                d.stats, d.slot_count = st.data_ptr() + 4 * b0 * slots * cout * 2, sc.data_ptr()
            meta = {"layer": name, "B": nb, "H": H, "W": W, "cin": cin, "cout": cout, "mode": int(src.mode), "tiling": tiling}
            if splits > 1:
                meta["splits"] = splits
                entry_s = "nd_conv3x3_wino4_16_splitk_nhwc_f32" if w4kind == "wino4_16" else "nd_conv3x3_wino4_splitk_nhwc_f32"
                self._add(entry_s, C.byref(d), ws.data_ptr(), splits, e.stream, meta=meta)
            else:
                self._add(entry, C.byref(d), e.stream, meta=meta)
            self._keep.append(d)
        if ws is not None:
            self._release(ws)
        return out, st, sc, slots

    def _wino4_kind(self, name: str, mode: int, upsample: bool, c0: int, c1: int, ld0: int, ld1: int, cin: int, cout: int, H: int, W: int, rows: Optional[int] = None) -> str:
        up = 1 if upsample else 0
        rows = self.B if rows is None else rows
        src_px = rows * (H >> up) * (W >> up) + (W >> up) + 2
        src_bytes = src_px * 4 * max(ld0, ld1)
        common = (WINOGRAD and WINO4 and H >= 16 and W >= 16 and cout <= 2048 and (name + ".weight.wino4") in self.e.slots
                  and W <= 2048 and (c1 == 0 or (c0 % 16 == 0 and not up)) and src_bytes < (1 << 30) - (1 << 16) and src_px < (1 << 24)
                  and (not up or (H % 2 == 0 and W % 2 == 0)))
        if not common:
            return ""
        takes16 = WINO4_16 != "0" and mode in (L.PRO_NONE, L.PRO_AFFINE_SILU) and (W % 16 == 0 or W >= 48)
        few = _few_items(H, W, cout)
        if takes16 and (WINO4_16 == "all" or W < 32 or (few and EIGHT_TILES_RULE and not SPLIT_K)):
            return "wino4_16"
        return "wino4" if self._wino4_takes(name, mode, upsample, c0, c1, ld0, ld1, cin, cout, H, W, rows) else ""

    def _wino4_takes(self, name: str, mode: int, upsample: bool, c0: int, c1: int, ld0: int, ld1: int, cin: int, cout: int, H: int, W: int, rows: Optional[int] = None) -> bool:
        up = 1 if upsample else 0
        if (WINO2 and not SPLIT_K and EIGHT_TILES_RULE and ((H + 15) // 16) * ((W + 31) // 32) * ((cout + 63) // 64) <= 8 and (c1 == 0 or c0 % 32 == 0)
                and not (mode == L.PRO_AFFINE_MAP_SILU and up)):
            return False
        rows = self.B if rows is None else rows
        src_px = rows * (H >> up) * (W >> up) + (W >> up) + 2
        src_bytes = src_px * 4 * max(ld0, ld1)
        return (WINOGRAD and WINO4 and H >= 16 and W >= 16 and cout <= 2048 and (name + ".weight.wino4") in self.e.slots
                and mode in (L.PRO_NONE, L.PRO_AFFINE_SILU, L.PRO_AFFINE_MAP_SILU, L.PRO_AFFINE_GENMAP_SILU)
                and not (mode == L.PRO_AFFINE_MAP_SILU and (up or (rows * H + 2) * W * 8 * cin >= (1 << 30) - (1 << 16)))
                and not (mode == L.PRO_AFFINE_GENMAP_SILU and (up or c1 or cin % 16))
                and W >= 32 and (W % 32 == 0 or W >= 96) and W <= 2048 and (c1 == 0 or (c0 % 16 == 0 and not up))
                and src_bytes < (1 << 30) - (1 << 16) and src_px < (1 << 24)
                and (not up or (H % 2 == 0 and W % 2 == 0)))

    def pw(self, name: str, src: L.Src, cin: int, cout: int, HW: int, W: int, act=L.ACT_NONE, bias=True,
           res0=None, res1=None, vec=None, gn_t=None, gn_mad=None, out=None, variant: str = "") -> torch.Tensor:
        e = self.e
        if out is None:
            out = self._alloc(self.B, HW, cout)
        d = L.Pointwise()
        d.src, d.out = src, out.data_ptr()
        d.bias = e.p(name + ".bias" + variant) if bias else None
        d.B, d.HW, d.W, d.cin, d.cout, d.ldo, d.act = self.B, HW, W, cin, cout, cout, act
        split = not variant and (name + ".weight.split") in e.slots and bool(e.lib.nd_pointwise_gemm_split_takes(C.byref(d)))
        d.weight = e.p(name + (".weight.split" if split else ".weight" + variant))
        if res0 is not None:
            d.res0, d.ldr0 = res0.data_ptr(), res0.shape[-1]
        if res1 is not None:
            d.res1, d.ldr1 = res1.data_ptr(), res1.shape[-1]
        if vec is not None:
            d.vec = vec.data_ptr()
        if gn_t is not None:
            d.gn_t, d.ldt, d.gn_mad = gn_t.data_ptr(), gn_t.shape[-1], gn_mad.data_ptr()
        self._add("nd_pointwise_gemm_split_nhwc_f32" if split else "nd_pointwise_gemm_nhwc_f32", C.byref(d), e.stream,
                  meta={"layer": name, "B": self.B, "HW": HW, "cin": cin, "cout": cout, "split": int(split)})
        self._keep.append(d)
        return out

    def gn_finalize(self, st, sc, slots: int, norm: str, C_: int, groups: int, ss_off: Optional[int]) -> torch.Tensor:
        e = self.e
        mad = self._alloc(self.B, 3, C_)
        ss = (self.tproj.data_ptr() + 4 * ss_off) if ss_off is not None else None
        self._add("nd_groupnorm_finalize_f32", st.data_ptr(), sc.data_ptr(), slots, e.p(norm + ".weight"), e.p(norm + ".bias"),
                  ss, e.tproj_rows, mad.data_ptr(), self.B, C_, groups, GN_EPS, e.stream)
        return mad

    def linear_rows(self, x: torch.Tensor, w: int, b: Optional[int], out: torch.Tensor, K: int, N: int, act_in=0, act_out=0):
        self._add("nd_linear_rows_f32", x.data_ptr(), x.shape[-1], w, b, out.data_ptr(), out.shape[-1], self.B, K, N,
                  act_in, act_out, self.e.stream)

    def resnet(self, name: str, x: torch.Tensor, skip: Optional[torch.Tensor], cout: int, H: int, W: int, groups: int,
               posmap: Optional[torch.Tensor] = None, extra_res: Optional[torch.Tensor] = None) -> torch.Tensor:
        cin = x.shape[-1] + (skip.shape[-1] if skip is not None else 0)
        HW = H * W
        c1, st1, sc1, n1 = self.conv3(name + ".block1.proj", self._src(x, skip), cin, cout, H, W, stats=True)
        ss_off = None if posmap is not None else self.e.tproj_off.get(name)
        mad1 = self.gn_finalize(st1, sc1, n1, name + ".block1.norm", cout, groups, ss_off)
        a1 = None
        if PREACT and posmap is None and cout >= PREACT_MIN and H >= 16 and W >= 16:
            a1 = self._alloc(self.B, HW, cout)
            self._add("nd_affine_silu_add_f32", c1.data_ptr(), cout, mad1.data_ptr(), None, cout, None, cout, a1.data_ptr(), cout,
                      self.B, HW, cout, self.e.stream,
                      meta={"layer": name + ".block1.act", "stream_bytes": 4.0 * self.B * HW * cout * 2})
            src2 = self._src(a1)
        else:
            if posmap is not None and self.posgen:
                src2 = self._src(c1, None, L.PRO_AFFINE_GENMAP_SILU, mad=mad1, map=self.pos_e, gamma=self.e.p(name + ".mlp.1.weight.gen"),
                                 beta=self.e.p(name + ".mlp.1.bias"))
            else:
                mode = L.PRO_AFFINE_MAP_SILU if posmap is not None else L.PRO_AFFINE_SILU
                src2 = self._src(c1, None, mode, mad=mad1, **({"map": posmap, "map_blocked": int(self.posmap_blocked)} if posmap is not None else {}))
        c2, st2, sc2, n2 = self.conv3(name + ".block2.proj", src2, cout, cout, H, W, stats=True)
        if a1 is not None:
            self._release(a1)
        mad2 = self.gn_finalize(st2, sc2, n2, name + ".block2.norm", cout, groups, None)
        if cin != cout:
            assert extra_res is None
            out = self.pw(name + ".res_conv", self._src(x, skip), cin, cout, HW, W, gn_t=c2, gn_mad=mad2)
        else:
            assert skip is None
            out = self._alloc(self.B, HW, cout)
            self._add("nd_affine_silu_add_f32", c2.data_ptr(), cout, mad2.data_ptr(), x.data_ptr(), cout,
                      extra_res.data_ptr() if extra_res is not None else None, cout, out.data_ptr(), cout,
                      self.B, HW, cout, self.e.stream,
                      meta={"layer": name + ".tail", "stream_bytes": 4.0 * self.B * HW * cout * (4 if extra_res is not None else 3)})
        self._release(c1, st1, sc1, mad1, c2, st2, sc2, mad2)
        return out.view(self.B, H, W, cout)

    def chain(self, name: str, src: L.Src, stages, HW: int) -> torch.Tensor:
        e = self.e
        out = self._alloc(self.B, HW, stages[-1][2])
        split = all((layer + ".weight.chain_s") in e.slots for layer, *_ in stages) and (src.c1 == 0 or stages[0][1] <= 16)
        ldo = stages[-1][2]
        rows = self.B
        if split:
            per = 4 * HW * max(src.ld0, src.ld1, ldo)
            rows = max(1, min(self.B, _CHAIN_SPLIT_LIMIT // per))
            rows = -(-self.B // -(-self.B // rows))
        for b0 in range(0, self.B, rows):
            nb = min(rows, self.B - b0)
            d = L.Chain()
            sp = L.Src.from_buffer_copy(src)
            if b0:
                sp.p0 = src.p0 + 4 * b0 * HW * src.ld0
                if src.p1:
                    sp.p1 = src.p1 + 4 * b0 * HW * src.ld1
                if src.vec:
                    sp.vec = src.vec + 4 * b0 * (src.c0 + src.c1)
            d.src, d.out, d.n_stages, d.B, d.HW, d.ldo = sp, out.data_ptr() + 4 * b0 * HW * ldo, len(stages), nb, HW, ldo
            for i, (layer, cin, cout, act, res) in enumerate(stages):
                d.st[i].weight, d.st[i].bias = e.p(layer + (".weight.chain_s" if split else ".weight.chain")), e.p(layer + ".bias")
                d.st[i].cin, d.st[i].cout, d.st[i].act, d.st[i].res = cin, cout, act, res
            self._add("nd_pointwise_chain_split_nhwc_f32" if split else "nd_pointwise_chain_nhwc_f32", C.byref(d), e.stream,
                      meta={"layer": name, "B": nb, "HW": HW, "cin": stages[0][1], "cout": stages[-1][2], "split": int(split),
                            "flop_per_px": 2.0 * sum(c_in * c_out for _, c_in, c_out, _, _ in stages)})
            self._keep.append(d)
        return out

    def _chain_ok(self, HW: int, widths) -> bool:
        w = list(widths) + [0] * (4 - len(widths))
        return CHAIN and HW % 32 == 0 and bool(self.e.lib.nd_pointwise_chain_supported(*w))

    def attn_block(self, name: str, x: torch.Tensor, H: int, W: int) -> torch.Tensor:
        Cc, HW = x.shape[-1], H * W
        cb = self.cb[name]
        if self._chain_ok(HW, (Cc, 2 * Cc, Cc, Cc)):
            ln = self._src(x, None, L.PRO_LAYERNORM, vec=cb, gamma=self.e.p(name + ".norm2.weight"), beta=self.e.p(name + ".norm2.bias"))
            y = self.chain(name + ".ff+proj_out", ln,
                           [(name + ".ff.net.0.0", Cc, 2 * Cc, L.ACT_GELU, L.CHAIN_RES_NONE),
                            (name + ".ff.net.2", 2 * Cc, Cc, L.ACT_NONE, L.CHAIN_RES_INPUT),
                            (name + ".proj_out", Cc, Cc, L.ACT_NONE, L.CHAIN_RES_INPUT_RAW)], HW)
            return y.view(self.B, H, W, Cc)
        kw = {}
        rs = None
        if Cc > 64:
            rs = self._alloc(self.B, HW, 2)
            self._add("nd_layernorm_stats_f32", x.data_ptr(), Cc, cb.data_ptr(), rs.data_ptr(), self.B, HW, Cc, 1e-5, self.e.stream)
            kw["rowstats"] = rs
        ln = self._src(x, None, L.PRO_LAYERNORM, vec=cb, gamma=self.e.p(name + ".norm2.weight"), beta=self.e.p(name + ".norm2.bias"), **kw)
        h1 = self.pw(name + ".ff.net.0.0", ln, Cc, 2 * Cc, HW, W, act=L.ACT_GELU)
        x2 = self.pw(name + ".ff.net.2", self._src(h1), 2 * Cc, Cc, HW, W, res0=x, vec=cb)
        y = self.pw(name + ".proj_out", self._src(x2), Cc, Cc, HW, W, res0=x)
        self._release(h1, x2)
        if rs is not None:
            self._release(rs)
        return y.view(self.B, H, W, Cc)

    def mlp(self, name: str, src: L.Src, cin: int, hid: int, cout: int, H: int, W: int, res0=None) -> torch.Tensor:
        if res0 is None and src.mode == L.PRO_NONE and self._chain_ok(H * W, (cin, hid, cout)):
            o = self.chain(name, src, [(name + ".fc1", cin, hid, L.ACT_GELU, L.CHAIN_RES_NONE),
                                       (name + ".fc2", hid, cout, L.ACT_NONE, L.CHAIN_RES_NONE)], H * W)
            return o.view(self.B, H, W, cout)
        h = self.pw(name + ".fc1", src, cin, hid, H * W, W, act=L.ACT_GELU)
        o = self.pw(name + ".fc2", self._src(h), hid, cout, H * W, W, res0=res0)
        self._release(h)
        return o.view(self.B, H, W, cout)

    def _record_condition(self) -> None:
        e, B, H, W, st = self.e, self.B, self.H, self.W, self.e.stream
        tr = e.traits
        if tr.position:
            pe = self._alloc(B, H, W, 3 * POS_DIM)
            self._add("nd_pos_enc_f32", self.position.data_ptr(), e.p("pos_enc.weights.weight"), e.p("pos_enc.weights.bias"),
                      pe.data_ptr(), B, H, W, POS_DIM, st)
            h = self.pw("pos_mlp.fc1", self._src(pe), 3 * POS_DIM, 2 * POS_DIM, H * W, W, act=L.ACT_GELU)
            self.pw("pos_mlp.fc2", self._src(h), 2 * POS_DIM, POS_DIM, H * W, W, out=self.pos_emb)
            if self.posgen:
                self._add("nd_affine_silu_add_f32", self.pos_emb.data_ptr(), POS_DIM, self.pos_e_mad.data_ptr(), None, POS_DIM, None, POS_DIM,
                          self.pos_e.data_ptr(), POS_DIM, B, H * W, POS_DIM, st, meta={"layer": "pos_emb.silu", "stream_bytes": 8.0 * B * H * W * POS_DIM})
            for blk, dst in (() if self.posgen else (("pos_block1", self.posmap1), ("pos_block2", self.posmap2))):
                self.pw(blk + ".mlp.1", self._src(self.pos_emb, None, L.PRO_SILU), POS_DIM, 2 * e.dim, H * W, W, out=dst,
                        variant=".blk16" if self.posmap_blocked else "")
            self._release(pe, h)
        if tr.iso_attn:
            self._add("nd_embedding_rows_f32", self.iso_idx.data_ptr(), e.p("iso_embed.weight"), self.iso_emb.data_ptr(), B,
                      ISO_TABLE_ROWS, ISO_DIM, st)
            inner = ATTN_HEADS * ATTN_DIM_HEAD
            v = self._alloc(B, inner)
            for n in self.attn_names:
                Cc = self.cb[n].shape[-1]
                self.linear_rows(self.iso_emb, e.p(n + ".attn.to_v.weight"), None, v, ISO_DIM, inner)
                self.linear_rows(v, e.p(n + ".attn.to_out.0.weight"), e.p(n + ".attn.to_out.0.bias"), self.cb[n], inner, Cc)
            self._release(v)
        self.clean_emb = None
        if tr.cond_branch:
            ce = self._alloc(B, H, W, e.dim)
            self._add("nd_conv7x7_c4_f32", self.clean.data_ptr(), e.p("cond_init_conv.weight"), e.p("cond_init_conv.bias"),
                      ce.data_ptr(), e.dim, B, H, W, e.dim, st)
            self.clean_emb = self._tap("clean_emb", self.resnet("cond_res_block1", ce, None, e.dim, H, W, RESNET_GROUPS))
            self._release(ce)

    def _record_time(self) -> None:
        e, d = self.e, self.e.dim
        if COND_STEP and 4 * d <= 2048 and e.lib.nd_cond_step_lds_bytes(self.B, d) <= 160 * 1024:
            args = (self.time.data_ptr(), e.p("time_freqs"), e.p("time_mlp.1.weight"), e.p("time_mlp.1.bias"),
                    e.p("time_mlp.3.weight"), e.p("time_mlp.3.bias"), e.p("tproj.weight"), e.p("tproj.bias"), self.tproj.data_ptr(),
                    e.tproj_rows, self.B, d, e.tproj_rows)
            if e.time_table and "tproj_table" in e.slots and e.tproj_rows % 4 == 0:
                self._add("nd_cond_step_ptable_f32", *args, e.p("time_table"), TIME_TABLE_ROWS, e.p("tproj_table"), e.stream)
            elif e.time_table:
                self._add("nd_cond_step_table_f32", *args, e.p("time_table"), TIME_TABLE_ROWS, e.stream)
            else:
                self._add("nd_cond_step_f32", *args, e.stream)
            return
        self._add("nd_sinusoidal_time_emb_f32", self.time.data_ptr(), e.p("time_freqs"), self.emb.data_ptr(), self.B, d // 2, e.stream)
        self.linear_rows(self.emb, e.p("time_mlp.1.weight"), e.p("time_mlp.1.bias"), self.t1, d, 4 * d, act_out=L.ACT_GELU)
        self.linear_rows(self.t1, e.p("time_mlp.3.weight"), e.p("time_mlp.3.bias"), self.st, 4 * d, 4 * d, act_out=L.ACT_SILU)
        self.linear_rows(self.st, e.p("tproj.weight"), e.p("tproj.bias"), self.tproj, 4 * d, e.tproj_rows)

    def _record_net(self) -> None:
        e, B, H, W, d = self.e, self.B, self.H, self.W, self.e.dim
        G, tr = RESNET_GROUPS, self.e.traits
        shot_noise = None
        if tr.shot_branch:
            r_shot = self.mlp("shot_mlp1", self._src(self.clean, self.x), 2 * e.inp_dim, d, d, H, W)
            s = self.attn_block("shot_attn", r_shot, H, W)
            s2 = self.mlp("shot_mlp2", self._src(s), d, d, d, H, W)
            s3 = self.resnet("shot_time", s2, None, d, H, W, SHOT_GROUPS, extra_res=r_shot)
            shot_noise = self._tap("shot_noise", self.mlp("shot_mlp3", self._src(s3), d, d, e.inp_dim, H, W))
            for nm, tt in (("shot_mlp1", r_shot), ("shot_attn", s), ("shot_mlp2", s2), ("shot_time", s3)):
                self._tap(nm, tt)
            self._release(r_shot, s, s2, s3)
        x0 = self._alloc(B, H, W, d)
        stem_split = "init_conv.weight.split" in e.slots
        self._add("nd_conv7x7_c4_split_f32" if stem_split else "nd_conv7x7_c4_f32", self.x.data_ptr(),
                  e.p("init_conv.weight.split" if stem_split else "init_conv.weight"), e.p("init_conv.bias"), x0.data_ptr(), d, B, H, W, d, e.stream)
        self._tap("init_conv", x0)
        xin = x0
        if tr.cond_branch:
            xin, *_ = self.conv3("cond_concat_conv", self._src(x0, self.clean_emb), 2 * d, d, H, W, stats=False)
            self._tap("cond_concat", xin)
        pm1, pm2 = ((self.pos_e, self.pos_e) if self.posgen else (self.posmap1, self.posmap2)) if tr.position else (None, None)
        x = self._tap("pos_block1", self.resnet("pos_block1", xin, None, d, H, W, POS_GROUPS, posmap=pm1))
        if xin is not x0:
            self._release(xin)
        rs = 3 if tr.iso_attn else 2
        hs: List[torch.Tensor] = []
        h, w = H, W
        for i, (cin, cout) in enumerate(stage_dims(d)):
            p = f"downs.{i}"
            x1 = self.resnet(p + ".0", x, None, cin, h, w, G)
            self._release(x)
            x2 = self.resnet(p + ".1", x1, None, cin, h, w, G)
            if e.stage_attn and e.stage_attn[i]:
                x2 = self._stage_attention(f"down_attns.{i}", e.stage_attn[i], x2, h, w)
            hs += [x1, x2]
            xa = self.attn_block(p + ".2", x2, h, w) if tr.iso_attn else x2
            self._tap(p + ".0", x1); self._tap(p + ".1", x2); self._tap(p + ".2", xa)
            if i == 3:
                x, *_ = self.conv3(f"{p}.{rs}", self._src(xa), cin, cout, h, w, stats=False)
            else:
                h, w = h // 2, w // 2
                x = self.pw(f"{p}.{rs}.1", self._src(xa, None, L.PRO_NONE, unshuffle=1, c0=4 * cin, ld0=cin), 4 * cin, cout,
                            h * w, w).view(B, h, w, cout)
            if xa is not x2:
                self._release(xa)
            self._tap(f"down{i}", x)
        mid = x.shape[-1]
        xm = self.resnet("mid_block1", x, None, mid, h, w, G)
        self._release(x)
        if e.mid_attn:
            xm = self._mid_attention(xm, h, w)
        x = self._tap("mid", self.resnet("mid_block2", xm, None, mid, h, w, G))
        self._release(xm)
        for i, (cin, cout) in enumerate(reversed(stage_dims(d))):
            p = f"ups.{i}"
            sk = hs.pop()
            x1 = self.resnet(p + ".0", x, sk, cout, h, w, G)
            self._release(x, sk)
            sk = hs.pop()
            x2 = self.resnet(p + ".1", x1, sk, cout, h, w, G)
            self._release(x1, sk)
            if e.stage_attn and e.stage_attn[3 - i]:
                x2 = self._stage_attention(f"up_attns.{i}", e.stage_attn[3 - i], x2, h, w)
            xa = self.attn_block(p + ".2", x2, h, w) if tr.iso_attn else x2
            if xa is not x2:
                self._release(x2)
            if i == 3:
                x, *_ = self.conv3(f"{p}.{rs}", self._src(xa), cout, cin, h, w, stats=False)
            else:
                h, w = h * 2, w * 2
                x, *_ = self.conv3(f"{p}.{rs}.1", self._src(xa, None, L.PRO_NONE, upsample=1), cout, cin, h, w, stats=False)
            self._release(xa)
            self._tap(p + ".0", x1); self._tap(p + ".1", x2); self._tap(p + ".2", xa); self._tap(f"up{i}", x)
        xp = self._tap("pos_block2", self.resnet("pos_block2", x, None, d, H, W, POS_GROUPS, posmap=pm2))
        self._release(x)
        xf = self._tap("final_res_block", self.resnet("final_res_block", xp, x0, d, H, W, G))
        self._release(xp, x0)
        self.pw("final_conv", self._src(xf), d, e.inp_dim, H * W, W, res0=shot_noise, out=self.model_out)
        self._release(xf)
        if shot_noise is not None:
            self._release(shot_noise)

    def _mid_attention(self, x: torch.Tensor, h: int, w: int, prefix: str = "mid_attn") -> torch.Tensor:
        e, B, Cc, N = self.e, self.B, x.shape[-1], h * w
        hid = ATTN_HEADS * ATTN_DIM_HEAD
        xn = self._alloc(B, N, Cc)
        self._add("nd_rmsnorm_nhwc_f32", x.data_ptr(), Cc, e.p(prefix + ".norm.g"), xn.data_ptr(), Cc, B, N, Cc, e.stream)
        qkv = self.pw(prefix + ".to_qkv", self._src(xn), Cc, 3 * hid, N, w, bias=False)
        att = self._alloc(B, N, hid)
        self._add("nd_attention_mfma_f32", qkv.data_ptr(), 3 * hid, att.data_ptr(), hid, B, N, ATTN_HEADS, ATTN_DIM_HEAD, e.stream)
        y = self.pw(prefix + ".to_out", self._src(att), hid, Cc, N, w, res0=x)
        self._release(xn, qkv, att, x)
        return y.view(B, h, w, Cc)

    def _stage_attention(self, prefix: str, kind: str, x: torch.Tensor, h: int, w: int) -> torch.Tensor:
        if kind == "full":
            return self._mid_attention(x, h, w, prefix)
        e, B, Cc, N = self.e, self.B, x.shape[-1], h * w
        hid = ATTN_HEADS * ATTN_DIM_HEAD
        xn = self._alloc(B, N, Cc)
        self._add("nd_rmsnorm_nhwc_f32", x.data_ptr(), Cc, e.p(prefix + ".norm.g"), xn.data_ptr(), Cc, B, N, Cc, e.stream)
        qkv = self.pw(prefix + ".to_qkv", self._src(xn), Cc, 3 * hid, N, w, bias=False)
        att = self._alloc(B, N, hid)
        ws = self._alloc(int(e.lib.nd_linear_attention_workspace_floats(B, N, ATTN_HEADS)))
        self._add("nd_linear_attention_f32", qkv.data_ptr(), 3 * hid, att.data_ptr(), hid, ws.data_ptr(), B, N, ATTN_HEADS, ATTN_DIM_HEAD, e.stream)
        o = self.pw(prefix + ".to_out.0", self._src(att), hid, Cc, N, w)
        y = self._alloc(B, N, Cc)
        self._add("nd_rmsnorm_add_nhwc_f32", o.data_ptr(), Cc, e.p(prefix + ".to_out.1.g"), x.data_ptr(), Cc, y.data_ptr(), Cc, B, N, Cc, e.stream)
        self._release(xn, qkv, att, ws, o, x)
        return y.view(B, h, w, Cc)

    @staticmethod
    def run(ops: List[Op]) -> None:
        for fn, args, name, _meta in ops:
            r = fn(*args)
            if r != 0:
                L.check(r, name)

    def set_condition(self, condition) -> None:
        B, H, W, e = self.B, self.H, self.W, self.e
        tr = e.traits
        if torch.is_tensor(condition):
            if tr.position or tr.iso_attn:
                raise TypeError(f"{e.arch} needs the condition dict (clean_img, position, iso_ratio_idx), got a tensor")
            condition = {"clean_img": condition}
        clean = condition["clean_img"]
        if tuple(clean.shape) != (B, e.inp_dim, H, W):
            raise ValueError(f"condition shapes: clean_img {tuple(clean.shape)} do not match batch {(B, e.inp_dim, H, W)}")
        with torch.cuda.device(self.dev):
            self.nchw_tmp.copy_(clean.to(self.dev, torch.float32))
            if tr.position:
                pos = condition["position"]
                if tuple(pos.shape) != (B, 2, H, W):
                    raise ValueError(f"condition shapes: position {tuple(pos.shape)} do not match batch {(B, 2, H, W)}")
                self.position.copy_(pos.to(self.dev, torch.float32))
            if tr.iso_attn:
                iso = condition["iso_ratio_idx"]
                if tuple(iso.shape) != (B,):
                    raise ValueError(f"condition shapes: iso_ratio_idx {tuple(iso.shape)} do not match batch {(B,)}")
                iso = iso.to(torch.int64)
                if int(iso.min()) < 0 or int(iso.max()) >= ISO_TABLE_ROWS:
                    raise IndexError("iso_ratio_idx out of range for nn.Embedding(100, 16)")
                self.iso_idx.copy_(iso.to(self.dev))
            torch.cuda.synchronize(self.dev)
            L.call("nd_nchw_to_nhwc_f32", self.nchw_tmp.data_ptr(), self.clean.data_ptr(), B, e.inp_dim, H, W, e.stream)
            self.run(self.cond_ops)
            e.sync()
        self.condition_set = True

    def load_x(self, x_nchw: torch.Tensor) -> None:
        e = self.e
        with torch.cuda.device(self.dev):
            self.nchw_tmp.copy_(x_nchw.to(self.dev, torch.float32))
            torch.cuda.synchronize(self.dev)
            L.call("nd_nchw_to_nhwc_f32", self.nchw_tmp.data_ptr(), self.x.data_ptr(), self.B, e.inp_dim, self.H, self.W, e.stream)

    def read_nchw(self, nhwc: torch.Tensor) -> torch.Tensor:
        e = self.e
        with torch.cuda.device(self.dev), torch.inference_mode(False):
            out = torch.empty(self.B, e.inp_dim, self.H, self.W, dtype=torch.float32, device=self.dev)
            L.call("nd_nhwc_to_nchw_f32", nhwc.data_ptr(), out.data_ptr(), self.B, e.inp_dim, self.H, self.W, e.stream)
            e.sync()
        return out

    def forward(self, x_nchw: torch.Tensor, time: torch.Tensor) -> torch.Tensor:
        if not self.condition_set:
            raise L.HipError("Plan.forward: set_condition() first")
        with torch.cuda.device(self.dev):
            self.time.copy_(time.to(self.dev, torch.int64))
        self.load_x(x_nchw)
        self.run(self.step_ops)
        return self.read_nchw(self.model_out)
```

Before: 0.9456 patches/s.

## Fold final res_conv into final_conv and fuse shot_time tail into shot_mlp3 chain

```diff
diff --git a/include/noisediff_hip.h b/include/noisediff_hip.h
--- a/include/noisediff_hip.h
+++ b/include/noisediff_hip.h
@@ -246,6 +246,20 @@
 int64_t nd_pack_pointwise_weight_split_floats(int cin, int cout);
 int nd_pack_pointwise_weight_split(const float* w, float* packed, int cin, int cout, void* stream);
 
+typedef struct nd_narrow_fold {
+    const float* p0; const float* p1;
+    const float* t;  const float* mad;
+    const float* weight; const float* bias;
+    const float* res0;
+    float*   out;
+    int32_t  B, HW, c0, c1, c2, ld0, ld1, ldt, cout, ldo, ldr0, reserved;
+} nd_narrow_fold;
+int nd_pointwise_narrow_fold_nhwc_f32(const nd_narrow_fold* d, void* stream);
+int nd_pointwise_narrow_fold_takes(int c0, int c1, int c2, int cout);
+int64_t nd_pack_narrow_fold_floats(int cin, int cout);
+int nd_pack_narrow_fold(const float* wf, const float* bf, const float* wr, const float* br, float* w_out, float* b_out, int cin_r, int mid, int cout,
+                        void* stream);
+
 enum nd_chain_res { ND_CHAIN_RES_NONE = 0, ND_CHAIN_RES_INPUT = 1 , ND_CHAIN_RES_INPUT_RAW = 2  };
 typedef struct nd_chain_stage {
     const float* weight;
@@ -267,6 +281,15 @@
 int nd_pointwise_chain_split_nhwc_f32(const nd_chain* d, void* stream);
 int64_t nd_pack_chain_weight_split_floats(int cin, int cout, int first_stage);
 int nd_pack_chain_weight_split(const float* w, float* packed, int cin, int cout, int first_stage, void* stream);
+typedef struct nd_chain_tail {
+    nd_chain chain;
+    const float* mad;
+    const float* r0;
+    const float* r1;
+    int32_t  ldr0, ldr1;
+} nd_chain_tail;
+int nd_pointwise_chain_tail_split_nhwc_f32(const nd_chain_tail* d, void* stream);
+int nd_pointwise_chain_tail_takes(int cin, int n1, int n2, int n3);
 
 
 int nd_groupnorm_finalize_f32(const float* stats, const float* slot_count, int slots,
diff --git a/noisediff_amd/_lib.py b/noisediff_amd/_lib.py
--- a/noisediff_amd/_lib.py
+++ b/noisediff_amd/_lib.py
@@ -57,6 +57,16 @@
 class Chain(C.Structure):
     _fields_ = [("src", Src), ("st", ChainStage * 3), ("out", fptr), ("n_stages", C.c_int32), ("B", C.c_int32), ("HW", C.c_int32),
                 ("ldo", C.c_int32)]
+
+
+class ChainTail(C.Structure):
+    _fields_ = [("chain", Chain), ("mad", fptr), ("r0", fptr), ("r1", fptr), ("ldr0", C.c_int32), ("ldr1", C.c_int32)]
+
+
+class NarrowFold(C.Structure):
+    _fields_ = [("p0", fptr), ("p1", fptr), ("t", fptr), ("mad", fptr), ("weight", fptr), ("bias", fptr), ("res0", fptr), ("out", fptr),
+                ("B", C.c_int32), ("HW", C.c_int32), ("c0", C.c_int32), ("c1", C.c_int32), ("c2", C.c_int32), ("ld0", C.c_int32), ("ld1", C.c_int32),
+                ("ldt", C.c_int32), ("cout", C.c_int32), ("ldo", C.c_int32), ("ldr0", C.c_int32), ("reserved", C.c_int32)]
 
 
 class RawSample(C.Structure):
@@ -141,6 +151,12 @@
     "nd_pointwise_gemm_split_takes": (i32, [C.POINTER(Pointwise)]),
     "nd_pack_pointwise_weight_split_floats": (i64, [i32, i32]),
     "nd_pack_pointwise_weight_split": (i32, [vp, vp, i32, i32, vp]),
+    "nd_pointwise_chain_tail_split_nhwc_f32": (i32, [C.POINTER(ChainTail), vp]),
+    "nd_pointwise_chain_tail_takes": (i32, [i32, i32, i32, i32]),
+    "nd_pointwise_narrow_fold_nhwc_f32": (i32, [C.POINTER(NarrowFold), vp]),
+    "nd_pointwise_narrow_fold_takes": (i32, [i32, i32, i32, i32]),
+    "nd_pack_narrow_fold_floats": (i64, [i32, i32]),
+    "nd_pack_narrow_fold": (i32, [vp, vp, vp, vp, vp, vp, i32, i32, i32, vp]),
     "nd_pack_pointwise_weight_floats": (i64, [i32, i32]),
     "nd_pack_pointwise_weight": (i32, [vp, vp, i32, i32, i32, vp]),
     "nd_pack_pointwise_weight_t": (i32, [vp, vp, i32, i32, vp]),
@@ -255,7 +271,7 @@
     "nd_raw_diffusion_batch_f32": (i32, [vp, i32, i32, i32, vp, f32, f32, vp, vp, vp, vp, i32, i32, i32, vp]),
 }
 
-_UNCHECKED = {"nd_version", "nd_last_error", "nd_stream_device", "nd_conv3x3_wgrad_form", "nd_adam_chunk_elements", "nd_ema_chunk_elements", "nd_conv7x7_c4_wgrad_workspace_floats", "nd_conv3x3_stat_slots", "nd_conv3x3_tiling_id", "nd_pack_conv3x3_weight_floats",
+_UNCHECKED = {"nd_pointwise_chain_tail_takes", "nd_pointwise_narrow_fold_takes", "nd_pack_narrow_fold_floats", "nd_version", "nd_last_error", "nd_stream_device", "nd_conv3x3_wgrad_form", "nd_adam_chunk_elements", "nd_ema_chunk_elements", "nd_conv7x7_c4_wgrad_workspace_floats", "nd_conv3x3_stat_slots", "nd_conv3x3_tiling_id", "nd_pack_conv3x3_weight_floats",
               "nd_pack_pointwise_weight_floats", "nd_linear_attention_workspace_floats", "nd_conv3x3_wino_stat_slots", "nd_conv3x3_wino4_stat_slots",
               "nd_pack_conv3x3_wino_weight_floats", "nd_pack_conv3x3_wino4_weight_floats", "nd_conv3x3_wino4_splitk_plan", "nd_conv3x3_wino4_16_splitk_plan", "nd_conv3x3_wino4_splitk_workspace_floats", "nd_token_sum_workspace_floats", "nd_cond_step_lds_bytes", "nd_conv3x3_wgrad_workspace_floats",
               "nd_groupnorm_train_workspace_floats", "nd_linear_wgrad_workspace_floats",
diff --git a/noisediff_amd/csrc/pointwise.hip b/noisediff_amd/csrc/pointwise.hip
--- a/noisediff_amd/csrc/pointwise.hip
+++ b/noisediff_amd/csrc/pointwise.hip
@@ -856,6 +856,116 @@
     }
 }
 
+template <int CO>
+__device__ __forceinline__ void nf_fma(float (&acc)[CO], const f32x4 x, const float* wq) {
+#pragma unroll
+    for (int n = 0; n < CO; ++n) {
+        const f32x4 w = nd_ld4(wq + n * 4);
+        acc[n] = fmaf(x.w, w.w, fmaf(x.z, w.z, fmaf(x.y, w.y, fmaf(x.x, w.x, acc[n]))));
+    }
+}
+
+template <int CO>
+__global__ __launch_bounds__(256) void pointwise_narrow_fold_kernel(const nd_narrow_fold d) {
+    extern __shared__ __attribute__((aligned(16))) float wl[];
+    const int tid = threadIdx.x, part = tid & 3;
+    const int nq0 = d.c0 >> 2, nq1 = d.c1 >> 2, nq2 = d.c2 >> 2;
+    for (int i = tid; i < (nq0 + nq1 + nq2) * CO; i += 256) nd_st4(wl + i * 4, nd_ld4(d.weight + (size_t)i * 4));
+    __syncthreads();
+    const long P = (long)d.B * d.HW;
+    for (long base = (long)blockIdx.x * 128; base < P; base += (long)gridDim.x * 128) {
+        long pix[2], pc[2];
+        float acc[2][CO];
+#pragma unroll
+        for (int j = 0; j < 2; ++j) {
+            pix[j] = base + 64 * j + (tid >> 2);
+            pc[j] = pix[j] < P ? pix[j] : P - 1;
+#pragma unroll
+            for (int n = 0; n < CO; ++n) acc[j][n] = 0.0f;
+        }
+        {
+            const float* ra = d.p0 + pc[0] * d.ld0;
+            const float* rb = d.p0 + pc[1] * d.ld0;
+#pragma unroll 4
+            for (int q = part; q < nq0; q += 4) {
+                const f32x4 xa = nd_ld4(ra + 4 * q), xb = nd_ld4(rb + 4 * q);
+                nf_fma<CO>(acc[0], xa, wl + q * CO * 4);
+                nf_fma<CO>(acc[1], xb, wl + q * CO * 4);
+            }
+        }
+        if (nq1 > 0) {
+            const float* ra = d.p1 + pc[0] * d.ld1;
+            const float* rb = d.p1 + pc[1] * d.ld1;
+#pragma unroll 4
+            for (int q = part; q < nq1; q += 4) {
+                const f32x4 xa = nd_ld4(ra + 4 * q), xb = nd_ld4(rb + 4 * q);
+                nf_fma<CO>(acc[0], xa, wl + (nq0 + q) * CO * 4);
+                nf_fma<CO>(acc[1], xb, wl + (nq0 + q) * CO * 4);
+            }
+        }
+        {
+            const float* ra = d.t + pc[0] * d.ldt;
+            const float* rb = d.t + pc[1] * d.ldt;
+            const float* ma = d.mad + (pc[0] / d.HW) * 3 * d.c2;
+            const float* mb = d.mad + (pc[1] / d.HW) * 3 * d.c2;
+#pragma unroll 4
+            for (int q = part; q < nq2; q += 4) {
+                const f32x4 ta = nd_ld4(ra + 4 * q), tb = nd_ld4(rb + 4 * q);
+                const f32x4 xa = nd_silu4((ta - nd_ld4(ma + 4 * q)) * nd_ld4(ma + d.c2 + 4 * q) + nd_ld4(ma + 2 * d.c2 + 4 * q));
+                const f32x4 xb = nd_silu4((tb - nd_ld4(mb + 4 * q)) * nd_ld4(mb + d.c2 + 4 * q) + nd_ld4(mb + 2 * d.c2 + 4 * q));
+                nf_fma<CO>(acc[0], xa, wl + (nq0 + nq1 + q) * CO * 4);
+                nf_fma<CO>(acc[1], xb, wl + (nq0 + nq1 + q) * CO * 4);
+            }
+        }
+#pragma unroll
+        for (int j = 0; j < 2; ++j) {
+#pragma unroll
+            for (int n = 0; n < CO; ++n) {
+                acc[j][n] += __int_as_float(__builtin_amdgcn_update_dpp(0, __float_as_int(acc[j][n]), 0xB1, 0xF, 0xF, true));
+                acc[j][n] += __int_as_float(__builtin_amdgcn_update_dpp(0, __float_as_int(acc[j][n]), 0x4E, 0xF, 0xF, true));
+            }
+            if (part == 0 && pix[j] < P) {
+#pragma unroll
+                for (int q = 0; q < CO / 4; ++q) {
+                    f32x4 v = {acc[j][4 * q], acc[j][4 * q + 1], acc[j][4 * q + 2], acc[j][4 * q + 3]};
+                    v += nd_ld4(d.bias + 4 * q);
+                    if (d.res0) v += nd_ld4(d.res0 + pix[j] * d.ldr0 + 4 * q);
+                    nd_st4(d.out + pix[j] * d.ldo + 4 * q, v);
+                }
+            }
+        }
+    }
+}
+
+__global__ void pack_narrow_fold_kernel(const float* __restrict__ wf, const float* __restrict__ bf, const float* __restrict__ wr, const float* __restrict__ br,
+                                        float* __restrict__ w_out, float* __restrict__ b_out, int cin_r, int mid, int cout, int CO) {
+    const int total = (cin_r + mid) * CO;
+    for (int i = blockIdx.x * blockDim.x + threadIdx.x; i < total + CO; i += gridDim.x * blockDim.x) {
+        if (i >= total) {
+            const int n = i - total;
+            double s = 0.0;
+            if (n < cout) {
+                for (int j = 0; j < mid; ++j) s += (double)wf[(size_t)n * mid + j] * (double)(br ? br[j] : 0.0f);
+                s += (double)(bf ? bf[n] : 0.0f);
+            }
+            b_out[n] = (float)s;
+            continue;
+        }
+        const int e = i & 3, r = i >> 2, n = r % CO, k = (r / CO) * 4 + e;
+        float v = 0.0f;
+        if (n < cout) {
+            if (k < cin_r) {
+                double s = 0.0;
+                for (int j = 0; j < mid; ++j) s += (double)wf[(size_t)n * mid + j] * (double)wr[(size_t)j * cin_r + k];
+                v = (float)s;
+            } else {
+                v = wf[(size_t)n * mid + (k - cin_r)];
+            }
+        }
+        w_out[i] = v;
+    }
+}
+
 __global__ void pack_pointwise_kernel(const float* __restrict__ w, float* __restrict__ out,
                                       int cin, int cout, int cinP, int coutP, int unshuffle_c, int transposed) {
     const size_t total = (size_t)cinP * coutP;
@@ -1144,6 +1254,42 @@
 
 extern "C" int nd_pointwise_gemm_split_takes(const nd_pointwise* d) { return d && pw_split_takes(d) ? 1 : 0; }
 
+extern "C" int nd_pointwise_narrow_fold_takes(int c0, int c1, int c2, int cout) {
+    return c0 > 0 && c1 >= 0 && c2 > 0 && c0 % 4 == 0 && c1 % 4 == 0 && c2 % 4 == 0 && (cout == 4 || cout == 8) && (long)(c0 + c1 + c2) * cout <= 8192;
+}
+
+extern "C" int64_t nd_pack_narrow_fold_floats(int cin, int cout) { return (int64_t)nd_round_up(cin, 4) * nd_round_up(cout, 4); }
+
+extern "C" int nd_pack_narrow_fold(const float* wf, const float* bf, const float* wr, const float* br, float* w_out, float* b_out, int cin_r, int mid, int cout,
+                                   void* stream) {
+    ND_REQUIRE(wf && wr && w_out && b_out, ND_E_BADARG, "nd_pack_narrow_fold: null pointer");
+    ND_REQUIRE(cin_r > 0 && mid > 0 && cout > 0 && cin_r % 4 == 0 && mid % 4 == 0, ND_E_SHAPE, "nd_pack_narrow_fold: %d -> %d -> %d (widths of the wide layer in fours)", cin_r, mid, cout);
+    const int CO = nd_round_up(cout, 4), total = (cin_r + mid) * CO + CO;
+    hipLaunchKernelGGL(pack_narrow_fold_kernel, dim3(nd_cdiv(total, 256)), dim3(256), 0, (hipStream_t)stream, wf, bf, wr, br, w_out, b_out, cin_r, mid, cout, CO);
+    return nd_launch_status("nd_pack_narrow_fold");
+}
+
+extern "C" int nd_pointwise_narrow_fold_nhwc_f32(const nd_narrow_fold* d, void* stream) {
+    ND_REQUIRE(d, ND_E_BADARG, "nd_pointwise_narrow_fold: null descriptor");
+    ND_REQUIRE(d->p0 && d->t && d->mad && d->weight && d->bias && d->out, ND_E_BADARG, "nd_pointwise_narrow_fold: null tensor pointer");
+    ND_REQUIRE(d->B > 0 && d->HW > 0 && (long)d->B * d->HW < (1L << 31), ND_E_BADARG, "nd_pointwise_narrow_fold: B = %d, HW = %d", d->B, d->HW);
+    ND_REQUIRE((d->c1 == 0) == (d->p1 == nullptr), ND_E_BADARG, "nd_pointwise_narrow_fold: p1/c1 mismatch");
+    ND_REQUIRE(nd_pointwise_narrow_fold_takes(d->c0, d->c1, d->c2, d->cout), ND_E_SHAPE,
+               "nd_pointwise_narrow_fold: %d + %d + %d -> %d is not a shape of this kernel (channels in fours, cout 4 or 8, cin * cout <= 8192: "
+               "nd_pointwise_narrow_fold_takes)", d->c0, d->c1, d->c2, d->cout);
+    ND_REQUIRE(d->ld0 >= d->c0 && (d->c1 == 0 || d->ld1 >= d->c1) && d->ldt >= d->c2 && d->ldo >= d->cout && (!d->res0 || d->ldr0 >= d->cout), ND_E_SHAPE,
+               "nd_pointwise_narrow_fold: a pixel stride below its channel count");
+    ND_REQUIRE(d->ld0 % 4 == 0 && d->ld1 % 4 == 0 && d->ldt % 4 == 0 && d->ldo % 4 == 0 && d->ldr0 % 4 == 0, ND_E_ALIGN, "nd_pointwise_narrow_fold: pixel strides must be multiples of 4");
+    ND_REQUIRE(nd_aligned16(d->p0) && nd_aligned16(d->p1) && nd_aligned16(d->t) && nd_aligned16(d->mad) && nd_aligned16(d->weight) && nd_aligned16(d->bias) &&
+               nd_aligned16(d->res0) && nd_aligned16(d->out), ND_E_ALIGN, "nd_pointwise_narrow_fold: pointers must be 16-byte aligned");
+    const long blocks = ((long)d->B * d->HW + 127) / 128;
+    const int grid = (int)(blocks < 8L * nd_device_cus() ? blocks : 8L * nd_device_cus());
+    const size_t lds = (size_t)(d->c0 + d->c1 + d->c2) * d->cout * sizeof(float);
+    if (d->cout == 4) hipLaunchKernelGGL((pointwise_narrow_fold_kernel<4>), dim3(grid), dim3(256), lds, (hipStream_t)stream, *d);
+    else hipLaunchKernelGGL((pointwise_narrow_fold_kernel<8>), dim3(grid), dim3(256), lds, (hipStream_t)stream, *d);
+    return nd_launch_status("nd_pointwise_narrow_fold_nhwc_f32");
+}
+
 extern "C" int64_t nd_pack_pointwise_weight_split_floats(int cin, int cout) {
     return (int64_t)nd_round_up(cin, 32) * nd_round_up(cout, 128) * 3 / 2;
 }
diff --git a/noisediff_amd/csrc/pwchain.hip b/noisediff_amd/csrc/pwchain.hip
--- a/noisediff_amd/csrc/pwchain.hip
+++ b/noisediff_amd/csrc/pwchain.hip
@@ -8,6 +8,10 @@
     nd_chain d;
     int n_tiles;
     int tiles_per_sample;
+    const float* mad;
+    const float* r0;
+    const float* r1;
+    int ldr0, ldr1;
 };
 
 template <int K, int N>
@@ -152,10 +156,11 @@
 
 template <bool SPLIT> constexpr int chain_w_floats(int n, int k) { return SPLIT ? n * k * 3 / 2 : n * k; }
 
-template <int K0, int N1, int N2, int N3, int MODE, bool SPLIT = false>
+template <int K0, int N1, int N2, int N3, int MODE, bool SPLIT = false, bool TAIL = false>
 __global__ __launch_bounds__(chain_threads(N1, SPLIT, K0), 1) void chain_kernel(const ChainArgs a) {
     constexpr int THREADS = chain_threads(N1, SPLIT, K0), WAVES = THREADS / 64;
     static_assert(!SPLIT || K0 % 16 == 0, "SPLIT: the first stage reads whole 16-channel K steps");
+    static_assert(!TAIL || (SPLIT && MODE == ND_PRO_NONE), "TAIL: a prologue of the SPLIT form");
     extern __shared__ __attribute__((aligned(16))) float lds[];
     float* w1 = lds;
     float* w2 = w1 + chain_w_floats<SPLIT>(N1, K0);
@@ -166,6 +171,7 @@
     float* gam = b3 + (N3 > 0 ? N3 : 0);
     float* bet = gam + K0;
     float* vst = bet + K0;
+    float* mst = vst + WAVES * K0;
 
     const int tid = threadIdx.x, lane = tid & 63, wave = tid >> 6, half = lane >> 5;
     const nd_src& s = a.d.src;
@@ -196,6 +202,7 @@
     const int n_waves = gridDim.x * WAVES, wid = blockIdx.x * WAVES + wave;
     const int t_begin = (int)((long)wid * a.n_tiles / n_waves), t_end = (int)((long)(wid + 1) * a.n_tiles / n_waves);
     float* myv = vst + wave * K0;
+    float* mym = mst + wave * 3 * K0;
     int b_cur = -1;
     const int cout_last = a.d.st[N3 > 0 ? 2 : 1].cout;
 
@@ -205,7 +212,12 @@
     const __amdgpu_buffer_rsrc_t rs1 = __builtin_amdgcn_make_buffer_rsrc(const_cast<float*>(s.p1 ? s.p1 : s.p0), 0,
                                                                           s.p1 ? (int)((unsigned)a.d.B * a.d.HW * s.ld1 * 4u) : 0, 0x00020000);
     const __amdgpu_buffer_rsrc_t rso = __builtin_amdgcn_make_buffer_rsrc(a.d.out, 0, (int)((unsigned)a.d.B * a.d.HW * a.d.ldo * 4u), 0x00020000);
+    const __amdgpu_buffer_rsrc_t rr0 = __builtin_amdgcn_make_buffer_rsrc(const_cast<float*>(TAIL ? a.r0 : s.p0), 0,
+                                                                          TAIL ? (int)((unsigned)a.d.B * a.d.HW * a.ldr0 * 4u) : 0, 0x00020000);
+    const __amdgpu_buffer_rsrc_t rr1 = __builtin_amdgcn_make_buffer_rsrc(const_cast<float*>(TAIL && a.r1 ? a.r1 : s.p0), 0,
+                                                                          TAIL && a.r1 ? (int)((unsigned)a.d.B * a.d.HW * a.ldr1 * 4u) : 0, 0x00020000);
     f32x4 Xn[SPLIT ? K0 / 8 : 1], Xm[TWO ? K0 / 8 : 1];
+    f32x4 R0n[TAIL ? K0 / 8 : 1], R1n[TAIL ? K0 / 8 : 1];
     auto prefetch_rows = [&](int t_) {
         const unsigned pix_ = (unsigned)t_ * 32u + (unsigned)(lane & 31);
 #pragma unroll
@@ -214,6 +226,10 @@
             Xn[SPLIT ? q : 0] = __builtin_bit_cast(f32x4, __builtin_amdgcn_raw_buffer_load_b128(rs0, c < s.c0 ? (pix_ * (unsigned)s.ld0 + c) * 4u : OOB, 0, 0));
             if constexpr (TWO)
                 Xm[q] = __builtin_bit_cast(f32x4, __builtin_amdgcn_raw_buffer_load_b128(rs1, (c >= s.c0 && c < cin) ? (pix_ * (unsigned)s.ld1 + (c - s.c0)) * 4u : OOB, 0, 0));
+            if constexpr (TAIL) {
+                R0n[q] = __builtin_bit_cast(f32x4, __builtin_amdgcn_raw_buffer_load_b128(rr0, c < cin ? (pix_ * (unsigned)a.ldr0 + c) * 4u : OOB, 0, 0));
+                R1n[q] = __builtin_bit_cast(f32x4, __builtin_amdgcn_raw_buffer_load_b128(rr1, c < cin ? (pix_ * (unsigned)a.ldr1 + c) * 4u : OOB, 0, 0));
+            }
         }
     };
     if constexpr (SPLIT) {
@@ -232,12 +248,23 @@
             for (int c = lane; c < K0; c += 64) myv[c] = c < cin ? s.vec[(size_t)b * cin + c] : 0.0f;
             b_cur = b;
         }
+        if (TAIL && b != b_cur) {
+            for (int c = lane; c < 3 * K0; c += 64) {
+                const int j = c / K0, cc = c - j * K0;
+                mym[c] = cc < cin ? a.mad[((size_t)b * 3 + j) * cin + cc] : 0.0f;
+            }
+            b_cur = b;
+        }
         f32x4 X[K0 / 8];
         if constexpr (SPLIT) {
 #pragma unroll
             for (int q = 0; q < K0 / 8; ++q) {
                 X[q] = Xn[q];
                 if constexpr (TWO) X[q] += Xm[q];
+                if constexpr (TAIL) {
+                    const float* m = mym + 8 * q + 4 * half;
+                    X[q] = nd_silu4((X[q] - nd_ld4(m)) * nd_ld4(m + K0) + nd_ld4(m + 2 * K0)) + R0n[q] + R1n[q];
+                }
             }
             prefetch_rows(t + 1 < t_end ? t + 1 : t);
             if (s.vec) {
@@ -360,16 +387,17 @@
     }
 }
 
-template <int K0, int N1, int N2, int N3, int MODE, bool SPLIT = false>
+template <int K0, int N1, int N2, int N3, int MODE, bool SPLIT = false, bool TAIL = false>
 int launch(const ChainArgs& a, hipStream_t st) {
     static nd_device_once configured;
     constexpr int THREADS = chain_threads(N1, SPLIT, K0), WAVES = THREADS / 64;
-    const size_t lds = (size_t)(chain_w_floats<SPLIT>(N1, K0) + chain_w_floats<SPLIT>(N2, N1) + chain_w_floats<SPLIT>(N3, N2) + N1 + N2 + N3 + 2 * K0 + WAVES * K0) * sizeof(float);
-    static_assert((size_t)(chain_w_floats<SPLIT>(N1, K0) + chain_w_floats<SPLIT>(N2, N1) + chain_w_floats<SPLIT>(N3, N2) + N1 + N2 + N3 + 2 * K0 + 16 * K0) * 4 <= 160 * 1024, "LDS");
-    if (int e = nd_reserve_lds(configured, reinterpret_cast<const void*>(chain_kernel<K0, N1, N2, N3, MODE, SPLIT>), lds, "nd_pointwise_chain")) return e;
+    constexpr int STASH = (TAIL ? 4 : 1) * K0;
+    const size_t lds = (size_t)(chain_w_floats<SPLIT>(N1, K0) + chain_w_floats<SPLIT>(N2, N1) + chain_w_floats<SPLIT>(N3, N2) + N1 + N2 + N3 + 2 * K0 + WAVES * STASH) * sizeof(float);
+    static_assert((size_t)(chain_w_floats<SPLIT>(N1, K0) + chain_w_floats<SPLIT>(N2, N1) + chain_w_floats<SPLIT>(N3, N2) + N1 + N2 + N3 + 2 * K0 + 16 * STASH) * 4 <= 160 * 1024, "LDS");
+    if (int e = nd_reserve_lds(configured, reinterpret_cast<const void*>(chain_kernel<K0, N1, N2, N3, MODE, SPLIT, TAIL>), lds, "nd_pointwise_chain")) return e;
     const int wgs = nd_cdiv(a.n_tiles, WAVES);
     const int grid = wgs < nd_device_cus() ? wgs : nd_device_cus();
-    hipLaunchKernelGGL((chain_kernel<K0, N1, N2, N3, MODE, SPLIT>), dim3(grid), dim3(THREADS), lds, st, a);
+    hipLaunchKernelGGL((chain_kernel<K0, N1, N2, N3, MODE, SPLIT, TAIL>), dim3(grid), dim3(THREADS), lds, st, a);
     return 0;
 }
 
@@ -448,7 +476,7 @@
     ND_REQUIRE(nd_pointwise_chain_supported(cin, d->st[0].cout, d->st[1].cout, n3), ND_E_SHAPE,
                "nd_pointwise_chain: widths %d->%d->%d->%d are not instantiated (use nd_pointwise_gemm_nhwc_f32 per layer)", cin,
                d->st[0].cout, d->st[1].cout, n3);
-    ChainArgs a;
+    ChainArgs a{};
     a.d = *d;
     a.tiles_per_sample = d->HW / 32;
     const long tiles = (long)d->B * a.tiles_per_sample;
@@ -499,6 +527,48 @@
     return nd_launch_status("nd_pointwise_chain_nhwc_f32");
 }
 
+extern "C" int nd_pointwise_chain_tail_takes(int cin, int n1, int n2, int n3) {
+    return n3 == 0 && (cin == 64 || cin == 48) && nd_round_up(n1, 32) == 64 && n1 > 0 && nd_round_up(n2, 32) == 32 && n2 > 0;
+}
+
+extern "C" int nd_pointwise_chain_tail_split_nhwc_f32(const nd_chain_tail* dt, void* stream) {
+    ND_REQUIRE(dt, ND_E_BADARG, "nd_pointwise_chain_tail: null descriptor");
+    const nd_chain* d = &dt->chain;
+    const nd_src& s = d->src;
+    ND_REQUIRE(d->n_stages == 2 && s.p0 && d->out && dt->mad && dt->r0, ND_E_BADARG, "nd_pointwise_chain_tail: two stages, t, mad, r0 and out");
+    ND_REQUIRE(d->B > 0 && d->HW > 0 && d->HW % 32 == 0, ND_E_SHAPE, "nd_pointwise_chain_tail: HW=%d must be a positive multiple of 32", d->HW);
+    ND_REQUIRE(s.c1 == 0 && !s.p1 && s.mode == ND_PRO_NONE && !s.vec && !s.upsample && !s.unshuffle && !s.rowstats, ND_E_BADARG,
+               "nd_pointwise_chain_tail: one plain source (the affine + SiLU is this entry point's own prologue)");
+    const int cin = s.c0;
+    ND_REQUIRE(nd_pointwise_chain_tail_takes(cin, d->st[0].cout, d->st[1].cout, 0), ND_E_SHAPE,
+               "nd_pointwise_chain_tail: widths %d->%d->%d are not instantiated (nd_affine_silu_add_f32, then the chain)", cin, d->st[0].cout, d->st[1].cout);
+    ND_REQUIRE(s.ld0 >= cin && s.ld0 % 4 == 0 && dt->ldr0 >= cin && dt->ldr0 % 4 == 0 && (!dt->r1 || (dt->ldr1 >= cin && dt->ldr1 % 4 == 0)), ND_E_ALIGN,
+               "nd_pointwise_chain_tail: pixel strides must be >= channels and multiples of 4");
+    int width = cin;
+    for (int i = 0; i < 2; ++i) {
+        const nd_chain_stage& g = d->st[i];
+        ND_REQUIRE(g.weight && g.cin == width && g.cout > 0 && g.res == ND_CHAIN_RES_NONE, ND_E_SHAPE, "nd_pointwise_chain_tail: stage %d is %d->%d, expected input width %d, no residual",
+                   i, g.cin, g.cout, width);
+        ND_REQUIRE(nd_aligned16(g.weight), ND_E_ALIGN, "nd_pointwise_chain_tail: weights must be 16-byte aligned");
+        width = g.cout;
+    }
+    ND_REQUIRE(width % 4 == 0 && d->ldo >= width && d->ldo % 4 == 0, ND_E_SHAPE, "nd_pointwise_chain_tail: output width %d, ldo %d", width, d->ldo);
+    ND_REQUIRE(nd_aligned16(s.p0) && nd_aligned16(d->out) && nd_aligned16(dt->mad) && nd_aligned16(dt->r0) && nd_aligned16(dt->r1), ND_E_ALIGN,
+               "nd_pointwise_chain_tail: tensors must be 16-byte aligned");
+    const long px = (long)d->B * d->HW, lim = (1L << 32) - 65536;
+    ND_REQUIRE(px * s.ld0 * 4 < lim && px * dt->ldr0 * 4 < lim && px * (dt->r1 ? dt->ldr1 : 0) * 4 < lim && px * d->ldo * 4 < lim, ND_E_SHAPE,
+               "nd_pointwise_chain_tail: a tensor of 4 GiB or more");
+    ChainArgs a{};
+    a.d = *d;
+    a.tiles_per_sample = d->HW / 32;
+    ND_REQUIRE(px / 32 < (1L << 31), ND_E_SHAPE, "nd_pointwise_chain_tail: too many pixels");
+    a.n_tiles = (int)(px / 32);
+    a.mad = dt->mad;  a.r0 = dt->r0;  a.r1 = dt->r1;  a.ldr0 = dt->ldr0;  a.ldr1 = dt->r1 ? dt->ldr1 : 0;
+    const int rc = cin == 64 ? launch<64, 64, 32, 0, ND_PRO_NONE, true, true>(a, (hipStream_t)stream) : launch<48, 64, 32, 0, ND_PRO_NONE, true, true>(a, (hipStream_t)stream);
+    if (rc) return rc;
+    return nd_launch_status("nd_pointwise_chain_tail_split_nhwc_f32");
+}
+
 #ifdef CHAIN_STAMP
 extern "C" int nd_chain_debug_read(unsigned long long* host, int n_words) {
     return (int)hipMemcpyFromSymbol(host, HIP_SYMBOL(chain_dbg), (size_t)n_words * 8);
diff --git a/noisediff_amd/engine.py b/noisediff_amd/engine.py
--- a/noisediff_amd/engine.py
+++ b/noisediff_amd/engine.py
@@ -35,6 +35,8 @@
 _SPLIT = os.environ.get("ND_SPLIT_GEMM", "1")
 SPLIT_GEMM = _SPLIT != "0"
 SPLIT_CHAIN, SPLIT_PW = _SPLIT in ("1", "chain"), _SPLIT in ("1", "pw")
+FOLD_FINAL = os.environ.get("ND_FOLD_FINAL", "1") != "0"
+SHOT_TAIL = os.environ.get("ND_SHOT_TAIL", "1") != "0"
 TIME_TABLE = True
 PROJ_TABLE = True
 TIME_TABLE_ROWS = 1000
@@ -177,6 +179,11 @@
         add("tproj.weight", j * 4 * self.dim, "derived", (j, 4 * self.dim))
         add("tproj.bias", j, "derived", (j,))
         add("time_freqs", self.dim // 2, "derived", (self.dim // 2,))
+        wr, wf = self.slots.get("final_res_block.res_conv.weight"), self.slots.get("final_conv.weight")
+        if wr is not None and wf is not None and wf.shape[1] == wr.shape[0] and wr.shape[1] == 2 * wr.shape[0] and \
+                self.lib.nd_pointwise_narrow_fold_takes(wr.shape[0], wr.shape[0], wr.shape[0], wf.shape[0]):
+            add("final_fold.weight", self.lib.nd_pack_narrow_fold_floats(wr.shape[1] + wr.shape[0], wf.shape[0]), "derived", (wf.shape[0], wr.shape[1] + wr.shape[0]))
+            add("final_fold.bias", wf.shape[0], "derived", (wf.shape[0],))
         self.time_table = TIME_TABLE and 4 * self.dim <= 2048 and self.lib.nd_cond_step_lds_bytes(16, self.dim) <= 160 * 1024
         if self.time_table:
             add("time_table", TIME_TABLE_ROWS * 4 * self.dim, "derived", (TIME_TABLE_ROWS, 4 * self.dim))
@@ -245,6 +252,11 @@
                     L.call("nd_pack_conv7x7_weight", t.data_ptr(), dst, p.shape[0], st)
                     if p.name + ".split" in self.slots:
                         L.call("nd_pack_conv7x7_weight_split", t.data_ptr(), self.p(p.name + ".split"), p.shape[0], st)
+            if "final_fold.weight" in self.slots:
+                raw = {p.name: t for p, t in zip([q for q in self.spec if q.name in self.slots], keep)}
+                wr, wf = raw["final_res_block.res_conv.weight"], raw["final_conv.weight"]
+                L.call("nd_pack_narrow_fold", wf.data_ptr(), raw["final_conv.bias"].data_ptr(), wr.data_ptr(), raw["final_res_block.res_conv.bias"].data_ptr(),
+                       self.p("final_fold.weight"), self.p("final_fold.bias"), wr.shape[1], wr.shape[0], wf.shape[0], st)
             L.call("nd_stream_sync", st)
             tw = torch.cat([self.view(r + ".mlp.1.weight") for r in self.resnet_names])
             tb = torch.cat([self.view(r + ".mlp.1.bias") for r in self.resnet_names])
@@ -609,7 +621,7 @@
                   act_in, act_out, self.e.stream)
 
     def resnet(self, name: str, x: torch.Tensor, skip: Optional[torch.Tensor], cout: int, H: int, W: int, groups: int,
-               posmap: Optional[torch.Tensor] = None, extra_res: Optional[torch.Tensor] = None) -> torch.Tensor:
+               posmap: Optional[torch.Tensor] = None, extra_res: Optional[torch.Tensor] = None, tail: bool = True):
         cin = x.shape[-1] + (skip.shape[-1] if skip is not None else 0)
         HW = H * W
         c1, st1, sc1, n1 = self.conv3(name + ".block1.proj", self._src(x, skip), cin, cout, H, W, stats=True)
@@ -633,6 +645,9 @@
         if a1 is not None:
             self._release(a1)
         mad2 = self.gn_finalize(st2, sc2, n2, name + ".block2.norm", cout, groups, None)
+        if not tail:
+            self._release(c1, st1, sc1, mad1, st2, sc2)
+            return c2, mad2
         if cin != cout:
             assert extra_res is None
             out = self.pw(name + ".res_conv", self._src(x, skip), cin, cout, HW, W, gn_t=c2, gn_mad=mad2)
@@ -646,14 +661,16 @@
         self._release(c1, st1, sc1, mad1, c2, st2, sc2, mad2)
         return out.view(self.B, H, W, cout)
 
-    def chain(self, name: str, src: L.Src, stages, HW: int) -> torch.Tensor:
+    def chain(self, name: str, src: L.Src, stages, HW: int, tail=None) -> torch.Tensor:
         e = self.e
         out = self._alloc(self.B, HW, stages[-1][2])
         split = all((layer + ".weight.chain_s") in e.slots for layer, *_ in stages) and (src.c1 == 0 or stages[0][1] <= 16)
         ldo = stages[-1][2]
+        if tail is not None and not split:
+            raise L.HipError(f"{name}: the tail prologue is a form of the split chain only")
         rows = self.B
         if split:
-            per = 4 * HW * max(src.ld0, src.ld1, ldo)
+            per = 4 * HW * max(src.ld0, src.ld1, ldo, *([t.shape[-1] for t in tail[1:] if t is not None] if tail else []))
             rows = max(1, min(self.B, _CHAIN_SPLIT_LIMIT // per))
             rows = -(-self.B // -(-self.B // rows))
         for b0 in range(0, self.B, rows):
@@ -670,9 +687,19 @@
             for i, (layer, cin, cout, act, res) in enumerate(stages):
                 d.st[i].weight, d.st[i].bias = e.p(layer + (".weight.chain_s" if split else ".weight.chain")), e.p(layer + ".bias")
                 d.st[i].cin, d.st[i].cout, d.st[i].act, d.st[i].res = cin, cout, act, res
-            self._add("nd_pointwise_chain_split_nhwc_f32" if split else "nd_pointwise_chain_nhwc_f32", C.byref(d), e.stream,
-                      meta={"layer": name, "B": nb, "HW": HW, "cin": stages[0][1], "cout": stages[-1][2], "split": int(split),
-                            "flop_per_px": 2.0 * sum(c_in * c_out for _, c_in, c_out, _, _ in stages)})
+            meta = {"layer": name, "B": nb, "HW": HW, "cin": stages[0][1], "cout": stages[-1][2], "split": int(split),
+                    "flop_per_px": 2.0 * sum(c_in * c_out for _, c_in, c_out, _, _ in stages)}
+            if tail is not None:
+                mad, r0, r1 = tail
+                dt = L.ChainTail()
+                dt.chain, dt.mad = d, mad.data_ptr() + 4 * b0 * 3 * src.c0
+                dt.r0, dt.ldr0 = r0.data_ptr() + 4 * b0 * HW * r0.shape[-1], r0.shape[-1]
+                if r1 is not None:
+                    dt.r1, dt.ldr1 = r1.data_ptr() + 4 * b0 * HW * r1.shape[-1], r1.shape[-1]
+                self._add("nd_pointwise_chain_tail_split_nhwc_f32", C.byref(dt), e.stream, meta=meta)
+                self._keep.append(dt)
+                continue
+            self._add("nd_pointwise_chain_split_nhwc_f32" if split else "nd_pointwise_chain_nhwc_f32", C.byref(d), e.stream, meta=meta)
             self._keep.append(d)
         return out
 
@@ -775,11 +802,21 @@
             r_shot = self.mlp("shot_mlp1", self._src(self.clean, self.x), 2 * e.inp_dim, d, d, H, W)
             s = self.attn_block("shot_attn", r_shot, H, W)
             s2 = self.mlp("shot_mlp2", self._src(s), d, d, d, H, W)
-            s3 = self.resnet("shot_time", s2, None, d, H, W, SHOT_GROUPS, extra_res=r_shot)
-            shot_noise = self._tap("shot_noise", self.mlp("shot_mlp3", self._src(s3), d, d, e.inp_dim, H, W))
-            for nm, tt in (("shot_mlp1", r_shot), ("shot_attn", s), ("shot_mlp2", s2), ("shot_time", s3)):
-                self._tap(nm, tt)
-            self._release(r_shot, s, s2, s3)
+            if (SHOT_TAIL and not self.debug and SPLIT_CHAIN and self._chain_ok(H * W, (d, d, e.inp_dim)) and e.lib.nd_pointwise_chain_tail_takes(d, d, e.inp_dim, 0)
+                    and all(n + ".weight.chain_s" in e.slots for n in ("shot_mlp3.fc1", "shot_mlp3.fc2"))):
+                c2, mad2 = self.resnet("shot_time", s2, None, d, H, W, SHOT_GROUPS, tail=False)
+                shot_noise = self.chain("shot_time.tail+shot_mlp3", self._src(c2), [("shot_mlp3.fc1", d, d, L.ACT_GELU, L.CHAIN_RES_NONE),
+                                                                                   ("shot_mlp3.fc2", d, e.inp_dim, L.ACT_NONE, L.CHAIN_RES_NONE)], H * W,
+                                        tail=(mad2, s2, r_shot)).view(B, H, W, e.inp_dim)
+                self._release(r_shot, s, s2, c2, mad2)
+                s3 = None
+            else:
+                s3 = self.resnet("shot_time", s2, None, d, H, W, SHOT_GROUPS, extra_res=r_shot)
+                shot_noise = self._tap("shot_noise", self.mlp("shot_mlp3", self._src(s3), d, d, e.inp_dim, H, W))
+            if s3 is not None:
+                for nm, tt in (("shot_mlp1", r_shot), ("shot_attn", s), ("shot_mlp2", s2), ("shot_time", s3)):
+                    self._tap(nm, tt)
+                self._release(r_shot, s, s2, s3)
         x0 = self._alloc(B, H, W, d)
         stem_split = "init_conv.weight.split" in e.slots
         self._add("nd_conv7x7_c4_split_f32" if stem_split else "nd_conv7x7_c4_f32", self.x.data_ptr(),
@@ -844,6 +881,21 @@
             self._tap(p + ".0", x1); self._tap(p + ".1", x2); self._tap(p + ".2", xa); self._tap(f"up{i}", x)
         xp = self._tap("pos_block2", self.resnet("pos_block2", x, None, d, H, W, POS_GROUPS, posmap=pm2))
         self._release(x)
+        if FOLD_FINAL and not self.debug and "final_fold.weight" in e.slots:
+            c2, mad2 = self.resnet("final_res_block", xp, x0, d, H, W, G, tail=False)
+            nf = L.NarrowFold()
+            nf.p0, nf.p1, nf.t, nf.mad = xp.data_ptr(), x0.data_ptr(), c2.data_ptr(), mad2.data_ptr()
+            nf.weight, nf.bias, nf.out = e.p("final_fold.weight"), e.p("final_fold.bias"), self.model_out.data_ptr()
+            nf.B, nf.HW, nf.c0, nf.c1, nf.c2, nf.ld0, nf.ld1, nf.ldt, nf.cout, nf.ldo = B, H * W, d, d, d, d, d, d, e.inp_dim, e.inp_dim
+            if shot_noise is not None:
+                nf.res0, nf.ldr0 = shot_noise.data_ptr(), e.inp_dim
+            self._add("nd_pointwise_narrow_fold_nhwc_f32", C.byref(nf), e.stream,
+                      meta={"layer": "final_res_block.res_conv+final_conv", "B": B, "HW": H * W, "cin": 3 * d, "cout": e.inp_dim})
+            self._keep.append(nf)
+            self._release(xp, x0, c2, mad2)
+            if shot_noise is not None:
+                self._release(shot_noise)
+            return
         xf = self._tap("final_res_block", self.resnet("final_res_block", xp, x0, d, H, W, G))
         self._release(xp, x0)
         self.pw("final_conv", self._src(xf), d, e.inp_dim, H * W, W, res0=shot_noise, out=self.model_out)
```

Result: faster. 0.9663 patches/s (median of 6 runs) (+2.2%).
